# vvvvvw/Sentinel

Hardware: AMD Instinct MI355X
Metric: decided entries/sec (whole node) at 1M resources; % of HBM roofline (higher is better)
Workload: dtype int64/f64

## Files before the change

### sentinel_amd/csrc/chain.h

```cpp
#pragma once
#include <hip/hip_runtime.h>
#include <stdint.h>

#include "../../include/sentinel_gpu.h"
#include "dev_types.h"

namespace sg {

__device__ __forceinline__ int64_t j_d2l(double d) {
    if (d != d) return 0;
    if (d >= 9223372036854775807.0) return INT64_MAX;
    if (d <= -9223372036854775808.0) return INT64_MIN;
    return (int64_t)d;
}
__device__ __forceinline__ int32_t j_d2i(double d) {
    if (d != d) return 0;
    if (d >= 2147483647.0) return INT32_MAX;
    if (d <= -2147483648.0) return INT32_MIN;
    return (int32_t)d;
}
__device__ __forceinline__ int32_t j_iadd(int32_t a, int32_t b) { return (int32_t)((uint32_t)a + (uint32_t)b); }
__device__ __forceinline__ int64_t j_round(double a) {
    int64_t bits = __double_as_longlong(a);
    int64_t biased = (bits & 0x7ff0000000000000LL) >> 52;
// ... 307 lines not shown
__device__ __forceinline__ int64_t try_occupy_next(Node& N, const Ctx& C, int64_t now, int acquire, double threshold,
                                                   int32_t occupy_timeout) {
    const double max_count = threshold * 1000 / 1000;
    const int64_t cur_borrow = bor_waiting(N.bor, now);
    if ((double)cur_borrow >= max_count) return occupy_timeout;
    const int64_t wlen = 500;
    int64_t earliest = now - now % wlen + wlen - 1000;
    int64_t idx = 0;
    sec_current(N, now, C.max_rt);
    int64_t cur_pass = SEC_SUM(N, now, pass);
    while (earliest < now) {
        const int64_t wait = idx * wlen + wlen - now % wlen;
        if (wait >= occupy_timeout) break;
        const int64_t wp = sec_window_pass(N, earliest);
        if ((double)(cur_pass + cur_borrow + acquire - wp) <= max_count) return wait;
        earliest += wlen;
        cur_pass -= wp;
        ++idx;
    }
    return occupy_timeout;
}
__device__ __forceinline__ int default_can_pass_prio(Node& N, const Ctx& C, const DRule& r, int64_t t, int acquire,
                                                     int32_t occupy_timeout, int64_t& wait) {
    int32_t cur;
    if (r.grade == SG_FLOW_GRADE_THREAD) cur = N.thread;
    else { sec_current(N, t, C.max_rt); cur = j_d2i((double)SEC_SUM(N, t, pass)); }
    if (!((double)j_iadd(cur, acquire) > r.count)) return 1;
    if (r.grade != SG_FLOW_GRADE_QPS || !N.bor) return 0;
    const int64_t w = try_occupy_next(N, C, t, acquire, r.count, occupy_timeout);
    if (w >= occupy_timeout) return 0;
    const int bs = bor_current(N.bor, t + w);
    if (bs >= 0) N.bor[2 * bs + 1] += acquire;
    min_current(N, C.minb, t, C.max_rt, C.pflags);
    if (!(N.mst & MS_DETACHED)) {
        N.mb.occ += acquire;
        N.mb.pass += acquire;
        N.mst |= MS_DIRTY;
    }
    wait = w;
    return 2;
}

__device__ __forceinline__ void stat_entry(Node& N, const Ctx& C, int64_t t, int count, bool passed) {
    int sl = sec_current(N, t, C.max_rt);
    min_current(N, C.minb, t, C.max_rt, C.pflags);
    if (passed) {
        N.thread++;
        sec_add(N, sl, count, 0, 0, 0, 0, INT64_MAX);
        min_add(N, count, 0, 0, 0, 0, INT64_MAX);
    } else {
        sec_add(N, sl, 0, count, 0, 0, 0, INT64_MAX);
        min_add(N, 0, count, 0, 0, 0, INT64_MAX);
    }
}
__device__ __forceinline__ void stat_exit(Node& N, const Ctx& C, int64_t t, int count, int64_t rt) {
    int sl = sec_current(N, t, C.max_rt);
    sec_add(N, sl, 0, 0, count, rt, 0, rt);
    min_current(N, C.minb, t, C.max_rt, C.pflags);
    min_add(N, 0, 0, count, rt, 0, rt);
    N.thread--;
}
__device__ __forceinline__ void stat_trace(Node& N, const Ctx& C, int64_t t, int count) {
    if (count <= 0) return;
    int sl = sec_current(N, t, C.max_rt);
    sec_add(N, sl, 0, 0, 0, 0, count, INT64_MAX);
    min_current(N, C.minb, t, C.max_rt, C.pflags);
    if (!(N.mst & MS_DETACHED)) {
        min_add(N, 0, 0, 0, 0, count, INT64_MAX);
        if (N.exc_sum_sec == t - t % 1000) N.exc_sum += count;
    }
}

__device__ __forceinline__ void node_store(const Node& N, const DevState& S, uint32_t res, uint32_t pflags) {
    S.sec[(uint64_t)res * 2 + 0] = N.sb[0];
    S.sec[(uint64_t)res * 2 + 1] = N.sb[1];
    NodeInfo o = S.info[res];
    o.thread = N.thread;
    o.flags = N.flags;
    o.exc_sum_sec = (pflags & PF_EXC_COUNT) ? N.exc_sum_sec : -1;
    o.exc_sum = N.exc_sum;
    S.info[res] = o;
}

}
```

### sentinel_amd/csrc/decide.hip

```cpp
#include <hip/hip_runtime.h>
#include <stdlib.h>
#include <stdint.h>

#include "authority.h"
#include "chain.h"
#include "aux.h"
#include "pmap.h"

using namespace sg;

#define WAVE 64
#define MAXR 16
#define JMAX_FLOW 4
#define JMAX_DEG 4
#define JMAX_RL 2

__device__ __forceinline__ uint32_t lane_id() { return __lane_id(); }
__device__ __forceinline__ uint64_t lanemask_lt() {
    uint32_t l = lane_id();
    return l == 0 ? 0ull : (~0ull >> (64 - l));
}

#define J8_MAX (1u << 23)
#define SEG_ITEMS 16
// ... 1079 lines not shown
                if (r.kind == SG_EV_EXIT) {
                    const uint64_t ref = r.code == RC_NONE ? SG_REF_NONE
                                         : r.code == RC_BATCH ? S.gbase + (vals[r.x] & 0x7FFFFFFFu) : (aux & SG_REF_NONE);
                    lane_exit<NRMAX>(N, C, S, cfg, pg, res, t, r, x, ref, bflags, LP);
                } else {
                    stat_trace(N, C, t, r.cnt);
                }
            }
            LPROF(ktc)
        }
        if (r.kind == SG_EV_ENTRY) dec[sg.start + j] = d;
    }
    min_flush(N, C.minb);
    node_store(N, S, res, pg.pflags);
    if (L.mid != NO_ID) pm_store(S, L.mid, L.mp);
    if (L.tid != NO_ID) pm_store(S, L.tid, L.tm);
#pragma unroll
    for (int s = 0; s < NRMAX; ++s) if (s < nr) S.rstate[pg.rule_off + s] = rs[s];
#ifdef SG_KPROF
    if (kp) {
        S.dbg[32] += kta; S.dbg[33] += ktb; S.dbg[34] += ktc; S.dbg[35] += sg.len; S.dbg[36] += 1;
    }
#endif
#undef LPROF
}
template <int NRMAX>
__global__ __launch_bounds__(256) void k_lane(const SEv* __restrict__ recs, const sg_event* __restrict__ ev,
                                              const uint32_t* __restrict__ vals, const Seg* __restrict__ segs,
                                              const uint32_t* __restrict__ order, uint32_t m, DevState S, DevCfg cfg,
                                              int64_t t0, uint32_t* __restrict__ dec, uint32_t* __restrict__ bflags) {
    const uint32_t i = blockIdx.x * blockDim.x + threadIdx.x;
    if (i >= m) return;
    lane_seg<NRMAX>(recs, ev, vals, segs[order[i]], S, cfg, t0, dec, bflags, i);
}

struct MinDelta {
    int32_t p, b, s, rt, e, minrt;
};
struct LiteMin {
    int64_t T;
    MinDelta pd;
    int64_t H;
};
__device__ __forceinline__ void md_zero(MinDelta& d) { d.p = d.b = d.s = d.rt = d.e = 0; d.minrt = INT32_MAX; }
__device__ __forceinline__ bool md_full(const MinDelta& d) { return (uint32_t)(d.p | d.b | d.s | d.rt | d.e) >= 0x40000000u; }
__device__ __forceinline__ Bkt md_apply(Bkt b, int64_t T, const MinDelta& d, int32_t max_rt) {
    if (b.ws > T) return b;
    if (b.ws < T) bkt_reset(b, T, max_rt);
    b.pass += d.p; b.block += d.b; b.succ += d.s; b.rt += d.rt; b.exc += d.e;
    if ((int64_t)d.minrt < b.minrt) b.minrt = d.minrt;
    return b;
}
__device__ __forceinline__ void lm_put(LiteMin& L, Bkt* minb, int32_t max_rt, bool check, uint32_t* bflags) {
    if (L.T < 0) return;
    Bkt* p = minb + (L.T / 1000) % 60;
    if (L.T > L.H) {
        if (check && p->ws >= L.T) atomicOr(bflags, BF_LITE_STALE);
        Bkt b;
        bkt_reset(b, L.T, max_rt);
        b.pass = L.pd.p; b.block = L.pd.b; b.succ = L.pd.s; b.rt = L.pd.rt; b.exc = L.pd.e;
        if ((int64_t)L.pd.minrt < b.minrt) b.minrt = L.pd.minrt;
        *p = b;
        L.H = L.T;
    } else {
        *p = md_apply(*p, L.T, L.pd, max_rt);
    }
}
__device__ __forceinline__ void lm_roll(LiteMin& L, Node& N, Bkt* minb, int64_t T, int32_t max_rt, uint32_t pflags,
                                        bool check, uint32_t* bflags) {
    lm_put(L, minb, max_rt, check, bflags);
    L.T = T;
    md_zero(L.pd);
    if ((pflags & PF_EXC_COUNT) && N.exc_sum_sec < T) exc_advance(N, minb, T);
}
template <uint32_t CH>
__device__ __forceinline__ void lite_flush(uint32_t* __restrict__ dec, uint32_t base, uint32_t n, const uint32_t (&w)[CH],
                                           uint32_t& mask) {
#pragma unroll
    for (uint32_t m = 0; m < CH; ++m)
        if ((mask >> m) & 1u) dec[base + m - (CH - n)] = w[m];
    mask = 0;
}

#ifndef LITE_PL_WAVES
#define LITE_PL_WAVES 1
#endif
template <bool PL>
__global__ __launch_bounds__(256) __attribute__((amdgpu_waves_per_eu(PL ? LITE_PL_WAVES : 2))) void k_lite(const SEv* __restrict__ recs, const sg_event* __restrict__ ev,
                                              const uint32_t* __restrict__ vals, const Seg* __restrict__ segs,
                                              const uint32_t* __restrict__ order, uint32_t m, DevState S, DevCfg cfg,
                                              int64_t t0, uint32_t* __restrict__ dec, uint32_t* __restrict__ bflags) {
    const uint32_t i = blockIdx.x * blockDim.x + threadIdx.x;
    if (i >= m) return;
    const Seg sg = segs[order[i]];
    const uint32_t res = sg.res;
    const Prog pg = S.prog[res];
    Node N;
    node_load(N, S, res);
#ifndef LITE_CH
#define LITE_CH 4
#endif
    constexpr uint32_t CH = LITE_CH;
    const uint4* r4 = reinterpret_cast<const uint4*>(recs + sg.start);
    const uint32_t qmax = sg.len ? sg.len - 1 : 0;
    uint4 cur[CH], nxt[CH];
#pragma unroll
    for (uint32_t k = 0; k < CH; ++k) cur[k] = r4[k < qmax ? k : qmax];
    if (((pg.xf & XF_PLITE) != 0) != PL) return;
    const int nf = pg.n_flow, nd = pg.n_degrade;
    const DRule* rules = S.rules + pg.rule_off + (PL ? 1 : 0);
    __shared__ DRule spr[PL ? 256 : 1];
    __shared__ PMap smp[PL ? 256 : 1], stm[PL ? 256 : 1];
    DRule& pr = spr[PL ? threadIdx.x : 0];
    PmLaneRef PLM{NO_ID, NO_ID, smp[PL ? threadIdx.x : 0], stm[PL ? threadIdx.x : 0]};
    if (PL) {
        pr = S.rules[pg.rule_off];
        PLM.mid = pr.pmap;
        PLM.mp = S.pmap[pr.pmap];
        PLM.tid = tmap_of(S, pg.tm_base, 0);
        if (PLM.tid != NO_ID) PLM.tm = S.pmap[PLM.tid];
    }
    double fcnt[2] = {0.0, 0.0};
    bool fthr[2] = {false, false};
    uint32_t fslot[2] = {0, 0};
    DegParam dr[2];
    uint32_t dslot[2] = {0, 0};
    RState ds[2];
    if (nf + nd) {
        const int last = nf + nd - 1;
#pragma unroll
        for (int k = 0; k < 2; ++k) {
            const int fi = k < last ? k : last, di = nf + k < last ? nf + k : last;
            fcnt[k] = rules[fi].count;
            fthr[k] = rules[fi].grade == SG_FLOW_GRADE_THREAD;
            fslot[k] = rules[fi].slot;
            dr[k] = deg_param(rules[di]);
            dslot[k] = rules[di].slot;
            ds[k] = S.rstate[pg.rule_off + (PL ? 1 : 0) + di];
        }
    }
#ifdef SG_KPROF
    const bool kp = S.dbg && i == 0;
    unsigned long long kt0 = kp ? __builtin_amdgcn_s_memtime() : 0, kta = 0, ktb = 0, ktc = 0, ktd = 0, ktf = 0, ktg = 0, kth = 0;
#define LPROF(acc)                                                \
    if (kp) {                                                     \
        unsigned long long _n = __builtin_amdgcn_s_memtime();     \
        acc += _n - kt0;                                          \
        kt0 = _n;                                                 \
    }
#else
#define LPROF(acc)
#endif
    const Ctx C{S.minb + (uint64_t)res * 60, cfg.max_rt, pg.pflags};
    LiteMin L;
    L.T = -1;
    md_zero(L.pd);
    {
        const int64_t sw = N.sb[0].ws > N.sb[1].ws ? N.sb[0].ws : N.sb[1].ws;
        const int64_t sh = sw < 0 ? -1 : sw - sw % 1000;
        L.H = sh > cfg.snap_hi ? sh : cfg.snap_hi;
    }
    const bool lchk = (cfg.dbg_flags & LITE_CHECK) != 0;
    const bool has_chain = (N.flags & NI_CHAIN) != 0;
    const bool chain = has_chain && cfg.switch_on;
    if (sg.len && (t0 + recs[sg.start].dt) < (N.sb[0].ws > N.sb[1].ws ? N.sb[0].ws : N.sb[1].ws))
        atomicOr(bflags, BF_BACKWARD);
    uint64_t pm0 = 0, pm1 = 0, pm2 = 0, pm3 = 0;
#ifndef LITE_HOLD
#define LITE_HOLD 1
#endif
    uint32_t dw[CH], dmask = 0;
#pragma unroll
    for (uint32_t k = 0; k < CH; ++k) dw[k] = 0;
    LPROF(kta)
    for (uint32_t j0 = 0; j0 < sg.len; j0 += CH) {
    if (j0) lite_flush<CH>(dec, sg.start + j0 - CH, CH, dw, dmask);
#pragma unroll
    for (uint32_t k = 0; k < CH; ++k) nxt[k] = r4[j0 + CH + k < qmax ? j0 + CH + k : qmax];
#pragma unroll 1
    for (uint32_t k = 0; k < CH; ++k) {
        const uint4 rw = cur[0];
#pragma unroll
        for (uint32_t m = 0; m + 1 < CH; ++m) cur[m] = cur[m + 1];
        const uint32_t j = j0 + k;
        if (j >= sg.len) break;
        const int32_t rdt = (int32_t)rw.x;
        const uint32_t rx = rw.y;
        const int cntv = (int)(rw.z & 0xFFFFu);
        const int32_t rtv = (int32_t)(rw.z >> 16);
        const uint32_t kind = rw.w & 0xFFu, code = (rw.w >> 16) & 0xFFu;
        const int64_t t = t0 + rdt;
        const int64_t T = t - t % 1000;
        uint32_t d = mk_dec(ST_NOT_ENTRY, 0, 0);
        if (kind == SG_EV_ENTRY) {
            if (!chain) d = mk_dec(ST_NO_CHECK, 0, 0);
            else {
                if (T != L.T || md_full(L.pd)) lm_roll(L, N, C.minb, T, C.max_rt, C.pflags, lchk, bflags);
                uint32_t status = ST_PASS, slot = 0;
                uint64_t key = NO_KEY;
                if (PL) {
                    N.flags |= NI_PM | ni_tm(0);
                    if ((rw.w >> 8) & SG_F_HAS_ARG)
                        key = S.key_ring[(S.gbase + (vals[sg.start + j] & 0x7FFFFFFFu)) & cfg.ring_mask];
                    if (key != NO_KEY && !param_default_lane(S, pr, PLM.mp, cntv, key, t, bflags)) {
                        status = ST_BLOCK_PARAM;
                        slot = pr.slot;
                    }
                }
#pragma unroll
                for (int k = 0; k < 2; ++k) {
                    if (k < nf && status == ST_PASS) {
                        int32_t cur;
                        if (fthr[k]) cur = N.thread;
                        else { sec_current(N, t, C.max_rt); cur = j_d2i((double)SEC_SUM(N, t, pass)); }
                        if ((double)j_iadd(cur, cntv) > fcnt[k]) { status = ST_BLOCK_FLOW; slot = fslot[k]; }
                    }
                }
                LPROF(ktf)
                const int64_t exc_total = N.exc_sum;
#pragma unroll
                for (int k = 0; k < 2; ++k) {
                    if (k < nd && status == ST_PASS && !degrade_pass(N, C, dr[k], ds[k], t, &exc_total)) {
                        status = ST_BLOCK_DEGRADE;
                        slot = dslot[k];
                    }
                }
                LPROF(ktg)
                const bool passed = status == ST_PASS;
                const int sl = sec_current(N, t, C.max_rt);
                if (passed) {
                    N.thread++;
                    sec_add(N, sl, cntv, 0, 0, 0, 0, INT64_MAX);
                    L.pd.p += cntv;
                } else {
                    sec_add(N, sl, 0, cntv, 0, 0, 0, INT64_MAX);
                    L.pd.b += cntv;
                }
                LPROF(kth)
                if (PL && passed && key != NO_KEY && PLM.tid != NO_ID) thread_add_lane(S, PLM.tm, key, 1, bflags);
                d = passed ? mk_dec(ST_PASS, 0, 0) : mk_dec(status, slot, 0);
                if (passed && j < 256) {
                    const uint64_t b = 1ull << (j & 63);
                    if (j < 64) pm0 |= b; else if (j < 128) pm1 |= b; else if (j < 192) pm2 |= b; else pm3 |= b;
                }
            }
            LPROF(ktb)
        } else {
            bool eff;
            if (code == RC_NONE) eff = kind == SG_EV_EXIT ? chain : has_chain;
            else if (code == RC_PASSED) eff = true;
            else if (code == RC_NOT) eff = false;
            else {
                const uint32_t rel = rx - sg.start;
                if (rel >= j) { atomicOr(bflags, BF_BAD_REF); eff = false; }
                else if (rel < 256) {
                    const uint64_t w = rel < 64 ? pm0 : rel < 128 ? pm1 : rel < 192 ? pm2 : pm3;
                    eff = ((w >> (rel & 63)) & 1) != 0;
                } else {
                    if (rel >= j0) lite_flush<CH>(dec, sg.start + j0, k, dw, dmask);
                    eff = st_passed(dec[rx] & 0xFF);
                }
            }
            if (eff && kind == SG_EV_EXIT) {
                if (T != L.T || md_full(L.pd)) lm_roll(L, N, C.minb, T, C.max_rt, C.pflags, lchk, bflags);
                const int sl = sec_current(N, t, C.max_rt);
                sec_add(N, sl, 0, 0, cntv, rtv, 0, rtv);
                L.pd.s += cntv;
                L.pd.rt += rtv;
                if (rtv < L.pd.minrt) L.pd.minrt = rtv;
                N.thread--;
                const uint32_t rfl = (rw.w >> 8) & 0xFFu;
                if (PL && (rfl & SG_F_EXIT_ARGS) && (N.flags & NI_PM) && (N.flags & ni_tm(0)) && PLM.tid != NO_ID) {
                    uint64_t ref = SG_REF_NONE;
                    if (rfl & RF_OWN_ARGS) ref = S.gbase + (vals[sg.start + j] & 0x7FFFFFFFu);
                    else if (code == RC_BATCH) ref = S.gbase + (vals[rx] & 0x7FFFFFFFu);
                    else if (code == RC_PASSED) ref = ev[vals[sg.start + j] & 0x7FFFFFFFu].aux & SG_REF_NONE;
                    if (ref != SG_REF_NONE) {
                        const uint64_t key = S.key_ring[ref & cfg.ring_mask];
                        if (key != NO_KEY) thread_add_lane(S, PLM.tm, key, -1, bflags);
                    }
                }
            } else if (eff && cntv > 0) {
                if (T != L.T || md_full(L.pd)) lm_roll(L, N, C.minb, T, C.max_rt, C.pflags, lchk, bflags);
                const int sl = sec_current(N, t, C.max_rt);
                sec_add(N, sl, 0, 0, 0, 0, cntv, INT64_MAX);
                L.pd.e += cntv;
                if (N.exc_sum_sec == T) N.exc_sum += cntv;
            }
            LPROF(ktc)
        }
#if LITE_HOLD
#pragma unroll
        for (uint32_t m = 0; m + 1 < CH; ++m) dw[m] = dw[m + 1];
        dw[CH - 1] = d;
        dmask = (dmask >> 1) | (kind == SG_EV_ENTRY ? 1u << (CH - 1) : 0u);
#else
        if (kind == SG_EV_ENTRY) dec[sg.start + j] = d;
#endif
    }
#pragma unroll
    for (uint32_t k = 0; k < CH; ++k) cur[k] = nxt[k];
    }
    if (sg.len) {
        const uint32_t jl = (sg.len - 1) / CH * CH;
        lite_flush<CH>(dec, sg.start + jl, sg.len - jl, dw, dmask);
    }
    lm_put(L, C.minb, C.max_rt, lchk, bflags);
    node_store(N, S, res, pg.pflags);
#pragma unroll
    for (int k = 0; k < 2; ++k)
        if (k < nd) S.rstate[pg.rule_off + (PL ? 1 : 0) + nf + k] = ds[k];
    if (PL) {
        pm_store(S, PLM.mid, PLM.mp);
        if (PLM.tid != NO_ID) pm_store(S, PLM.tid, PLM.tm);
    }
    LPROF(ktd)
#ifdef SG_KPROF
    if (kp) {
        S.dbg[32] += kta; S.dbg[33] += ktb; S.dbg[34] += ktc; S.dbg[35] += sg.len; S.dbg[36] += 1; S.dbg[37] += ktd; S.dbg[38] += ktf; S.dbg[39] += ktg; S.dbg[51] += kth;
    }
#endif
#undef LPROF
}

#define DPP_STEP(v, ident, ctrl, rmask, OP) \
    v = OP((uint32_t)__builtin_amdgcn_update_dpp((int)(ident), (int)(v), ctrl, rmask, 0xf, false), v)
#define WAVE_SCAN(v, ident, OP)              \
    do {                                      \
        DPP_STEP(v, ident, 0x111, 0xf, OP);   \
        DPP_STEP(v, ident, 0x112, 0xf, OP);   \
        DPP_STEP(v, ident, 0x114, 0xf, OP);   \
        DPP_STEP(v, ident, 0x118, 0xf, OP);   \
        DPP_STEP(v, ident, 0x142, 0xa, OP);   \
        DPP_STEP(v, ident, 0x143, 0xc, OP);   \
    } while (0)
__device__ __forceinline__ uint32_t op_add(uint32_t a, uint32_t b) { return a + b; }
__device__ __forceinline__ uint32_t op_min(uint32_t a, uint32_t b) { return a < b ? a : b; }
__device__ __forceinline__ uint32_t op_max(uint32_t a, uint32_t b) { return a > b ? a : b; }
__device__ __forceinline__ void wave_total64(uint32_t v, uint64_t* dst) {
    uint32_t lo = v & 0xFFFFu, hi = v >> 16;
    WAVE_SCAN(lo, 0u, op_add);
    WAVE_SCAN(hi, 0u, op_add);
    if (lane_id() == 63) *dst = (uint64_t)lo + ((uint64_t)hi << 16);
}
__device__ __forceinline__ uint32_t op_seg(uint32_t a, uint32_t b) {
    return (b & 0x80000000u) ? b : ((a & 0x80000000u) | ((a + b) & 0x7fffffffu));
}
__device__ __forceinline__ uint32_t shr1(uint32_t incl, uint32_t ident) {
    uint32_t v = (uint32_t)__shfl_up((int)incl, 1, 64);
    return lane_id() == 0 ? ident : v;
}
__device__ __forceinline__ int64_t wscan_i64_add(int64_t x) {
    const uint32_t l = lane_id();
#pragma unroll
    for (int o = 1; o < 64; o <<= 1) {
        int64_t y = __shfl_up(x, o, 64);
        if (l >= (uint32_t)o) x += y;
    }
    return x;
}
__device__ __forceinline__ int64_t wscan_i64_max(int64_t x) {
    const uint32_t l = lane_id();
#pragma unroll
    for (int o = 1; o < 64; o <<= 1) {
        int64_t y = __shfl_up(x, o, 64);
        if (l >= (uint32_t)o) x = x > y ? x : y;
    }
    return x;
}
#define NEG_INF64 ((int64_t)0x8000000000000000LL)

#define NO_LANE 0xFFFFFFFFu

#define ROW_SCAN(v, ident, OP, NWV)                                    \
    do {                                                               \
        if ((NWV) > 1) DPP_STEP(v, ident, 0x111, 0xf, OP);              \
        if ((NWV) > 2) DPP_STEP(v, ident, 0x112, 0xf, OP);              \
        if ((NWV) > 4) DPP_STEP(v, ident, 0x114, 0xf, OP);              \
        if ((NWV) > 8) DPP_STEP(v, ident, 0x118, 0xf, OP);              \
    } while (0)
template <int NW>
__device__ __forceinline__ uint32_t blk_min(const uint32_t* a) {
    static_assert(NW <= 16, "one DPP row");
    uint32_t v = lane_id() < (uint32_t)NW ? a[lane_id()] : NO_LANE;
    ROW_SCAN(v, NO_LANE, op_min, NW);
    return (uint32_t)__builtin_amdgcn_readlane((int)v, NW - 1);
}
template <int NW>
__device__ __forceinline__ uint32_t blk_sum_before(const uint32_t* a, uint32_t stride, uint32_t wv, uint32_t* tot) {
    static_assert(NW <= 16, "one DPP row");
    uint32_t v = lane_id() < (uint32_t)NW ? a[lane_id() * stride] : 0u;
    ROW_SCAN(v, 0u, op_add, NW);
    *tot = (uint32_t)__builtin_amdgcn_readlane((int)v, NW - 1);
    return wv == 0 ? 0u : (uint32_t)__builtin_amdgcn_readlane((int)v, (int)wv - 1);
// ... 2293 lines not shown
```

### sentinel_amd/csrc/dev_types.h

```cpp
#pragma once
#include <hip/hip_runtime.h>
#include <stdint.h>

#include "../../include/sentinel_gpu.h"

namespace sg {

struct AuthDesc;

struct Bkt {
    int64_t ws;
    int64_t pass;
    int64_t block;
    int64_t exc;
    int64_t succ;
    int64_t rt;
    int64_t occ;
    int64_t minrt;
};
static_assert(sizeof(Bkt) == 64, "Bkt must be 64 B");

#define NO_KEY 0xFFFFFFFFFFFFFFFFull

enum : uint32_t {
    NI_CHAIN = 1u,
    NI_REJECTED = 2u,
    NI_PM = 4u,
    NI_TOUCHED = 32u,
    NI_TM_SHIFT = 6u
};
__host__ __device__ inline uint32_t ni_tm(uint32_t idx) { return 1u << (NI_TM_SHIFT + idx); }

enum : uint8_t {
    PM_PRIO = 1,
    PM_LANE = 2,
    PM_AUX = 4,
    PM_ARGL = 8,
    PM_XARGS = 16
};
#define TAG_ORIGIN_BITS 20u
__host__ __device__ inline uint32_t tag_origin(uint32_t tag) { return tag & ((1u << TAG_ORIGIN_BITS) - 1); }
__host__ __device__ inline uint32_t tag_ctx(uint32_t tag) { return tag >> TAG_ORIGIN_BITS; }
#define RF_OWN_ARGS 0x80u
#define RF_PBLK 0x40u

struct NodeInfo {
    int32_t thread;
    uint32_t flags;
    int64_t exc_sum_sec;
    int64_t exc_sum;
    int64_t last_fetch;
};
static_assert(sizeof(NodeInfo) == 32, "NodeInfo must be 32 B");

enum : uint8_t {
    PF_EXC_COUNT = 1,
    PF_WARM = 2,
    PF_PQ = 4,
    PF_SERIAL = 8,
    PF_RL = 16,
    PF_RT = 32,
    PF_FROZEN = 64,
    PF_J16 = 128
};

struct Prog {
    uint32_t rule_off;
    uint8_t n_param, n_flow, n_degrade, pflags;
    uint32_t tm_base;
    uint16_t multi;
    uint16_t xf;
};
enum : uint16_t {
    XF_PTHREAD = 1,
    XF_MIX = 2,
    XF_PLITE = 4,
    XF_PVPQ = 8,
    XF_HEADT = 16,
    XF_HEADR = 32
};
enum : uint32_t {
    PX_MULTI = 1,
    PX_ORIGIN = 2,
    PX_CHAIN = 4
};
static_assert(sizeof(Prog) == 16, "Prog must be 16 B");

enum : uint8_t { RK_PARAM = 0, RK_FLOW = 1, RK_DEGRADE = 2 };

enum : uint32_t { LA_DEFAULT = 0, LA_ORIGIN = 1, LA_OTHER = 2 };
#define NO_ID 0xFFFFFFFFu
struct DRule {
    uint8_t kind;
    uint8_t grade;
    uint8_t behavior;
    uint8_t slot;
    int32_t max_queue;
    double count;
    double slope;
    int32_t warning_token;
    int32_t max_token;
    int32_t count_div_cold;
    int32_t time_window;
    int32_t burst;
    int32_t token_count;
    int64_t duration_sec;
    int64_t token_count_l;
    uint32_t hot_off, hot_n;
    uint32_t pmap;
    uint32_t ref;
    int32_t param_idx;
    uint32_t la_kind;
    uint32_t la_origin;
    uint32_t strategy;
    uint32_t chain_ctx;
    uint32_t pad[3];
};
#define NO_REF 0xFFFFFFFFu
#define PB_INIT_ONLY 0xFF
static_assert(sizeof(DRule) == 112, "DRule must be 112 B");

struct DHot {
    uint64_t key;
    int32_t count;
    int32_t pad;
};

struct RState {
    int64_t a;
    int64_t b;
    int64_t c;
    int64_t d;
};

#define PM_BKT 8
#define PK_EMPTY 0xFFFFFFFFFFFFFFFFull
struct PBucket {
    uint64_t key[PM_BKT];
    int64_t stamp[PM_BKT];
};
static_assert(sizeof(PBucket) == 128, "PBucket must be one 128-byte line");
struct PData {
    int64_t v0;
    int32_t v1;
    uint32_t pad;
};
static_assert(sizeof(PData) == 16, "PData must be 16 B");
#define PM_MIN_NB 2u
enum { PC_NEXT = 0, PC_FLOOR = 1, PC_RESCUES = 2, PC_RESCUE = 3, PC_WORDS = 4 };
__host__ __device__ inline uint32_t map_buckets(uint32_t cap) { return (2u * cap + PM_BKT - 1) / PM_BKT > 2u ? (2u * cap + PM_BKT - 1) / PM_BKT : 2u; }
struct PMap {
    uint64_t base;
    uint64_t bm;
    int64_t clock;
    int64_t thr;
    uint32_t nb;
    uint32_t cap;
    uint32_t live;
    uint32_t rb_log2;
    uint32_t pad[4];
};
static_assert(sizeof(PMap) == 64, "PMap must be 64 B");
#define PM_BASE_CAP 4000u
#define PM_TOTAL_CAP 200000u
#define PQ_MAX_CAP 8176u

enum : uint8_t { ST_PASS = 0, ST_PASS_WAIT = 1, ST_BLOCK_FLOW = 2, ST_BLOCK_DEGRADE = 3, ST_BLOCK_PARAM = 4,
                 ST_NO_CHECK = 5, ST_BLOCK_UPSTREAM = 6, ST_BLOCK_AUTHORITY = 7, ST_NOT_ENTRY = 0xFF };

// ... 86 lines not shown
    int64_t occ_pass, occ_req;
};
struct CSlot {
    int64_t key;
    uint32_t idx, pad;
};
#define CP_MAXN 16
struct PFlow {
    int64_t flow_id;
    double count;
    int32_t thr_type;
    int32_t n, interval;
    int32_t connected;
    uint32_t hoff, nhot;
    int64_t fws[CP_MAXN];
};
struct PHot {
    uint64_t key;
    int32_t count, pad;
};
#define PV_EMPTY 0xFFFFFFFFu
struct PVal {
    uint64_t key;
    uint32_t flow, pad;
    int64_t ws[CP_MAXN];
    int64_t cnt[CP_MAXN];
};
#define NS_BUCKETS 10
#define NS_WLEN 100
#define NS_INTERVAL 1000
struct NsLimiter {
    int64_t ws[NS_BUCKETS];
    int64_t cnt[NS_BUCKETS];
};

struct Link {
    uint64_t exit_l;
    uint64_t trace_l;
};
struct Span {
    uint32_t s, e, res;
    int32_t pint;
};
#define SPAN_CHUNK 8192u
#define BST_STATIC 0x80000000u
#define BST_CNT 0x7FFFFFFFu

struct AuxNode {
    unsigned long long key;
    int32_t thread;
    uint32_t flags;
    int64_t mws[2];
    int64_t mpass[2];
    int64_t pad0[2];
    Bkt sec[2];
    int64_t borrow[4];
    int64_t pad1[4];
};
static_assert(sizeof(AuxNode) == 256, "AuxNode size");
#define AUXF_BORROW 1u
#define AUX_EMPTY 0xFFFFFFFFFFFFFFFFull
enum : uint32_t { AUX_ORIGIN = 0, AUX_CONTEXT = 1 };
struct AuxAcc {
    uint32_t key;
    int32_t thread;
    int64_t W[2];
    uint64_t s[2][4];
    uint32_t minrt[2];
    int64_t MW[2];
    uint64_t mpass[2];
};
static_assert(sizeof(AuxAcc) == 128, "AuxAcc size");
#define AUX_PIECE 4096u

struct DevState {
    Bkt* sec;
    int64_t* borrow;
    const uint32_t* prio;
    uint64_t* key_ring;
    uint64_t gbase;
    Bkt* minb;
    NodeInfo* info;
    const Prog* prog;
    const DRule* rules;
    RState* rstate;
    const DHot* hot;
    PMap* pmap;
    PBucket* pbkt;
    PData* pdat;
    uint64_t* pbm;
    uint32_t* ppre;
    const uint32_t* tmid;
    uint8_t* ring;
    unsigned long long* dbg;
    uint32_t* sink;
    const Link* link;
    const uint32_t* bst;
    uint32_t* pend;
    Span* spans;
    uint32_t* nspan;
    uint32_t span_cap;
    uint32_t epoch;
    uint32_t skip_ok;
    uint32_t skip_min;
    const sg_event_ext* ext;
    const sg_arg* args;
    AuxNode* aux_tab;
    uint32_t* aux_count;
    uint32_t aux_cap;
    uint32_t max_ctx;
    uint64_t aux_mask;
    const AuthDesc* auth;
    const uint32_t* auth_ids;
};

enum : uint32_t { BF_PRIORITIZED = 1,
                  BF_PQ_INVARIANT = 2,
                  BF_PTAB_FULL = 4,
                  BF_BAD_RES = 8, BF_BAD_REF = 16,
                  BF_BACKWARD = 32, BF_TSPAN = 64,
                  BF_BAD_ARGS = 512,
                  BF_AUX_FULL = 1024,
                  BF_POOL_FULL = 2048,
                  BF_MULTI_LINK = 128,
                  BF_ZERO_CNT = 256,
                  BF_TINY_FALLBACK = 4096,
                  BF_TINY_REJECTED = 8192,
                  BF_LITE_STALE = 16384 };

struct SEv {
    int32_t dt;
    uint32_t x;
    uint16_t cnt;
    uint16_t rt;
    uint8_t kind;
    uint8_t flags;
    uint8_t code;
    uint8_t pad;
};
static_assert(sizeof(SEv) == 16, "SEv must be 16 B");
enum : uint8_t {
    RC_NONE = 0,
    RC_BATCH = 1,
    RC_PASSED = 2,
    RC_NOT = 3,
    RC_PREV = 4
};

enum : uint32_t {
    BIN_J16 = 0,
    BIN_J4 = 1,
    BIN_J1 = 2,
    BIN_PQ16 = 3,
    BIN_PQ4 = 4,
    BIN_J8 = 5,
    BIN_LANE = 6,
    LANE_BINS = 19,
    BIN_LANE16 = BIN_LANE + LANE_BINS,
    BIN_LITE = BIN_LANE16 + LANE_BINS,
    N_BINS = BIN_LITE + LANE_BINS
};

}
```

### sentinel_amd/csrc/engine.cpp

```cpp
#include <hip/hip_runtime.h>

#include <algorithm>
#include <array>
#include <chrono>
#include <cmath>
#include <cstdint>
#include <cstdio>
#include <cstdlib>
#include <cstring>
#include <deque>
#include <functional>
#include <map>
#include <set>
#include <string>
#include <unordered_map>
#include <vector>

#include "../../include/sentinel_gpu.h"
#include "authority.h"
#include "dev_types.h"
#include "pkeys.h"
#include "pmap.h"

namespace sg {
hipError_t launch_rs_first(const sg_event* ev, uint64_t n, uint32_t max_res, uint64_t gbase, const uint8_t* ring,
                           uint64_t ring_mask, int32_t max_rt, SEv* rec_o, uint32_t* keys, uint32_t* vals,
                           uint32_t* ghist, uint32_t nblocks, uint32_t* bflags, int64_t* t0_out, uint32_t* prio,
                           uint64_t* key_ring, const uint32_t* comp, const sg_event_ext* ext, const sg_arg* args,
                           uint64_t n_args, uint32_t max_ctx, const AuthDesc* auth, const uint32_t* auth_ids,
                           hipStream_t st);
hipError_t launch_radix_hist(const uint32_t* keys, uint64_t n, int shift, uint32_t* ghist, uint32_t nblocks,
                             hipStream_t st);
hipError_t launch_radix_hist_n(const uint32_t* keys, uint64_t n, const uint32_t* ndev, int shift, uint32_t* ghist,
                               uint32_t nblocks, hipStream_t st);
hipError_t launch_radix_scatter_n(const uint32_t* kin, const uint32_t* vin, uint64_t n, const uint32_t* ndev, int shift,
                                  const uint32_t* goff, uint32_t nblocks, uint32_t* kout, uint32_t* vout, hipStream_t st);
hipError_t launch_radix_scatter_x(const uint32_t* kin, const uint32_t* vin, uint64_t n, const uint32_t* ndev,
                                  const uint32_t* tcnt, const uint32_t* dbase, int shift, const uint32_t* goff,
                                  uint32_t nblocks, uint32_t* kout, uint32_t* vout, uint32_t* pos_of, hipStream_t st);
hipError_t launch_grp_first(const sg_event* ev, uint64_t n, uint32_t max_res, uint64_t gbase, uint64_t ring_mask,
                            uint32_t* bflags, int64_t* t0_out, uint32_t* prio, uint64_t* key_ring, const uint32_t* comp,
                            const sg_event_ext* ext, const sg_arg* args, uint64_t n_args, uint32_t max_ctx,
                            const AuthDesc* auth, const uint32_t* auth_ids,
                            const uint16_t* hot_tab, uint32_t nhot, uint32_t nblocks, uint32_t* words,
                            uint32_t* hot_hist, uint32_t* ckeys, uint32_t* cvals, uint32_t* ccnt, uint32_t* chist,
                            hipStream_t st);
hipError_t launch_hot_scan(uint32_t* C, uint32_t nblocks, uint32_t nhot, uint32_t* part, uint32_t* hb, uint32_t* total,
                           hipStream_t st);
hipError_t launch_hot_bmax(const sg_event* ev, uint32_t nblocks, const uint32_t* P, uint32_t nhot, const uint32_t* hb,
                           uint32_t* edges, uint32_t* bmax, hipStream_t st);
hipError_t launch_grp_records(const sg_event* ev, uint64_t n, uint64_t gbase, uint64_t ring_mask, int32_t max_rt,
                              const uint32_t* words, const uint32_t* P, uint32_t nhot, uint32_t nblocks,
                              const uint32_t* hb, SEv* recs, uint32_t* svals, uint32_t* prev,
                              uint32_t* nprev, uint32_t* bst, uint32_t* bflags, const sg_event_ext* ext,
                              const sg_arg* args, uint32_t max_ctx, Link* link, uint32_t epoch,
                              const uint32_t* need_hot, const uint32_t* need_blk, hipStream_t st);
hipError_t launch_hot_segs(const uint32_t* hb, uint32_t nhot, const uint32_t* hot_list, Seg* segs, uint32_t* out,
                           hipStream_t st);
hipError_t launch_hot_build(const Seg* segs, const uint32_t* mp, uint32_t mb, uint32_t min_len, uint32_t max_res, uint16_t* hot_tab,
                            uint32_t* hot_list, uint32_t nhot_old, uint32_t* hot_n, hipStream_t st);
hipError_t launch_cold_n(uint64_t n, const uint32_t* hot_total, uint32_t* out, hipStream_t st);
hipError_t launch_cold_small(const uint32_t* kin, const uint32_t* vin, const uint32_t* cnt, const uint32_t* dbase,
                             uint32_t* kout, uint32_t* vout, uint32_t* words, hipStream_t st);
uint32_t hot_max();
hipError_t launch_grp_clear(uint32_t* bsmall, uint32_t nsmall, uint32_t* bst, uint32_t nbst, uint32_t* need,
                            uint32_t nneed, hipStream_t st);
hipError_t launch_seg_cold(const uint32_t* keys, uint64_t n, const uint32_t* lo, const uint32_t* sbase, uint32_t* flag,
                           uint32_t* pos, Seg* segs, hipStream_t st,
                           hipError_t (*scan)(const uint32_t*, uint32_t*, uint64_t, uint32_t*, uint32_t*, hipStream_t),
                           uint32_t* part, uint32_t* ccount, uint32_t* nseg);
hipError_t launch_block_sums(const SEv* recs, uint64_t n, uint32_t* bst, Link* link, uint32_t epoch, uint32_t* bflags,
                             const uint32_t* skeys, const uint32_t* lo, const uint32_t* need_blk, hipStream_t st);
hipError_t launch_radix_scatter(const uint32_t* kin, const uint32_t* vin, uint64_t n, int shift, const uint32_t* goff,
                                uint32_t nblocks, uint32_t* kout, uint32_t* vout, uint32_t* pos_of, hipStream_t st);
uint32_t radix_tile();
hipError_t launch_scan(const uint32_t*, uint32_t*, uint64_t, uint32_t*, uint32_t*, hipStream_t);
hipError_t launch_snapshot(Bkt*, NodeInfo*, uint32_t, int64_t, int32_t, uint32_t*, uint32_t*, uint32_t*, uint32_t*,
                           sg_metric_node*, uint64_t, hipStream_t);
hipError_t launch_init_state(Bkt* sec, Bkt* minb, NodeInfo* info, int64_t* borrow, uint32_t nres, hipStream_t st);
hipError_t launch_set_flags(NodeInfo* info, const uint64_t* upd, uint32_t n, hipStream_t st);
hipError_t launch_region_copy(const uint64_t* src, uint64_t* dst, const uint64_t* tri, uint32_t n, hipStream_t st);
hipError_t launch_seg(const uint32_t* keys, uint64_t n, uint32_t* flag, uint32_t* pos, Seg* segs, hipStream_t st,
                      hipError_t (*scan)(const uint32_t*, uint32_t*, uint64_t, uint32_t*, uint32_t*, hipStream_t),
                      uint32_t* part, uint32_t* nseg);
hipError_t launch_seg_bin(Seg* segs, const uint32_t* mp, uint32_t mb, uint64_t n, const Prog* prog, const uint32_t* prio,
                          uint32_t lane_max, uint32_t j1_max, uint32_t j4_max, uint32_t force_lane, uint32_t* blkcnt,
                          uint32_t pq_ok, uint32_t pq_wide, uint32_t* aux, uint32_t* ashort, uint64_t* along,
                          uint64_t* amulti, uint32_t* mixc, uint32_t* mix, uint32_t mix_cap, uint32_t* mixlen,
                          uint32_t mix_wide, uint32_t head_min, const uint16_t* hot_tab, uint32_t nhot,
                          const uint32_t* nhotseg, uint32_t* need_hot, uint32_t* need_blk, const uint32_t* bmax,
                          uint32_t skip_min, uint32_t* nmark, hipStream_t st);
hipError_t launch_aux(const SEv* recs, const Seg* segs, const uint32_t* aux, const uint32_t* ashort,
                      const uint64_t* along, uint64_t* apiece, const uint64_t* amulti, const DevState& S, const DevCfg& cfg,
                      int64_t t0, const uint32_t* dec, AuxAcc* pool, uint32_t pool_cap, uint32_t* pool_n, uint64_t* meta,
                      uint32_t* bflags, hipStream_t st);
hipError_t launch_aux_cold(const SEv* recs, const Seg* segs, const uint32_t* aux, const uint32_t* ashort, const DevState& S,
                           const DevCfg& cfg, int64_t t0, const uint32_t* dec, uint32_t* bflags, hipStream_t st);
hipError_t launch_pq(int wide, const SEv* recs, const sg_event* ev, const uint32_t* vals, const Seg* segs,
                     const uint32_t* order, uint32_t m, const DevState& S, const DevCfg& cfg, int64_t t0, uint32_t* dec,
                     uint32_t* bflags, hipStream_t st);
hipError_t launch_pm_grow(const Seg* segs, const uint32_t* mp, uint32_t mb, const DevState& S, unsigned long long* pool_next,
                          uint64_t pool_nb, uint32_t* bflags, uint4* mv, uint32_t* nmv, uint32_t mcap, uint32_t epoch,
                          uint32_t nm, PBucket* b2, PData* d2, uint32_t* sz, uint32_t* off, uint32_t* part,
                          hipError_t (*scan)(const uint32_t*, uint32_t*, uint64_t, uint32_t*, uint32_t*, hipStream_t),
                          hipStream_t st);
hipError_t launch_pm_compact(PMap* pm, uint32_t n, const PBucket* ob, const PData* od, PBucket* nbk, PData* nd,
                             uint32_t* sz, uint32_t* off, uint32_t* part, unsigned long long* pool_next,
                             hipError_t (*scan)(const uint32_t*, uint32_t*, uint64_t, uint32_t*, uint32_t*, hipStream_t),
                             hipStream_t st);
hipError_t launch_pm_grow_ids(const uint32_t* ids, uint32_t n, const DevState& S, unsigned long long* pool_next,
                              uint64_t pool_nb, uint32_t* bflags, hipStream_t st);
hipError_t launch_pv_a(SEv* recs, const uint32_t* vals, Seg* segs, const uint32_t* list, uint32_t m,
                       const DevState& S, const DevCfg& cfg, uint32_t* dec, PvSeg* pv, PvBuf B, uint32_t cap,
                       uint32_t* tot, uint32_t* hist, uint32_t* part, hipStream_t st,
                       hipError_t (*radix_hist)(const uint32_t*, uint64_t, const uint32_t*, int, uint32_t*, uint32_t, hipStream_t),
                       hipError_t (*radix_scatter)(const uint32_t*, const uint32_t*, uint64_t, const uint32_t*, int,
                                                   const uint32_t*, uint32_t, uint32_t*, uint32_t*, hipStream_t),
                       hipError_t (*scan)(const uint32_t*, uint32_t*, uint64_t, uint32_t*, uint32_t*, hipStream_t),
                       uint32_t tile, uint32_t* rest, uint32_t grant_all);
hipError_t launch_pv_b(SEv* recs, Seg* segs, const uint32_t* list, uint32_t m, const DevState& S, int64_t t0,
                       uint32_t* dec, uint32_t* bflags, PvSeg* pv, PvBuf B, uint32_t cap, uint32_t* tot, uint32_t* part,
                       uint32_t jumps, hipStream_t st,
                       hipError_t (*scan)(const uint32_t*, uint32_t*, uint64_t, uint32_t*, uint32_t*, hipStream_t),
                       uint32_t* rest);
hipError_t launch_pvt(SEv* recs, const sg_event* ev, const uint32_t* vals, Seg* segs, const uint32_t* list, uint32_t m,
                      const DevState& S, const DevCfg& cfg, uint32_t* dec, uint32_t* bflags, PvSeg* pv, PvBuf B,
                      uint32_t cap, uint32_t* tot, uint32_t* hist, uint32_t* part, hipStream_t st,
                      hipError_t (*radix_hist)(const uint32_t*, uint64_t, const uint32_t*, int, uint32_t*, uint32_t, hipStream_t),
                      hipError_t (*radix_scatter)(const uint32_t*, const uint32_t*, uint64_t, const uint32_t*, int,
                                                      const uint32_t*, uint32_t, uint32_t*, uint32_t*, hipStream_t),
                      hipError_t (*scan)(const uint32_t*, uint32_t*, uint64_t, uint32_t*, uint32_t*, hipStream_t),
                      uint32_t tile, uint32_t* rest);
hipError_t launch_pq_mix(int post, SEv* recs, const sg_event* ev, const uint32_t* vals, const Seg* segs,
// ... 287 lines not shown
    h = h31(h, s.burst_count);
    h = h31(h, long_hash(s.duration_in_sec));
    int32_t lh = 1;
    for (auto& q : p.items) {
        int32_t e = q.has_obj ? j_string_hash(q.obj.c_str()) : 0;
        e = h31(e, q.has_count ? q.count : 0);
        e = h31(e, q.has_ct ? j_string_hash(q.ct.c_str()) : 0);
        lh = h31(lh, e);
    }
    h = h31(h, lh);
    h = h31(h, s.cluster_mode ? 1 : 0);
    int32_t ch = 0;
    if (s.cluster_mode || s.cluster_flow_id)
        ch = cluster_hash(s.cluster_flow_id, s.cluster_threshold_type, s.cluster_fallback_to_local, 0,
                          s.cluster_sample_count, s.cluster_window_interval_ms, false);
    p.hash = h31(h, ch);
    char buf[512];
    std::snprintf(buf, sizeof(buf), "%d|%016llx|%d|%d|%d|%lld|%d|%d:%d|", s.grade, (unsigned long long)dbl_bits(s.count),
                  s.control_behavior, s.max_queueing_time_ms, s.burst_count, (long long)s.duration_in_sec,
                  s.cluster_mode ? 1 : 0, s.has_param_idx, s.has_param_idx ? s.param_idx : 0);
    std::string k = std::string(buf) + p.res + "\x01" + p.la + "\x01";
    for (auto& q : p.items) {
        std::snprintf(buf, sizeof(buf), "[%d%d%d:%d]", q.has_obj, q.has_ct, q.has_count, q.has_count ? q.count : 0);
        k += buf + q.obj + "\x02" + q.ct + "\x03";
    }
    if (s.cluster_mode || s.cluster_flow_id) {
        std::snprintf(buf, sizeof(buf), "C%lld|%d|%d|%d|%d", (long long)s.cluster_flow_id, s.cluster_threshold_type,
                      s.cluster_fallback_to_local ? 1 : 0, s.cluster_sample_count, s.cluster_window_interval_ms);
        k += buf;
    }
    p.eqkey = k;
    return p;
}

template <class T> void dfree(T*& p) {
    if (p) (void)hipFree(p);
    p = nullptr;
}

}

#define TMAP_KEY (1ull << 63)
struct sg_engine {
    sg_config cfg;
    int device = 0;
    hipStream_t stream = nullptr;
    double last_ms[4] = {0, 0, 0, 0};

    std::unordered_map<std::string, uint32_t> ids;
    std::vector<std::string> names;
    uint32_t n_chains = 0;

    bool flow_loaded = false, deg_loaded = false, par_loaded = false;
    std::vector<std::string> last_flow, last_deg, last_par;
    std::vector<FlowR> flows;
    std::vector<DegR> degs;
    std::vector<ParamR> params;
    std::vector<std::vector<int>> res_flow, res_deg, res_par;
    std::map<std::string, uint32_t> psid_of;
    uint32_t next_psid = 1;
    std::map<uint32_t, uint32_t> rmap_cap;
    std::set<uint64_t> tmaps;
    std::vector<uint64_t> pmap_key;
    std::unordered_map<uint32_t, uint32_t> pmap_index;
    std::vector<uint32_t> tm_base;
    uint64_t n_pslot = 0;
    uint64_t pool_nb = 0;
    unsigned long long* d_pool_next = nullptr;
    uint4* d_pmoves = nullptr;
    PBucket* d_pbkt2 = nullptr;
    PData* d_pdat2 = nullptr;
    uint32_t* d_pcwork = nullptr;
    uint64_t pmoves_cap = 0;
    unsigned long long* h_pool_next = nullptr;
    uint64_t n_compact = 0;
    uint64_t pool2_nb = 0;
    uint32_t n_dev_rules = 0;

    Bkt* d_sec = nullptr;
    Bkt* d_minb = nullptr;
    int64_t snap_hi = -1;
    NodeInfo* d_info = nullptr;
    Prog* d_prog = nullptr;
    DRule* d_rules = nullptr;
    RState* d_rstate = nullptr;
    DHot* d_hot = nullptr;
    PMap* d_pmap = nullptr;
    PBucket* d_pbkt = nullptr;
    PData* d_pdat = nullptr;
    uint64_t* d_pbm = nullptr;
    uint32_t* d_ppre = nullptr;
    uint32_t* d_tmid = nullptr;
    uint8_t* d_ring = nullptr;
    uint32_t rules_cap = 0, hot_cap = 0;

    struct BatchSlot {
        sg_event* d_ev = nullptr;
        uint32_t* d_out = nullptr;
        uint32_t *d_k0 = nullptr, *d_v0 = nullptr, *d_k1 = nullptr, *d_v1 = nullptr;
        uint32_t *d_hist = nullptr, *d_part = nullptr, *d_flag = nullptr, *d_pos = nullptr, *d_order = nullptr;
        uint32_t *d_posof = nullptr, *d_dec = nullptr, *d_blkcnt = nullptr, *d_prev = nullptr;
        SEv *d_recs = nullptr, *d_rec_o = nullptr;
        uint32_t* d_ccnt = nullptr;
        bool radix = false;
        uint32_t nhot = 0;
        uint32_t hot_marked = 0;
        Seg* d_segs = nullptr;
        uint64_t* d_cand = nullptr;
        uint32_t* d_bsmall = nullptr;
        sg_event_ext* d_ext = nullptr;
        sg_arg* d_args = nullptr;
        uint64_t ext_cap = 0, args_cap = 0;
        uint32_t* d_ashort = nullptr;
        uint64_t *d_apiece = nullptr, *d_amulti = nullptr, *d_along = nullptr;
        uint64_t aux_cap_n = 0;
        uint32_t* d_mix = nullptr;
        uint64_t mix_cap = 0;
        Link* d_link = nullptr;
        uint32_t *d_bst = nullptr, *d_pend = nullptr;
        Span* d_spans = nullptr;
        hipEvent_t* ev = nullptr;
        hipEvent_t last_post = nullptr;
        uint32_t* h_head = nullptr;
        struct Grouped {
            uint64_t n = 0, n_args = 0, gbase = 0, ring_mask = 0;
            const sg_event* dev_ev = nullptr;
            const sg_event_ext* dev_ext = nullptr;
            const sg_arg* dev_args = nullptr;
            uint32_t *out = nullptr, *dev_out = nullptr, *vin = nullptr;
            uint32_t epoch = 0, skip_min = 0, lane_max = 0, mb = 0;
            bool ext = false, host_out = false, force_lane = false;
            int set = 0;
        } g;
    } slot[2];
    int cur = 0;
    int last = -1;
    int grouped = -1;
    int held_rc = 0;
    std::string held_msg;
    bool handoff_late = true;
    static constexpr int N_SETS = 4;
    hipEvent_t evset[N_SETS][5] = {};
    uint32_t* h_mirror = nullptr;
    uint64_t seq = 0;
    struct InFlight { int set; uint32_t hot_marked; };
    std::deque<InFlight> inflight;
    hipStream_t gstream = nullptr;
    std::vector<std::array<double, 4>> tlog;
    std::vector<std::array<double, 2>> glog;
    std::string fatal;
    uint32_t* d_prio = nullptr;
    uint16_t* d_hot_tab = nullptr;
    uint32_t* d_hot_list = nullptr;
    uint32_t nhot = 0;
    uint32_t* d_hot_part = nullptr;
    uint32_t* d_hot_hb = nullptr;
    uint32_t* d_need = nullptr;
    uint64_t need_words = 0;
    uint32_t* d_edges = nullptr;
    uint32_t hot_marked_last = 0;
    bool radix_group = false;
    uint64_t radix_below = 1u << 18;
    uint32_t tok_light = 8192;
    uint32_t tok_wide = 1024;
    bool tiny_on = true;
    AuxNode* d_auxtab = nullptr;
    uint32_t* d_auxcnt = nullptr;
    uint64_t aux_mask = 0;
    AuxAcc* d_auxpool = nullptr;
    uint64_t* d_auxmeta = nullptr;
    uint32_t auxpool_cap = 0;
    uint64_t auxmeta_cap = 0;
    std::unordered_map<std::string, uint32_t> origin_ids, context_ids;
    std::unordered_map<std::string, int> rule_names;
    AuthTable auth;
    AuthDesc* d_auth = nullptr;
    uint32_t* d_auth_ids = nullptr;
    size_t auth_ids_cap = 0;
    bool auth_on = false, auth_loaded = false;
    std::vector<std::string> last_auth;
    uint32_t* d_comp = nullptr;
    uint32_t* d_prev = nullptr;
    uint32_t* d_bsmall = nullptr;
    Link* d_link = nullptr;
    uint32_t *d_bst = nullptr, *d_pend = nullptr;
    Span* d_spans = nullptr;
    uint32_t span_cap = 0;
    uint32_t epoch = 0;
    uint64_t spans_total = 0;
    uint64_t cap_n = 0;
    sg_event* d_ev = nullptr;
    uint32_t* d_out = nullptr;
    uint32_t *d_k0 = nullptr, *d_v0 = nullptr, *d_k1 = nullptr, *d_v1 = nullptr;
    uint32_t *d_hist = nullptr, *d_part = nullptr, *d_flag = nullptr, *d_pos = nullptr, *d_order = nullptr;
    uint32_t *d_posof = nullptr, *d_dec = nullptr, *d_blkcnt = nullptr;
    SEv *d_recs = nullptr, *d_rec_o = nullptr;
    Seg* d_segs = nullptr;
    uint32_t* d_small = nullptr;
    uint32_t* d_sink = nullptr;
    int64_t* d_borrow = nullptr;
    uint64_t* d_keyring = nullptr;
    uint64_t* d_cand = nullptr;
    uint32_t dbg_flags = 0;
    int prof_bin = 0;
    unsigned long long* d_dbg = nullptr;
    uint64_t cap_hist = 0;
    uint64_t gbase = 0;
    hipStream_t bin_stream[2] = {nullptr, nullptr};
    hipEvent_t fork = nullptr, join[2] = {nullptr, nullptr};
    hipEvent_t fork0 = nullptr;
    hipEvent_t grown = nullptr;
    bool pipeline = true;
    int j1_stream = -1;
    uint32_t lane_max = 256, j1_max = 4096, j4_max = 65536;
    uint32_t head_min = 0;
    bool bins_pinned = false;
    uint32_t skip_min = 32768;
    bool pq_on = true;
    uint32_t pq_wide = 8192;
    bool mix_on = true;
    bool mix_pq = false;
    bool pv_pq = true;
    bool has_mix = false;
    bool has_head = false;
    bool pv_on = true;
    PvBuf pvb{};
    PvBuf pvbt{};
    bool has_multi = false;
    uint64_t pv_cap = 0;
    PvSeg* d_pvseg = nullptr;
    PvSeg* d_pvtseg = nullptr;
    uint32_t* d_pvrest = nullptr;
    bool pvt_on = false;
    uint64_t pvseg_cap = 0;
    uint64_t pvch_cap = 0;
    uint32_t *d_pvtot = nullptr, *d_pvhist = nullptr, *d_pvpart = nullptr, *d_pvthist = nullptr, *d_pvtpart = nullptr;
    uint32_t pv_last_m = 0;
    bool skip_pinned = false;
    std::vector<CFlow> cflows;
    std::unordered_map<int64_t, uint32_t> cmap;
    CFlow* d_cflow = nullptr;
    CBkt* d_cbkt = nullptr;
// ... 23 lines not shown
    uint32_t pftab_mask = 0;
    PVal* d_pvtab = nullptr;
    uint32_t pv_mask = 0;
    sg_param_token_req* d_preq = nullptr;
    uint64_t* d_pvals = nullptr;
    uint64_t pcap = 0, pvcap = 0;
    pk::Dict<pk::StdHash> pkeys;
    std::vector<uint64_t> par_pins;
    uint64_t* d_ks_key = nullptr;
    uint32_t *d_ks_idx = nullptr, *d_ks_marks = nullptr;
    uint64_t ks_cap = 0;
    hipEvent_t ks_ev[4] = {nullptr, nullptr, nullptr, nullptr};
    uint64_t ks_sweeps = 0, ks_last[4] = {0, 0, 0, 0};
    double ks_scan_ms[3] = {0, 0, 0};
    uint64_t pbm_words = 0;
    uint32_t *d_snap_cnt = nullptr, *d_snap_off = nullptr;
    sg_metric_node* d_snap_out = nullptr;
    uint64_t snap_cap = 0;
};

static int handoff(sg_engine* e);

namespace {

constexpr uint64_t SHARD_BATCH = 3ull << 21;

static void activate(sg_engine* e, int k) {
    auto& B = e->slot[k];
    e->d_ev = B.d_ev; e->d_out = B.d_out;
    e->d_k0 = B.d_k0; e->d_v0 = B.d_v0; e->d_k1 = B.d_k1; e->d_v1 = B.d_v1;
    e->d_hist = B.d_hist; e->d_part = B.d_part; e->d_flag = B.d_flag; e->d_pos = B.d_pos; e->d_order = B.d_order;
    e->d_posof = B.d_posof; e->d_dec = B.d_dec; e->d_blkcnt = B.d_blkcnt; e->d_prev = B.d_prev;
    e->d_recs = B.d_recs; e->d_rec_o = B.d_rec_o; e->d_segs = B.d_segs; e->d_cand = B.d_cand;
    e->d_bsmall = B.d_bsmall;
    e->d_link = B.d_link; e->d_bst = B.d_bst; e->d_pend = B.d_pend; e->d_spans = B.d_spans;
}
static void free_slot(sg_engine::BatchSlot& B) {
    dfree(B.d_ev); dfree(B.d_out); dfree(B.d_k0); dfree(B.d_v0); dfree(B.d_k1); dfree(B.d_v1);
    dfree(B.d_hist); dfree(B.d_part); dfree(B.d_flag); dfree(B.d_pos); dfree(B.d_order); dfree(B.d_segs);
    dfree(B.d_cand); dfree(B.d_posof); dfree(B.d_dec); dfree(B.d_recs); dfree(B.d_rec_o); dfree(B.d_blkcnt);
    dfree(B.d_prev); dfree(B.d_bsmall); dfree(B.d_ccnt);
    B.d_ccnt = nullptr;
    dfree(B.d_link); dfree(B.d_bst); dfree(B.d_pend); dfree(B.d_spans); dfree(B.d_ext); dfree(B.d_args);
    dfree(B.d_ashort); dfree(B.d_apiece); dfree(B.d_amulti); dfree(B.d_along); dfree(B.d_mix);
    B.d_mix = nullptr;
    B.ext_cap = B.args_cap = B.aux_cap_n = B.mix_cap = 0;
    B.d_link = nullptr; B.d_bst = B.d_pend = nullptr; B.d_spans = nullptr;
    B.d_ev = nullptr; B.d_out = nullptr; B.d_k0 = B.d_v0 = B.d_k1 = B.d_v1 = nullptr;
    B.d_hist = B.d_part = B.d_flag = B.d_pos = B.d_order = nullptr;
    B.d_posof = B.d_dec = B.d_blkcnt = B.d_prev = B.d_bsmall = nullptr;
    B.d_recs = B.d_rec_o = nullptr; B.d_segs = nullptr; B.d_cand = nullptr;
}
int ensure_batch(sg_engine* e, uint64_t n) {
    if (n <= e->cap_n) return SG_OK;
    uint64_t c = std::max<uint64_t>(n, 1u << 20);
    HIPCHK(hipStreamSynchronize(e->stream));
    uint64_t nblocks = (c + radix_tile() - 1) / radix_tile();
    e->cap_hist = nblocks * 256;
    for (auto& B : e->slot) {
        free_slot(B);
        HIPCHK(hipMalloc(&B.d_ev, c * sizeof(sg_event)));
        HIPCHK(hipMalloc(&B.d_out, c * 4));
        HIPCHK(hipMalloc(&B.d_k0, c * 4));
        HIPCHK(hipMalloc(&B.d_v0, c * 4));
        HIPCHK(hipMalloc(&B.d_k1, c * 4));
        HIPCHK(hipMalloc(&B.d_v1, c * 4));
        HIPCHK(hipMalloc(&B.d_hist, e->cap_hist * 4));
        HIPCHK(hipMalloc(&B.d_part, (e->cap_hist / 4096 + c / 4096 + 64) * 4));
        HIPCHK(hipMalloc(&B.d_flag, c * 4));
        HIPCHK(hipMalloc(&B.d_pos, c * 4));
        HIPCHK(hipMalloc(&B.d_order, c * 4));
        HIPCHK(hipMalloc(&B.d_segs, c * sizeof(Seg)));
        HIPCHK(hipMalloc(&B.d_cand, c * 8));
        HIPCHK(hipMalloc(&B.d_posof, c * 4));
        HIPCHK(hipMalloc(&B.d_dec, c * 4));
        HIPCHK(hipMalloc(&B.d_recs, c * sizeof(SEv)));
        const uint64_t co = (e->radix_group || c >= (1ull << 30)) ? c : std::min<uint64_t>(c, e->radix_below);
        if (co) HIPCHK(hipMalloc(&B.d_rec_o, co * sizeof(SEv)));
        HIPCHK(hipMalloc(&B.d_ccnt, 3 * (nblocks + 64) * 4));
    }
    dfree(e->d_hot_part);
    dfree(e->d_hot_hb);
    dfree(e->d_need);
    dfree(e->d_edges);
    e->need_words = hot_max() + c / 32768 + 2 + hot_max();
    HIPCHK(hipMalloc(&e->d_need, e->need_words * 4));
    HIPCHK(hipMalloc(&e->d_edges, (nblocks + 2) * 4));
    HIPCHK(hipMalloc(&e->d_hot_part, (nblocks / 16 + 2) * hot_max() * 4));
    HIPCHK(hipMalloc(&e->d_hot_hb, 2 * hot_max() * 4));
    for (auto& B : e->slot) {
        HIPCHK(hipMalloc(&B.d_blkcnt, ((c + 255) / 256 + 1) * N_BINS * 4));
        HIPCHK(hipMalloc(&B.d_prev, c * 4));
        HIPCHK(hipMalloc(&B.d_bsmall, 256 * 4));
        HIPCHK(hipMemset(B.d_bsmall, 0, 256 * 4));
        HIPCHK(hipMalloc(&B.d_link, c * sizeof(Link)));
        HIPCHK(hipMemset(B.d_link, 0, c * sizeof(Link)));
        HIPCHK(hipMalloc(&B.d_bst, ((c + 1023) / 1024 + 1) * 4));
        HIPCHK(hipMalloc(&B.d_pend, c * 4));
        HIPCHK(hipMalloc(&B.d_spans, (c / SPAN_CHUNK + 65536) * sizeof(Span)));
    }
    e->span_cap = (uint32_t)(c / SPAN_CHUNK + 65536);
    e->cap_n = c;
    activate(e, e->cur);
    return SG_OK;
}

constexpr uint32_t HEAD_WORDS = 77;
constexpr uint32_t MIRROR_WORDS = 121;

static int collect(sg_engine* e) {
    if (e->inflight.empty()) return SG_OK;
    const sg_engine::InFlight f = e->inflight.front();
    e->inflight.pop_front();
    hipEvent_t* ev = e->evset[f.set];
    HIPCHK(hipEventSynchronize(ev[4]));
    float g = 0, d = 0, p = 0;
    (void)hipEventElapsedTime(&g, ev[0], ev[1]);
    (void)hipEventElapsedTime(&d, ev[2], ev[3]);
    (void)hipEventElapsedTime(&p, ev[3], ev[4]);
    (void)hipGetLastError();
    e->last_ms[0] = g; e->last_ms[1] = d; e->last_ms[2] = p; e->last_ms[3] = (double)g + d + p;
    e->tlog.push_back({(double)g, (double)d, (double)p, (double)g + d + p});
    if (e->tlog.size() > 4096) e->tlog.erase(e->tlog.begin(), e->tlog.begin() + 2048);
    float ga = 0, gb = 0;
    const uint64_t collected = e->seq - e->inflight.size() - 1;
    if (collected > 0) {
        hipEvent_t* pv = e->evset[(f.set + sg_engine::N_SETS - 1) % sg_engine::N_SETS];
        if (hipEventElapsedTime(&ga, pv[1], ev[0]) != hipSuccess) ga = NAN;
        if (hipEventElapsedTime(&gb, pv[4], ev[2]) != hipSuccess) gb = NAN;
        (void)hipGetLastError();
    }
    e->glog.push_back({(double)ga, (double)gb});
    if (e->glog.size() > 4096) e->glog.erase(e->glog.begin(), e->glog.begin() + 2048);
    const uint32_t* mir = e->h_mirror + (size_t)f.set * MIRROR_WORDS;
    const uint32_t bflags = mir[0];
    e->spans_total += mir[120];
    e->hot_marked_last = f.hot_marked;
    if (bflags & BF_BAD_REF)
        return fail(SG_EINVAL, "an EXIT/TRACE references an event that is not an earlier ENTRY of the same resource");
    if (bflags & BF_BACKWARD)
        return fail(SG_EINVAL, "event timestamps must be non-decreasing across batches (SURVEY Q3)");
    if (bflags & BF_AUX_FULL) return fail(SG_ECAPACITY, "origin/context node pool full (raise aux_node_capacity)");
    if (bflags & BF_LITE_STALE)
        return fail(SG_ESTATE, "internal error (SG_LITE_CHECK): k_lite stored a minute bucket without a load that was not stale");
    if (bflags & BF_PQ_INVARIANT)
        e->fatal = "internal error: a k_pq tile's presorted key subset did not match its accesses";
    else if (bflags & BF_POOL_FULL)
        e->fatal = "the hot-parameter map pool is used up (raise param_table_log2)";
    else if (bflags & BF_PTAB_FULL)
        e->fatal = "a hot-parameter map table could not place a key (its map holds a ghost entry)";
    if (bflags & (BF_PQ_INVARIANT | BF_PTAB_FULL | BF_POOL_FULL)) return fail(SG_ECAPACITY, e->fatal + " -- engine unusable");
    return SG_OK;
}
static inline const AuthDesc* dev_auth(const sg_engine* e) { return e->auth_on ? e->d_auth : nullptr; }
static inline const uint32_t* dev_auth_ids(const sg_engine* e) { return e->auth_on ? e->d_auth_ids : nullptr; }

static int drain(sg_engine* e) {
    int rc = e->held_rc;
    std::string msg = e->held_msg;
    e->held_rc = 0;
    auto note = [&](int r) {
        if (r && !rc) { rc = r; msg = g_err; }
    };
    note(handoff(e));
    while (!e->inflight.empty()) note(collect(e));
    HIPCHK(hipStreamSynchronize(e->stream));
    return rc ? fail(rc, msg) : SG_OK;
}
static void drain_hold(sg_engine* e) {
    const int rc = drain(e);
    if (rc) { e->held_rc = rc; e->held_msg = g_err; }
}


static uint32_t rule_map_cap(int64_t duration_sec) {
    const int64_t c = (int64_t)PM_BASE_CAP * std::max<int64_t>(duration_sec, 1);
    return (uint32_t)std::min<int64_t>(c, PM_TOTAL_CAP);
}

int upload_rules(sg_engine* e, bool reset_flow_state, bool reset_deg_state, bool reset_par_state) {
    uint32_t R = e->cfg.max_resources;
    std::vector<Prog> prog(R);
    std::vector<DRule> rules;
    std::vector<RState> rst;
    std::vector<DHot> hot;
    std::vector<RState> old_rst;
    std::vector<Prog> old_prog;
    if ((!reset_flow_state || !reset_deg_state || !reset_par_state) && e->n_dev_rules) {
        old_rst.resize(e->n_dev_rules);
        old_prog.resize(R);
        HIPCHK(hipMemcpy(old_rst.data(), e->d_rstate, e->n_dev_rules * sizeof(RState), hipMemcpyDeviceToHost));
        HIPCHK(hipMemcpy(old_prog.data(), e->d_prog, R * sizeof(Prog), hipMemcpyDeviceToHost));
    }
    size_t nres = e->names.size();
    bool any_mix = false, any_head = false;
    std::vector<std::pair<uint32_t, uint32_t>> relate;
    for (size_t r = 0; r < nres && r < R; ++r) {
        Prog p;
        std::memset(&p, 0, sizeof(p));
        p.rule_off = (uint32_t)rules.size();
        p.tm_base = r < e->tm_base.size() ? e->tm_base[r] : NO_ID;
        const auto& pl = r < e->res_par.size() ? e->res_par[r] : std::vector<int>();
        for (size_t i = 0; i < pl.size(); ++i) {
            const ParamR& q = e->params[pl[i]];
            DRule d;
            std::memset(&d, 0, sizeof(d));
            d.kind = RK_PARAM;
            d.grade = (uint8_t)q.r.grade;
            d.behavior = (uint8_t)q.r.control_behavior;
            if (q.r.cluster_mode && q.r.grade == SG_FLOW_GRADE_QPS && !q.r.cluster_fallback_to_local) {
                d.behavior = PB_INIT_ONLY;
                if (q.r.param_idx >= 0 && p.n_param && rules.back().behavior == PB_INIT_ONLY &&
                    rules.back().param_idx >= 0) {
                    if (q.r.param_idx < SG_MAX_ARGS) rules.back().burst |= (int32_t)(1u << q.r.param_idx);
                    continue;
                }
            }
            d.slot = (uint8_t)i;
            d.max_queue = q.r.max_queueing_time_ms;
            d.count = q.r.count;
            d.burst = q.r.burst_count;
            if (d.behavior == PB_INIT_ONLY && q.r.param_idx >= 0)
                d.burst = q.r.param_idx < SG_MAX_ARGS ? (int32_t)(1u << q.r.param_idx) : 0;
            double c = q.r.count;
            d.token_count = (c != c) ? 0 : c >= 2147483647.0 ? INT32_MAX : (int32_t)c;
            d.token_count_l = (c != c) ? 0 : c >= 9.2e18 ? INT64_MAX : (int64_t)c;
            d.duration_sec = q.r.duration_in_sec;
            d.hot_off = (uint32_t)hot.size();
            d.hot_n = (uint32_t)q.hot.size();
            for (auto& h : q.hot) hot.push_back(DHot{h.first, h.second, 0});
            d.pmap = e->pmap_index.at(e->psid_of.at(q.res + std::string("\0", 1) + q.eqkey));
            d.param_idx = q.r.param_idx;
            d.ref = NO_REF;
            rules.push_back(d);
            rst.push_back(RState{0, 0, 0, 0});
            p.n_param++;
        }
        const auto& fl = r < e->res_flow.size() ? e->res_flow[r] : std::vector<int>();
        std::vector<uint32_t> skipped_origins;
        for (size_t i = 0; i < fl.size(); ++i) {
            const FlowR& f = e->flows[fl[i]];
            if (!(f.r.cluster_mode && !f.r.cluster_fallback_to_local) || f.la == "default" || f.la == "other") continue;
            auto oi = e->origin_ids.find(f.la);
            if (oi != e->origin_ids.end()) skipped_origins.push_back(oi->second);
        }
        for (size_t i = 0; i < fl.size(); ++i) {
            const FlowR& f = e->flows[fl[i]];
            if (f.r.cluster_mode && !f.r.cluster_fallback_to_local) continue;
            DRule d;
            std::memset(&d, 0, sizeof(d));
            d.kind = RK_FLOW;
            d.grade = (uint8_t)f.r.grade;
            d.behavior = (uint8_t)(f.r.grade == SG_FLOW_GRADE_QPS ? f.r.control_behavior : SG_CONTROL_BEHAVIOR_DEFAULT);
            if (d.behavior > 3) d.behavior = SG_CONTROL_BEHAVIOR_DEFAULT;
            d.slot = (uint8_t)i;
            d.max_queue = f.r.max_queueing_time_ms;
            d.count = f.r.count;
            d.ref = NO_REF;
            d.la_kind = f.la == "default" ? LA_DEFAULT : f.la == "other" ? LA_OTHER : LA_ORIGIN;
            auto oi = e->origin_ids.find(f.la);
// ... 131 lines not shown
            if (!reset_flow_state && op.n_flow == p.n_flow)
                for (int i = 0; i < p.n_flow; ++i) rst[p.rule_off + p.n_param + i] = old_rst[op.rule_off + op.n_param + i];
            if (!reset_deg_state && op.n_degrade == p.n_degrade)
                for (int i = 0; i < p.n_degrade; ++i)
                    rst[p.rule_off + p.n_param + p.n_flow + i] = old_rst[op.rule_off + op.n_param + op.n_flow + i];
        }
        prog[r] = p;
    }
    std::vector<uint32_t> comp;
    bool any_multi = false;
    if (!relate.empty()) {
        comp.resize(R);
        for (uint32_t x = 0; x < R; ++x) comp[x] = x;
        std::function<uint32_t(uint32_t)> find = [&](uint32_t x) { return comp[x] == x ? x : comp[x] = find(comp[x]); };
        for (auto& pr : relate) {
            uint32_t a = find(pr.first), b = find(pr.second);
            if (a != b) comp[std::max(a, b)] = std::min(a, b);
        }
        for (uint32_t x = 0; x < R; ++x) comp[x] = find(x);
        std::vector<uint32_t> members;
        for (uint32_t x = 0; x < R; ++x)
            if (comp[x] != x) { members.push_back(x); members.push_back(comp[x]); }
        std::sort(members.begin(), members.end());
        members.erase(std::unique(members.begin(), members.end()), members.end());
        for (uint32_t x : members) {
            if (comp[x] == x) { prog[x].multi |= PX_MULTI; prog[x].pflags |= PF_SERIAL; }
        }
        any_multi = !members.empty();
        std::vector<NodeInfo> ni(members.size());
        for (size_t k = 0; k < members.size(); ++k)
            HIPCHK(hipMemcpy(&ni[k], e->d_info + members[k], sizeof(NodeInfo), hipMemcpyDeviceToHost));
        for (size_t k = 0; k < members.size(); ++k) {
            if (ni[k].flags & NI_CHAIN) ni[k].flags |= NI_TOUCHED;
            HIPCHK(hipMemcpy(e->d_info + members[k], &ni[k], sizeof(NodeInfo), hipMemcpyHostToDevice));
        }
        if (e->d_pmap) {
            const std::set<uint32_t> ms(members.begin(), members.end());
            std::vector<uint32_t> ids;
            for (uint32_t i = 0; i < (uint32_t)e->pmap_key.size(); ++i)
                if ((e->pmap_key[i] & TMAP_KEY) && ms.count((uint32_t)(e->pmap_key[i] >> 8))) ids.push_back(i);
            for (const auto& kv : e->psid_of) {
                auto it = e->ids.find(kv.first.substr(0, kv.first.find('\0')));
                auto pi = e->pmap_index.find(kv.second);
                if (it != e->ids.end() && ms.count(it->second) && pi != e->pmap_index.end()) ids.push_back(pi->second);
            }
            if (!ids.empty()) {
                uint32_t* d_ids = nullptr;
                HIPCHK(hipMalloc(&d_ids, ids.size() * 4));
                HIPCHK(hipMemcpy(d_ids, ids.data(), ids.size() * 4, hipMemcpyHostToDevice));
                DevState Sg{};
                std::memset(&Sg, 0, sizeof(Sg));
                Sg.pmap = e->d_pmap; Sg.pbkt = e->d_pbkt; Sg.pdat = e->d_pdat; Sg.pbm = e->d_pbm;
                HIPCHK(hipMemset(e->d_small, 0, 4));
                HIPCHK(launch_pm_grow_ids(d_ids, (uint32_t)ids.size(), Sg, e->d_pool_next, e->pool_nb, e->d_small, e->stream));
                uint32_t fl = 0;
                HIPCHK(hipMemcpyAsync(&fl, e->d_small, 4, hipMemcpyDeviceToHost, e->stream));
                HIPCHK(hipStreamSynchronize(e->stream));
                (void)hipFree(d_ids);
                if (fl & (BF_POOL_FULL | BF_PTAB_FULL))
                    return fail(SG_ECAPACITY, "hot-parameter map pool too small for the maps of STRATEGY_RELATE members "
                                              "(raise param_table_log2)");
            }
        }
    }
    if (rules.size() > e->cfg.max_rules) return fail(SG_ECAPACITY, "compiled rule table exceeds max_rules");
    if (rules.size() > e->rules_cap) {
        dfree(e->d_rules); dfree(e->d_rstate);
        e->rules_cap = (uint32_t)std::max<size_t>(rules.size(), 1024);
        HIPCHK(hipMalloc(&e->d_rules, e->rules_cap * sizeof(DRule)));
        HIPCHK(hipMalloc(&e->d_rstate, e->rules_cap * sizeof(RState)));
    }
    if (hot.size() > e->hot_cap) {
        dfree(e->d_hot);
        e->hot_cap = (uint32_t)std::max<size_t>(hot.size(), 1024);
        HIPCHK(hipMalloc(&e->d_hot, e->hot_cap * sizeof(DHot)));
    }
    HIPCHK(hipDeviceSynchronize());
    if (!rules.empty()) {
        HIPCHK(hipMemcpy(e->d_rules, rules.data(), rules.size() * sizeof(DRule), hipMemcpyHostToDevice));
        HIPCHK(hipMemcpy(e->d_rstate, rst.data(), rst.size() * sizeof(RState), hipMemcpyHostToDevice));
    }
    if (!hot.empty()) HIPCHK(hipMemcpy(e->d_hot, hot.data(), hot.size() * sizeof(DHot), hipMemcpyHostToDevice));
    HIPCHK(hipMemcpy(e->d_prog, prog.data(), R * sizeof(Prog), hipMemcpyHostToDevice));
    e->n_dev_rules = (uint32_t)rules.size();
    e->has_mix = any_mix;
    e->has_head = any_head;
    e->has_multi = any_multi;
    if (comp.empty()) {
        dfree(e->d_comp);
        e->d_comp = nullptr;
    } else {
        if (!e->d_comp) HIPCHK(hipMalloc(&e->d_comp, (uint64_t)R * 4));
        HIPCHK(hipMemcpy(e->d_comp, comp.data(), (uint64_t)R * 4, hipMemcpyHostToDevice));
    }
    return SG_OK;
}

uint32_t intern(sg_engine* e, const std::string& name) {
    auto it = e->ids.find(name);
    if (it != e->ids.end()) return it->second;
    uint32_t id = (uint32_t)e->names.size();
    e->ids.emplace(name, id);
    e->names.push_back(name);
    return id;
}

template <class V> void resize_lists(sg_engine* e, V& v) {
    if (v.size() < e->names.size()) v.resize(e->names.size());
}

}

extern "C" {

const char* sg_last_error(void) { return g_err.c_str(); }

void sg_config_default(sg_config* c) {
    std::memset(c, 0, sizeof(*c));
    c->sample_count = 2;
    c->interval_ms = 1000;
    c->statistic_max_rt = 4900;
    c->cold_factor = 3;
    c->occupy_timeout_ms = 500;
    c->max_slot_chain_size = 6000;
    c->switch_on = 1;
    c->device = 0;
    c->max_resources = 1u << 20;
    c->max_rules = 1u << 21;
    c->param_table_log2 = 28;
    c->status_ring_log2 = 28;
    c->max_batch_events = 1u << 25;
    c->cluster_sample_count = 10;
    c->cluster_interval_ms = 1000;
    c->cluster_exceed_count = 1.0;
    c->cluster_max_occupy_ratio = 1.0;
    c->cluster_max_allowed_qps = 30000;
    c->aux_node_capacity = 65536;
}

int sg_engine_create(const sg_config* cfg_in, sg_engine** out) {
    if (!out) return fail(SG_EINVAL, "out is null");
    sg_config cfg;
    if (cfg_in) cfg = *cfg_in;
    else sg_config_default(&cfg);
    if (cfg.sample_count != 2 || cfg.interval_ms != 1000)
        return fail(SG_ENOTSUP, "the device path implements SAMPLE_COUNT=2, INTERVAL=1000 (the reference defaults)");
    if (cfg.cold_factor <= 1) return fail(SG_EINVAL, "cold factor must be > 1");
    if (cfg.max_resources == 0 || cfg.param_table_log2 < 4 || cfg.param_table_log2 > 34 || cfg.status_ring_log2 < 10 ||
        cfg.status_ring_log2 > 36)
        return fail(SG_EINVAL, "bad capacity in sg_config");
    int ndev = 0;
    if (hipGetDeviceCount(&ndev) != hipSuccess || ndev == 0) return fail(SG_EDEVICE, "no HIP device visible");
    if (cfg.device < 0 || cfg.device >= ndev) return fail(SG_EDEVICE, "device ordinal out of range");
    hipDeviceProp_t prop;
    if (hipGetDeviceProperties(&prop, cfg.device) != hipSuccess) return fail(SG_EDEVICE, "hipGetDeviceProperties failed");
    if (std::strncmp(prop.gcnArchName, "gfx950", 6) != 0)
        return fail(SG_EDEVICE, std::string("this build targets gfx950, found ") + prop.gcnArchName);
    sg_engine* e = new sg_engine();
    e->cfg = cfg;
    e->device = cfg.device;
    auto bad = [&](int rc) { sg_engine_destroy(e); return rc; };
    if (hipSetDevice(e->device) != hipSuccess) return bad(fail(SG_EDEVICE, "hipSetDevice failed"));
    int prio_lo = 0, prio_hi = 0;
    const char* sp = std::getenv("SG_STREAM_PRIO");
    if (!(sp && sp[0] == '0')) (void)hipDeviceGetStreamPriorityRange(&prio_lo, &prio_hi);
    if (!(sp && sp[0] == '1')) std::swap(prio_lo, prio_hi);
    if (hipStreamCreateWithPriority(&e->stream, hipStreamNonBlocking, prio_hi) != hipSuccess) return bad(fail(SG_EDEVICE, "stream"));
    if (hipStreamCreateWithPriority(&e->gstream, hipStreamNonBlocking, prio_lo) != hipSuccess) {
        return bad(fail(SG_EDEVICE, "stream"));
    }
    for (auto& s : e->evset)
        for (auto& v : s) if (hipEventCreate(&v) != hipSuccess) return bad(fail(SG_EDEVICE, "event"));
    for (auto& B : e->slot) {
        if (hipHostMalloc(&B.h_head, HEAD_WORDS * 4) != hipSuccess) return bad(fail(SG_ENOMEM, "pinned batch head"));
        B.ev = e->evset[0];
    }
    if (hipHostMalloc(&e->h_mirror, sg_engine::N_SETS * MIRROR_WORDS * 4) != hipSuccess)
        return bad(fail(SG_ENOMEM, "pinned batch flags"));
    std::memset(e->h_mirror, 0, sg_engine::N_SETS * MIRROR_WORDS * 4);
    uint64_t R = cfg.max_resources;
    if (hipMalloc(&e->d_sec, R * 2 * sizeof(Bkt)) != hipSuccess || hipMalloc(&e->d_minb, R * 60 * sizeof(Bkt)) != hipSuccess ||
        hipMalloc(&e->d_info, R * sizeof(NodeInfo)) != hipSuccess || hipMalloc(&e->d_prog, R * sizeof(Prog)) != hipSuccess ||
        hipMalloc(&e->d_ring, 1ull << cfg.status_ring_log2) != hipSuccess || hipMalloc(&e->d_small, 256 * 4) != hipSuccess ||
        hipMalloc(&e->d_sink, 1024 * 4) != hipSuccess || hipMalloc(&e->d_borrow, R * 4 * sizeof(int64_t)) != hipSuccess ||
        hipMalloc(&e->d_prio, R * 4) != hipSuccess || hipMalloc(&e->d_hot_tab, R * 2) != hipSuccess ||
        hipMalloc(&e->d_hot_list, hot_max() * 4) != hipSuccess)
        return bad(fail(SG_ENOMEM, "device allocation of the engine state failed"));
    {
        const uint64_t cap = std::max<uint32_t>(cfg.aux_node_capacity, 16u);
        uint64_t slots = 32;
        while (2 * slots < 3 * cap) slots <<= 1;
        e->aux_mask = slots - 1;
        e->cfg.aux_node_capacity = (uint32_t)cap;
        if (hipMalloc(&e->d_auxtab, slots * sizeof(AuxNode)) != hipSuccess || hipMalloc(&e->d_auxcnt, 4) != hipSuccess ||
            hipMemsetAsync(e->d_auxtab, 0xFF, slots * sizeof(AuxNode), e->stream) != hipSuccess ||
            hipMemsetAsync(e->d_auxcnt, 0, 4, e->stream) != hipSuccess)
            return bad(fail(SG_ENOMEM, "device allocation of the origin/context node table failed"));
    }
    if (hipMemsetAsync(e->d_prog, 0, R * sizeof(Prog), e->stream) != hipSuccess ||
        hipMemsetAsync(e->d_ring, 0xFF, 1ull << cfg.status_ring_log2, e->stream) != hipSuccess ||
        hipMemsetAsync(e->d_prio, 0, R * 4, e->stream) != hipSuccess ||
        hipMemsetAsync(e->d_hot_tab, 0xFF, R * 2, e->stream) != hipSuccess ||
        launch_init_state(e->d_sec, e->d_minb, e->d_info, e->d_borrow, (uint32_t)R, e->stream) != hipSuccess ||
        hipStreamSynchronize(e->stream) != hipSuccess)
        return bad(fail(SG_EDEVICE, "device initialisation failed"));
    for (auto& s : e->bin_stream)
        if (hipStreamCreateWithPriority(&s, hipStreamNonBlocking, prio_hi) != hipSuccess) return bad(fail(SG_EDEVICE, "stream"));
    if (hipEventCreateWithFlags(&e->fork, hipEventDisableTiming) != hipSuccess ||
        hipEventCreateWithFlags(&e->fork0, hipEventDisableTiming) != hipSuccess ||
        hipEventCreateWithFlags(&e->grown, hipEventDisableTiming) != hipSuccess)
        return bad(fail(SG_EDEVICE, "event"));
    for (auto& v : e->join)
        if (hipEventCreateWithFlags(&v, hipEventDisableTiming) != hipSuccess) return bad(fail(SG_EDEVICE, "event"));
    if (const char* d = std::getenv("SG_DEBUG")) {
        if (d[0] == '1' && hipMalloc(&e->d_dbg, 64 * 8) == hipSuccess) (void)hipMemset(e->d_dbg, 0, 64 * 8);
    }
    if (const char* f = std::getenv("SG_DEBUG_FLAGS")) e->dbg_flags = (uint32_t)std::strtoul(f, nullptr, 0);
    e->radix_group = (e->dbg_flags & 8192) != 0;
    if (const char* f = std::getenv("SG_PROF_BIN")) e->prof_bin = std::atoi(f);
    if (const char* v = std::getenv("SG_LANE_MAX")) { e->lane_max = (uint32_t)std::strtoul(v, nullptr, 0); e->bins_pinned = true; }
    if (const char* v = std::getenv("SG_J1_MAX")) { e->j1_max = (uint32_t)std::strtoul(v, nullptr, 0); e->bins_pinned = true; }
    if (const char* v = std::getenv("SG_HEAD_MIN")) e->head_min = (uint32_t)std::strtoul(v, nullptr, 0);
    if (const char* v = std::getenv("SG_J4_MAX")) { e->j4_max = (uint32_t)std::strtoul(v, nullptr, 0); e->bins_pinned = true; }
    if (const char* v = std::getenv("SG_PIPELINE")) e->pipeline = v[0] == '1';
    if (const char* v = std::getenv("SG_HANDOFF")) e->handoff_late = v[0] != '0';
    if (const char* v = std::getenv("SG_TINY")) e->tiny_on = v[0] != '0';
    if (const char* v = std::getenv("SG_LITE_CHECK")) { if (v[0] == '1') e->dbg_flags |= LITE_CHECK; }
    if (const char* v = std::getenv("SG_RADIX_BELOW")) e->radix_below = std::strtoull(v, nullptr, 0);
    if (const char* v = std::getenv("SG_TOK_WIDE")) e->tok_wide = std::atoi(v) == 512 ? 512u : 1024u;
    if (const char* v = std::getenv("SG_TOK_LIGHT")) e->tok_light = (uint32_t)std::strtoul(v, nullptr, 0);
    if (const char* v = std::getenv("SG_TOK_NS")) e->tok_ns = v[0] == '1';
    e->ns_names.push_back("default");
    e->ns_of["default"] = 0;
    e->ns_limit.push_back((double)cfg.cluster_max_allowed_qps);
    e->ns_conn.push_back(0);
    if (const char* v = std::getenv("SG_J1_STREAM")) e->j1_stream = std::atoi(v);
    if (const char* v = std::getenv("SG_PQ")) e->pq_on = v[0] != '0';
    if (const char* v = std::getenv("SG_MIX")) e->mix_on = v[0] != '0';
    if (const char* v = std::getenv("SG_MIX_PQ")) e->mix_pq = v[0] != '0';
    if (const char* v = std::getenv("SG_PV_PQ")) e->pv_pq = v[0] != '0';
    if (const char* v = std::getenv("SG_PV")) e->pv_on = v[0] != '0';
    e->pvt_on = e->pv_on;
    if (const char* v = std::getenv("SG_PVT")) e->pvt_on = v[0] != '0';
    if (const char* v = std::getenv("SG_PQ_WIDE")) e->pq_wide = (uint32_t)std::strtoul(v, nullptr, 0);
    if (const char* v = std::getenv("SG_SKIP_MIN")) {
        e->skip_min = std::max<uint32_t>(1u, (uint32_t)std::strtoul(v, nullptr, 0));
        e->skip_pinned = true;
    }
    *out = e;
    return SG_OK;
}

extern "C" int sgx_timing_log(sg_engine* e, double* out, int cap) {
    if (!e || !out) return 0;
    drain_hold(e);
    int k = 0;
    for (; k < cap && k < (int)e->tlog.size(); ++k)
        for (int j = 0; j < 4; ++j) out[4 * k + j] = e->tlog[k][j];
    e->tlog.clear();
    return k;
}
extern "C" int sgx_gap_log(sg_engine* e, double* out, int cap) {
    if (!e || !out) return 0;
    drain_hold(e);
    int k = 0;
    for (; k < cap && k < (int)e->glog.size(); ++k)
        for (int j = 0; j < 2; ++j) out[2 * k + j] = e->glog[k][j];
    e->glog.clear();
    return k;
}
extern "C" unsigned long long sgx_spans_total(sg_engine* e) {
    if (!e) return 0;
    drain_hold(e);
    return e->spans_total;
}
extern "C" unsigned int sgx_hot_marked(sg_engine* e) {
    if (!e) return 0;
    drain_hold(e);
    return e->hot_marked_last;
}
extern "C" int sgx_debug_reset(sg_engine* e) {
    if (!e || !e->d_dbg) return 0;
    drain_hold(e);
    unsigned long long z[64] = {0};
    z[20] = ~0ull;
    return hipMemcpy(e->d_dbg, z, sizeof(z), hipMemcpyHostToDevice) == hipSuccess ? 1 : 0;
}
extern "C" int sgx_debug_counters(sg_engine* e, unsigned long long* out, int cap) {
    if (!e || !e->d_dbg || !out) return 0;
    int k = cap < 64 ? cap : 64;
    if (hipDeviceSynchronize() != hipSuccess) return 0;
    if (hipMemcpy(out, e->d_dbg, (size_t)k * 8, hipMemcpyDeviceToHost) != hipSuccess) return 0;
    return k;
}

extern "C" int sgx_read_aux_node(sg_engine* e, uint32_t res, uint32_t kind, uint32_t id, long long* out) {
    if (!e || !out || drain(e) != SG_OK) return -1;
    const unsigned long long key = ((unsigned long long)res << 32) | ((unsigned long long)kind << 31) | (id & 0x7FFFFFFFu);
    uint64_t h = mix64(key) & e->aux_mask;
    for (uint64_t probe = 0; probe <= e->aux_mask; ++probe) {
        AuxNode a;
        if (hipMemcpy(&a, e->d_auxtab + h, sizeof(a), hipMemcpyDeviceToHost) != hipSuccess) return -1;
        if (a.key == AUX_EMPTY) return 0;
        if (a.key == key) {
            for (int p = 0; p < 2; ++p) {
                const Bkt& b = a.sec[p];
                const int64_t v[8] = {b.ws, b.pass, b.block, b.exc, b.succ, b.rt, b.occ, b.minrt};
                for (int k = 0; k < 8; ++k) out[8 * p + k] = v[k];
            }
            out[16] = a.thread;
            out[17] = a.mws[0]; out[18] = a.mpass[0]; out[19] = a.mws[1]; out[20] = a.mpass[1];
            return 1;
        }
        h = (h + 1) & e->aux_mask;
    }
    return 0;
}
extern "C" int sgx_pv_last(sg_engine* e, unsigned long long* out) {
    if (!e || !out || drain(e) != SG_OK) return -1;
    out[0] = out[1] = out[2] = out[3] = out[4] = out[5] = out[6] = 0;
    if (!e->d_pvseg || !e->d_pvtot || !e->pv_last_m) return 0;
    std::vector<PvSeg> v(e->pv_last_m);
    uint32_t tot[8] = {0, 0, 0, 0, 0, 0, 0, 0};
    if (hipMemcpy(v.data(), e->d_pvseg, v.size() * sizeof(PvSeg), hipMemcpyDeviceToHost) != hipSuccess) return -1;
    if (hipMemcpy(tot, e->d_pvtot, 32, hipMemcpyDeviceToHost) != hipSuccess) return -1;
    for (const auto& s : v) out[0] += s.ok ? 1 : 0;
    out[1] = tot[0];
    out[2] = tot[2];
    out[6] = tot[3];
    if (e->pvt_on && e->d_pvtseg) {
        if (hipMemcpy(v.data(), e->d_pvtseg, v.size() * sizeof(PvSeg), hipMemcpyDeviceToHost) != hipSuccess) return -1;
        for (const auto& s : v) out[3] += s.ok ? 1 : 0;
        out[4] = tot[4];
        out[5] = tot[7];
    }
    if (!e->pv_on) out[0] = out[1] = out[2] = out[6] = 0;
    return 0;
}
extern "C" int sgx_param_pool(sg_engine* e, unsigned long long* out) {
    if (!e || !out || drain(e) != SG_OK) return -1;
    unsigned long long ctl[PC_WORDS] = {0, 0, 0, 0};
    if (e->d_pool_next && hipMemcpy(ctl, e->d_pool_next, sizeof(ctl), hipMemcpyDeviceToHost) != hipSuccess) return -1;
    out[0] = e->pool_nb; out[1] = ctl[PC_NEXT]; out[2] = ctl[PC_FLOOR]; out[3] = e->n_compact; out[4] = ctl[PC_RESCUES];
    return 0;
}

static int compact_pmaps(sg_engine* e);
extern "C" int sgx_param_compact(sg_engine* e) {
    if (!e || drain(e) != SG_OK) return -1;
    if (!e->pool_nb) return 0;
    if (compact_pmaps(e) != SG_OK) return -1;
    ++e->n_compact;
    return 0;
}

static void free_pv(sg_engine* e);

int sg_engine_destroy(sg_engine* e) {
    if (!e) return SG_OK;
    (void)hipSetDevice(e->device);
    e->grouped = -1;
    if (e->stream) (void)hipStreamSynchronize(e->stream);
    if (e->gstream) (void)hipStreamSynchronize(e->gstream);
    dfree(e->d_sec); dfree(e->d_minb); dfree(e->d_info); dfree(e->d_prog); dfree(e->d_rules); dfree(e->d_rstate);
    dfree(e->d_hot); dfree(e->d_pmap); dfree(e->d_pbkt); dfree(e->d_pdat); dfree(e->d_pbm); dfree(e->d_ppre); dfree(e->d_tmid); dfree(e->d_ring); dfree(e->d_small); dfree(e->d_sink);
    dfree(e->d_pool_next); dfree(e->d_pmoves); dfree(e->d_pbkt2); dfree(e->d_pdat2); dfree(e->d_pcwork);
    if (e->h_pool_next) (void)hipHostFree(e->h_pool_next);
    free_pv(e);
    dfree(e->d_pvseg); dfree(e->d_pvtseg); dfree(e->d_pvtot); dfree(e->d_pvrest);
    if (e->gstream) (void)hipStreamSynchronize(e->gstream);
    for (auto& B : e->slot) free_slot(B);
    dfree(e->d_auth); dfree(e->d_auth_ids);
    dfree(e->d_prio); dfree(e->d_hot_tab); dfree(e->d_hot_list); dfree(e->d_hot_part); dfree(e->d_hot_hb); dfree(e->d_need); dfree(e->d_edges); dfree(e->d_comp); dfree(e->d_auxtab); dfree(e->d_auxpool); dfree(e->d_auxcnt); dfree(e->d_auxmeta);
    dfree(e->d_pflow); dfree(e->d_phot); dfree(e->d_pftab); dfree(e->d_pvtab); dfree(e->d_preq); dfree(e->d_pvals);
    dfree(e->d_cflow); dfree(e->d_cbkt); dfree(e->d_ctab); dfree(e->d_nslim); dfree(e->d_nslimit); dfree(e->d_nsb); dfree(e->d_borrow); dfree(e->d_keyring);
    dfree(e->d_treq); dfree(e->d_tres); dfree(e->d_tfidx); dfree(e->d_tbounds);
    dfree(e->d_snap_cnt); dfree(e->d_snap_off); dfree(e->d_snap_out); dfree(e->d_dbg);
    dfree(e->d_ks_key); dfree(e->d_ks_idx); dfree(e->d_ks_marks);
    for (auto& v : e->ks_ev) if (v) (void)hipEventDestroy(v);
    for (auto& s : e->evset)
        for (auto& v : s) if (v) (void)hipEventDestroy(v);
    for (auto& B : e->slot) if (B.h_head) (void)hipHostFree(B.h_head);
    if (e->h_mirror) (void)hipHostFree(e->h_mirror);
    if (e->gstream) (void)hipStreamDestroy(e->gstream);
    for (auto& v : e->join) if (v) (void)hipEventDestroy(v);
    if (e->fork) (void)hipEventDestroy(e->fork);
    if (e->fork0) (void)hipEventDestroy(e->fork0);
    if (e->grown) (void)hipEventDestroy(e->grown);
    for (auto& s : e->bin_stream) if (s) (void)hipStreamDestroy(s);
    if (e->stream) (void)hipStreamDestroy(e->stream);
    delete e;
    return SG_OK;
}

int sg_register_resources(sg_engine* e, const char* const* names, uint32_t n, uint32_t* out_ids) {
    if (!e || (n && !names)) return fail(SG_EINVAL, "null argument");
    if (int rc = drain(e)) return rc;
    for (uint32_t i = 0; i < n; ++i) {
        if (!names[i]) return fail(SG_EINVAL, "null resource name");
        auto it = e->ids.find(names[i]);
        uint32_t id;
        if (it != e->ids.end()) id = it->second;
        else {
            if (e->names.size() >= e->cfg.max_resources) return fail(SG_ECAPACITY, "max_resources reached");
            id = intern(e, names[i]);
        }
        if (out_ids) out_ids[i] = id;
    }
    return SG_OK;
}

int sg_resource_id(sg_engine* e, const char* name, uint32_t* out_id) {
    if (!e || !name || !out_id) return fail(SG_EINVAL, "null argument");
    auto it = e->ids.find(name);
    if (it == e->ids.end()) return fail(SG_ENOTFOUND, std::string("unknown resource ") + name);
    *out_id = it->second;
    return SG_OK;
}

int sg_param_key(sg_engine* e, const char* value, const char* class_type, uint64_t* out_key) {
    (void)e;
    if (!out_key) return fail(SG_EINVAL, "null out_key");
    *out_key = param_key(value, class_type);
    return SG_OK;
}

static int register_rule_resource(sg_engine* e, const char* name, uint32_t* id) {
    auto it = e->ids.find(name);
    if (it != e->ids.end()) { *id = it->second; return SG_OK; }
    if (e->names.size() >= e->cfg.max_resources) return fail(SG_ECAPACITY, "max_resources reached");
    *id = intern(e, name);
    return SG_OK;
}

int sg_param_intern(sg_engine* e, const char* value, const char* class_type, uint64_t* out_key) {
    if (!e || !out_key) return fail(SG_EINVAL, "null argument");
    *out_key = e->pkeys.intern(value, class_type);
    return SG_OK;
}

int sg_param_intern_batch(sg_engine* e, const char* const* values, const char* const* class_types, uint32_t n,
                          uint64_t* out_keys) {
    if (!e || (n && (!values || !out_keys))) return fail(SG_EINVAL, "null argument");
    for (uint32_t i = 0; i < n; ++i) out_keys[i] = e->pkeys.intern(values[i], class_types ? class_types[i] : nullptr);
    return SG_OK;
}

int sg_param_keys_sweep(sg_engine* e) {
    if (!e) return fail(SG_EINVAL, "null engine");
    HIPCHK(hipSetDevice(e->device));
    if (int rc = drain(e)) return rc;
    const auto t_start = std::chrono::steady_clock::now();
    std::vector<uint64_t> cand;
    const uint64_t E = e->pkeys.sweep_begin(cand);
    const uint64_t nc = cand.size();
    std::vector<uint32_t> held((nc + 31) / 32, 0u);
// ... 856 lines not shown
        }
        HIPCHK(hipMemcpyAsync(B.d_args, args, n_args * sizeof(sg_arg), hipMemcpyHostToDevice, gs));
        dev_args = B.d_args;
    }
    const uint64_t ring_mask = (1ull << e->cfg.status_ring_log2) - 1;
    if (!e->pipeline && e->last >= 0 && e->slot[e->last].last_post)
        HIPCHK(hipStreamWaitEvent(gs, e->slot[e->last].last_post, 0));
    HIPCHK(hipEventRecord(B.ev[0], gs));
    uint32_t R = e->cfg.max_resources;
    int bits = 1;
    while (bits < 32 && (1ull << bits) < R) ++bits;
    const int db = 8;
    int passes = (bits + db - 1) / db;
    uint32_t nblocks = (uint32_t)((n + radix_tile() - 1) / radix_tile());
    int64_t* d_t0 = reinterpret_cast<int64_t*>(e->d_bsmall + 4);
    uint32_t *kin = e->d_k1, *vin = e->d_v1, *kout = e->d_k0, *vout = e->d_v0;
    if (++e->epoch == 0) e->epoch = 1;
    B.radix = e->radix_group || n >= (1ull << 30) || n < e->radix_below;
    HIPCHK(launch_grp_clear(e->d_bsmall, 256, e->d_bst, B.radix ? 0u : (uint32_t)((n + 1023) / 1024), e->d_need,
                            B.radix ? 0u : (uint32_t)e->need_words, gs));
    const bool force_lane = !e->cfg.switch_on || (e->dbg_flags & 2);
    const uint32_t mb = (uint32_t)std::min<uint64_t>(n, R);
    const uint32_t nblk = (mb + 255) / 256;
    uint32_t lane_max = e->lane_max, j1_max = e->j1_max, j4_max = e->j4_max;
    if (!e->bins_pinned && n < SHARD_BATCH) {
        lane_max = std::min<uint32_t>(lane_max, 128);
        j1_max = std::min<uint32_t>(j1_max, 1024);
        j4_max = std::min<uint32_t>(j4_max, 4096);
    }
    j1_max = std::min<uint32_t>(j1_max, 64u * 65000u);
    j4_max = std::min<uint32_t>(j4_max, 256u * 65000u);
    const uint32_t skip_min = (!e->skip_pinned && n < SHARD_BATCH) ? std::min<uint32_t>(e->skip_min, 8192) : e->skip_min;
    auto bins = [&](uint32_t* need_hot, uint32_t* need_blk, const uint32_t* bmax) -> int {
        if (ext) {
            if (int arc = ensure_aux(e, B, n)) return arc;
        }
        if (e->has_mix) {
            if (int mrc = ensure_mix(B, mb)) return mrc;
        }
        HIPCHK(launch_seg_bin(e->d_segs, e->d_bsmall + 1, mb, n, e->d_prog, e->d_prio, lane_max, j1_max, j4_max,
                              force_lane ? 1 : 0, e->d_blkcnt, e->pq_on ? 1u : 0u, e->pq_wide, ext ? e->d_bsmall + 130 : nullptr,
                              B.d_ashort, B.d_along, B.d_amulti, e->d_bsmall + 6, e->has_mix ? B.d_mix : nullptr,
                              (uint32_t)B.mix_cap, e->d_bsmall + 72, (e->pv_on || e->pvt_on) ? 0u : e->pq_wide,
                              (e->dbg_flags & HEAD_OFF) ? 0u : e->head_min, e->d_hot_tab, e->nhot, e->d_bsmall + 80, need_hot,
                              need_blk, bmax, skip_min, e->d_bsmall + 73, gs));
        HIPCHK(launch_scan(e->d_blkcnt, e->d_blkcnt, (uint64_t)nblk * N_BINS, e->d_part, nullptr, gs));
        HIPCHK(launch_seg_order(e->d_segs, e->d_bsmall + 1, mb, e->d_blkcnt, e->d_order, e->d_bsmall + 8, gs));
        return SG_OK;
    };
    auto decide_prev = [&]() -> int {
        if (*prev < 0) return SG_OK;
        const int pk = *prev;
        *prev = -1;
        const int drc = decide_stage(e, pk);
        activate(e, k);
        return drc;
    };
    if (B.radix) {
        HIPCHK(launch_rs_first(dev_ev, n, R, e->gbase, e->d_ring, ring_mask, e->cfg.statistic_max_rt, e->d_rec_o,
                               e->d_k1, e->d_v1, e->d_hist, nblocks, e->d_bsmall + 0, d_t0, e->d_prio, e->d_keyring,
                               e->d_comp, dev_ext, dev_args, n_args, SG_MAX_CONTEXTS, dev_auth(e), dev_auth_ids(e), gs));
        if (int drc = decide_prev()) return drc;
        for (int p = 0; p < passes; ++p) {
            if (p > 0) HIPCHK(launch_radix_hist(kin, n, p * db, e->d_hist, nblocks, gs));
            HIPCHK(launch_scan(e->d_hist, e->d_hist, (uint64_t)nblocks << db, e->d_part, nullptr, gs));
            HIPCHK(launch_radix_scatter(kin, vin, n, p * db, e->d_hist, nblocks, kout, vout,
                                        p == passes - 1 ? e->d_posof : nullptr, gs));
            std::swap(kin, kout);
            std::swap(vin, vout);
        }
        HIPCHK(launch_seg(kin, n, e->d_flag, e->d_pos, e->d_segs, gs, launch_scan, e->d_part, e->d_bsmall + 1));
        HIPCHK(launch_gather(e->d_rec_o, vin, kin, n, e->d_posof, e->d_recs, e->d_prev, e->d_bsmall + 3, e->d_link,
                             e->d_bst, e->epoch, e->d_bsmall + 0, gs));
        if (int brc = bins(nullptr, nullptr, nullptr)) return brc;
    } else {
        const uint32_t nhot = e->nhot;
        B.nhot = nhot;
        uint32_t* words = e->d_flag;
        uint32_t* hot_off = e->d_pos;
        uint32_t* ccnt = B.d_ccnt;
        HIPCHK(launch_grp_first(dev_ev, n, R, e->gbase, ring_mask, e->d_bsmall + 0, d_t0, e->d_prio, e->d_keyring,
                                e->d_comp, dev_ext, dev_args, n_args, SG_MAX_CONTEXTS, dev_auth(e), dev_auth_ids(e),
                                e->d_hot_tab, nhot, nblocks,
                                words, hot_off, e->d_k1, e->d_v1, ccnt, e->d_hist, gs));
        if (int drc = decide_prev()) return drc;
        HIPCHK(launch_hot_scan(hot_off, nblocks, nhot, e->d_hot_part, e->d_hot_hb, e->d_bsmall + 77, gs));
        HIPCHK(launch_cold_n(n, e->d_bsmall + 77, e->d_bsmall + 78, gs));
        if (nblocks == 1) {
            HIPCHK(launch_cold_small(kin, vin, ccnt, e->d_bsmall + 77, kout, vout, words, gs));
            std::swap(kin, kout);
            std::swap(vin, vout);
        }
        for (int p = 0; p < passes && nblocks > 1; ++p) {
            if (p > 0) HIPCHK(launch_radix_hist_n(kin, n, e->d_bsmall + 78, p * db, e->d_hist, nblocks, gs));
            HIPCHK(launch_scan(e->d_hist, e->d_hist, (uint64_t)nblocks << db, e->d_part, nullptr, gs));
            const bool last = p == passes - 1;
            HIPCHK(launch_radix_scatter_x(kin, vin, n, p ? e->d_bsmall + 78 : nullptr, p ? nullptr : ccnt,
                                          last ? e->d_bsmall + 77 : nullptr, p * db, e->d_hist, nblocks, kout, vout,
                                          last ? words : nullptr, gs));
            std::swap(kin, kout);
            std::swap(vin, vout);
        }
        HIPCHK(launch_hot_segs(e->d_hot_hb, nhot, e->d_hot_list, e->d_segs, e->d_bsmall + 80, gs));
        const uint64_t sc = nblocks + 64;
        HIPCHK(launch_seg_cold(kin, n, e->d_bsmall + 77, e->d_bsmall + 80, ccnt + sc, ccnt + 2 * sc, e->d_segs, gs,
                               launch_scan, e->d_part, e->d_bsmall + 82, e->d_bsmall + 1));
        uint32_t *need_hot = nullptr, *need_blk = nullptr, *bmax = nullptr;
        if (!(e->dbg_flags & TABLES_ALL)) {
            need_hot = e->d_need;
            need_blk = e->d_need + hot_max();
            bmax = e->d_need + e->need_words - hot_max();
            HIPCHK(launch_hot_bmax(dev_ev, nblocks, hot_off, nhot, e->d_hot_hb, e->d_edges, bmax, gs));
        }
        if (int brc = bins(need_hot, need_blk, bmax)) return brc;
        HIPCHK(launch_grp_records(dev_ev, n, e->gbase, ring_mask, e->cfg.statistic_max_rt, words, hot_off, nhot, nblocks,
                                  e->d_hot_hb, e->d_recs, vin, e->d_prev, e->d_bsmall + 3, e->d_bst,
                                  e->d_bsmall + 0, dev_ext, dev_args, SG_MAX_CONTEXTS, e->d_link, e->epoch, need_hot,
                                  need_blk, gs));
        HIPCHK(launch_block_sums(e->d_recs, n, e->d_bst, e->d_link, e->epoch, e->d_bsmall + 0, kin, e->d_bsmall + 77,
                                 need_blk, gs));
    }
    const uint32_t hot_min = (uint32_t)std::max<uint64_t>(64, n / 8192);
    if (!B.radix)
        HIPCHK(launch_hot_build(e->d_segs, e->d_bsmall + 1, mb, hot_min, R, e->d_hot_tab, e->d_hot_list, e->nhot,
                                e->d_bsmall + 76, gs));
    static_assert(8 + N_BINS + 1 <= 72 && HEAD_WORDS == 77, "head layout");
    HIPCHK(hipMemcpyAsync(B.h_head, e->d_bsmall, HEAD_WORDS * 4, hipMemcpyDeviceToHost, gs));
    HIPCHK(hipEventRecord(B.ev[1], gs));
    auto& G = B.g;
    G.n = n; G.n_args = n_args; G.gbase = e->gbase; G.ring_mask = ring_mask;
    G.dev_ev = dev_ev; G.dev_ext = dev_ext; G.dev_args = dev_args;
    G.out = out; G.dev_out = dev_out; G.vin = vin;
    G.epoch = e->epoch; G.skip_min = skip_min; G.lane_max = lane_max; G.mb = mb;
    G.ext = ext != nullptr; G.host_out = host_out; G.force_lane = force_lane;
    G.set = (int)(e->seq % sg_engine::N_SETS);
    e->grouped = k;
    return SG_OK;
}

static int accept_grouped(sg_engine* e, bool drop = false) {
    const int k = e->grouped;
    auto& B = e->slot[k];
    e->grouped = -1;
    HIPCHK(hipEventSynchronize(B.ev[1]));
    const uint32_t* head = B.h_head;
    if (!B.radix) e->nhot = std::min<uint32_t>(head[76], hot_max());
    if (drop) return SG_OK;
    B.hot_marked = head[73];
    const uint32_t bflags = head[0];
    if (bflags & BF_BAD_RES) return fail(SG_EINVAL, "event res_id >= max_resources");
    if (bflags & BF_BAD_REF)
        return fail(SG_EINVAL, "an EXIT/TRACE references an event that is not an earlier ENTRY of the same resource");
    if (bflags & BF_TSPAN) return fail(SG_EINVAL, "a batch must span less than 2^31 ms");
    if (bflags & BF_BACKWARD) return fail(SG_EINVAL, "event timestamps must be non-decreasing (SURVEY Q3)");
    if (bflags & BF_BAD_ARGS)
        return fail(SG_EINVAL, "an sg_event_ext names args outside the table (or more than SG_MAX_ARGS, or a bad kind)");
    if (e->has_mix && head[7] && (e->pv_on || e->pvt_on) && head[72]) {
        if (int prc = ensure_pv(e, head[72], head[7])) return prc;
    }
    e->inflight.push_back({B.g.set, B.hot_marked});
    ++e->seq;
    e->last = k;
    e->cur = k ^ 1;
    e->gbase += B.g.n;
    return SG_OK;
}

static int handoff(sg_engine* e) {
    if (e->grouped < 0) return SG_OK;
    const int k = e->grouped;
    if (int rc = accept_grouped(e)) return rc;
    return decide_stage(e, k);
}

static int decide_enqueue(sg_engine* e, int k);

static int decide_stage(sg_engine* e, int k) {
    const int rc = decide_enqueue(e, k);
    if (rc) {
        const std::string why = g_err;
        if (!e->inflight.empty()) e->inflight.pop_back();
        if (e->fatal.empty()) e->fatal = "the decide stage of an accepted batch could not be enqueued (" + why + ")";
        return fail(rc, why);
    }
    return rc;
}

static int decide_enqueue(sg_engine* e, int k) {
    activate(e, k);
    auto& B = e->slot[k];
    const auto& G = B.g;
    hipStream_t st = e->stream;
    const uint64_t n = G.n, n_args = G.n_args, ring_mask = G.ring_mask;
    const sg_event* dev_ev = G.dev_ev;
    const sg_event_ext* dev_ext = G.dev_ext;
    const sg_arg* dev_args = G.dev_args;
    uint32_t *out = G.out, *dev_out = G.dev_out, *vin = G.vin;
    const uint32_t skip_min = G.skip_min, lane_max = G.lane_max, mb = G.mb;
    const bool ext = G.ext, host_out = G.host_out, force_lane = G.force_lane;
    (void)n_args;
    const uint32_t* head = B.h_head;
    const uint32_t m = head[1];
    const uint32_t nprev = head[3];
    int64_t t0 = 0;
    std::memcpy(&t0, head + 4, 8);
    const uint32_t bflags = head[0];
    const uint32_t* off = head + 8;
    uint32_t bin_n[N_BINS];
    for (int b = 0; b < N_BINS; ++b) bin_n[b] = off[b + 1] - off[b];
    DevCfg dc;
    std::memset(&dc, 0, sizeof(dc));
    dc.max_rt = e->cfg.statistic_max_rt;
    dc.occupy_timeout = e->cfg.occupy_timeout_ms;
    dc.max_chain = e->cfg.max_slot_chain_size;
    dc.switch_on = e->cfg.switch_on;
    dc.ring_mask = ring_mask;
    dc.snap_hi = e->snap_hi;
    dc.dbg_flags = e->dbg_flags;
    dc.heads = e->has_head ? 1u : 0u;
    DevState S{};
    std::memset(&S, 0, sizeof(S));
    S.sec = e->d_sec;
    S.minb = e->d_minb;
    S.info = e->d_info;
    S.prog = e->d_prog;
    S.rules = e->d_rules;
    S.rstate = e->d_rstate;
    S.hot = e->d_hot;
    S.pmap = e->d_pmap;
    S.pbkt = e->d_pbkt;
    S.pdat = e->d_pdat;
    S.pbm = e->d_pbm;
    S.ppre = e->d_ppre;
    S.tmid = e->d_tmid;
    S.ring = e->d_ring;
    S.sink = e->d_sink;
    S.borrow = e->d_borrow;
    S.prio = e->d_prio;
    S.key_ring = e->d_keyring;
    S.gbase = G.gbase;
    S.link = e->d_link;
    S.bst = e->d_bst;
    S.pend = e->d_pend;
    S.spans = e->d_spans;
    S.nspan = e->d_bsmall + 120;
    S.span_cap = e->span_cap;
    S.epoch = G.epoch;
    S.skip_ok = !(bflags & (BF_MULTI_LINK | BF_ZERO_CNT)) && !(e->dbg_flags & 4) ? 1u : 0u;
    S.skip_min = skip_min;
    S.ext = dev_ext;
    S.args = dev_args;
    S.aux_tab = e->d_auxtab;
    S.aux_count = e->d_auxcnt;
    S.aux_cap = e->cfg.aux_node_capacity;
    S.aux_mask = e->aux_mask;
    S.max_ctx = SG_MAX_CONTEXTS;
    S.auth = dev_auth(e);
    S.auth_ids = dev_auth_ids(e);
    HIPCHK(hipStreamWaitEvent(st, B.ev[1], 0));
    const uint32_t n_mix = e->has_mix ? head[6] : 0u, n_mixw = e->has_mix ? head[7] : 0u;
    const bool serial_bins = (e->dbg_flags & 8) != 0;
    const bool pre_split = (n_mix || n_mixw) && !serial_bins;
    hipStream_t ps = pre_split ? e->bin_stream[1] : st;
    const uint32_t grant_all = (e->cfg.switch_on && e->cfg.max_slot_chain_size <= 0) ? 1u : 0u;
    if (n_mixw && (e->pv_on || e->pvt_on) && head[72]) {
        if (int prc = ensure_pv(e, head[72], n_mixw)) return prc;
        e->pv_last_m = n_mixw;
    }
    const bool pv_ran = n_mixw && e->pv_on && head[72];
    const bool pv_early = pv_ran && pre_split && grant_all && !e->has_multi;
    if (pv_early) {
        HIPCHK(hipStreamWaitEvent(ps, B.ev[1], 0));
        HIPCHK(launch_pv_a(e->d_recs, vin, e->d_segs, B.d_mix + B.mix_cap, n_mixw, S, dc, e->d_dec, e->d_pvseg, e->pvb,
                           head[72], e->d_pvtot, e->d_pvhist, e->d_pvpart, ps, launch_radix_hist_n,
                           launch_radix_scatter_n, launch_scan, radix_tile(), e->d_pvrest, grant_all));
    }
    HIPCHK(launch_resolve(e->d_prev, nprev, e->d_ring, e->d_recs, vin, dev_ext, st));
    if (e->cfg.switch_on && (e->cfg.max_slot_chain_size <= 0 || e->n_chains < (uint32_t)e->cfg.max_slot_chain_size)) {
        const bool grant_all = e->cfg.max_slot_chain_size <= 0;
        HIPCHK(launch_chain(e->d_recs, vin, e->d_segs, m, e->d_info, grant_all ? 1 : 0, e->d_bsmall + 2, e->d_cand,
                            dev_ev, e->d_prog, dev_ext, SG_MAX_CONTEXTS, st));
        if (!grant_all) {
            uint32_t ncand = 0;
            HIPCHK(hipMemcpyAsync(&ncand, e->d_bsmall + 2, 4, hipMemcpyDeviceToHost, st));
            HIPCHK(hipStreamSynchronize(st));
            if (ncand) {
                std::vector<uint64_t> cand(ncand);
                HIPCHK(hipMemcpy(cand.data(), e->d_cand, ncand * 8ull, hipMemcpyDeviceToHost));
                std::sort(cand.begin(), cand.end());
                std::vector<uint64_t> upd;
                std::unordered_map<uint32_t, int> seen;
                for (uint32_t i = 0; i < ncand; ++i) {
                    uint32_t res = (uint32_t)cand[i];
                    if (!seen.emplace(res, 1).second) continue;
                    bool grant = e->n_chains < (uint32_t)e->cfg.max_slot_chain_size;
                    if (grant) e->n_chains++;
                    upd.push_back(((uint64_t)(grant ? NI_CHAIN : NI_REJECTED) << 32) | res | (1ull << 63));
                }
                ncand = (uint32_t)upd.size();
                HIPCHK(hipMemcpyAsync(e->d_cand, upd.data(), ncand * 8ull, hipMemcpyHostToDevice, st));
                HIPCHK(launch_set_flags(e->d_info, e->d_cand, ncand, st));
                HIPCHK(hipStreamSynchronize(st));
            }
        }
    }
    if (pre_split) {
        HIPCHK(hipEventRecord(e->fork0, st));
        HIPCHK(hipStreamWaitEvent(ps, e->fork0, 0));
// ... 171 lines not shown
    if (!late || compact) {
        if (prev >= 0) {
            const int pk = prev;
            prev = -1;
            if ((rc = decide_stage(e, pk))) return rc;
        }
        while (e->inflight.size() > 1)
            if ((rc = collect(e))) return rc;
    }
    if (compact) {
        if (int drc = drain(e)) return drc;
        if (int crc = compact_pmaps(e)) return crc;
        ++e->n_compact;
    }
    const int k = e->cur;
    if ((rc = group_stage(e, k, ev, ext, n, args, n_args, out, &prev))) return give_up(rc);
    if (!late) return handoff(e);
    while (e->inflight.size() > 1)
        if ((rc = collect(e))) {
            (void)accept_grouped(e, true);
            return rc;
        }
    return SG_OK;
}

constexpr int TINY_FALLBACK = 1;
static int tiny_impl(sg_engine* e, const sg_event* ev, const sg_event_ext* ext, uint64_t n, const sg_arg* args,
                     uint64_t n_args, uint32_t* out) {
    if (!e || !ev || !out) return fail(SG_EINVAL, "null argument");
    if (n_args && !args) return fail(SG_EINVAL, "null args table");
    if (!e->fatal.empty()) return fail(SG_ESTATE, e->fatal + " -- engine unusable, recreate it");
    if (n > e->cfg.max_batch_events) return fail(SG_EINVAL, "batch larger than max_batch_events");
    HIPCHK(hipSetDevice(e->device));
    int rc = ensure_batch(e, n);
    if (rc) return rc;
    if ((rc = drain(e))) return rc;
    if ((rc = ensure_pool2(e))) return rc;
    const unsigned long long pfloor = e->h_pool_next ? e->h_pool_next[PC_FLOOR] : 0;
    if (e->pool_nb && e->h_pool_next[PC_NEXT] > pfloor + (e->pool_nb - pfloor) / 2) return TINY_FALLBACK;
    const int k = e->cur;
    activate(e, k);
    auto& B = e->slot[k];
    hipStream_t st = e->stream;
    const sg_event* dev_ev = ev;
    const bool host_out = !is_device_ptr(out);
    if (!is_device_ptr(ev)) {
        HIPCHK(hipMemcpyAsync(e->d_ev, ev, n * sizeof(sg_event), hipMemcpyHostToDevice, st));
        dev_ev = e->d_ev;
    }
    uint32_t* dev_out = host_out ? e->d_out : out;
    const sg_event_ext* dev_ext = ext;
    const sg_arg* dev_args = n_args ? args : nullptr;
    if (ext && !is_device_ptr(ext)) {
        if (n > B.ext_cap) {
            dfree(B.d_ext);
            B.ext_cap = std::max<uint64_t>(n, 1u << 16);
            HIPCHK(hipMalloc(&B.d_ext, B.ext_cap * sizeof(sg_event_ext)));
        }
        HIPCHK(hipMemcpyAsync(B.d_ext, ext, n * sizeof(sg_event_ext), hipMemcpyHostToDevice, st));
        dev_ext = B.d_ext;
    }
    if (n_args && !is_device_ptr(args)) {
        if (n_args > B.args_cap) {
            dfree(B.d_args);
            B.args_cap = std::max<uint64_t>(n_args, 1u << 16);
            HIPCHK(hipMalloc(&B.d_args, B.args_cap * sizeof(sg_arg)));
        }
        HIPCHK(hipMemcpyAsync(B.d_args, args, n_args * sizeof(sg_arg), hipMemcpyHostToDevice, st));
        dev_args = B.d_args;
    }
    if (++e->epoch == 0) e->epoch = 1;
    DevCfg dc;
    std::memset(&dc, 0, sizeof(dc));
    dc.max_rt = e->cfg.statistic_max_rt;
    dc.occupy_timeout = e->cfg.occupy_timeout_ms;
    dc.max_chain = e->cfg.max_slot_chain_size;
    dc.switch_on = e->cfg.switch_on;
    dc.ring_mask = (1ull << e->cfg.status_ring_log2) - 1;
    dc.snap_hi = e->snap_hi;
    dc.dbg_flags = e->dbg_flags;
    dc.heads = e->has_head ? 1u : 0u;
    DevState S{};
    std::memset(&S, 0, sizeof(S));
    S.sec = e->d_sec; S.minb = e->d_minb; S.info = e->d_info; S.prog = e->d_prog; S.rules = e->d_rules;
    S.rstate = e->d_rstate; S.hot = e->d_hot; S.pmap = e->d_pmap; S.pbkt = e->d_pbkt; S.pdat = e->d_pdat;
    S.pbm = e->d_pbm; S.ppre = e->d_ppre; S.tmid = e->d_tmid; S.ring = e->d_ring; S.sink = e->d_sink;
    S.borrow = e->d_borrow; S.prio = e->d_prio; S.key_ring = e->d_keyring; S.gbase = e->gbase; S.link = e->d_link;
    S.bst = e->d_bst; S.pend = e->d_pend; S.spans = e->d_spans; S.nspan = e->d_bsmall + 120; S.span_cap = e->span_cap;
    S.epoch = e->epoch; S.skip_ok = 0; S.skip_min = e->skip_min; S.ext = dev_ext; S.args = dev_args;
    S.aux_tab = e->d_auxtab; S.aux_count = e->d_auxcnt; S.aux_cap = e->cfg.aux_node_capacity; S.aux_mask = e->aux_mask;
    S.max_ctx = SG_MAX_CONTEXTS;
    S.auth = dev_auth(e);
    S.auth_ids = dev_auth_ids(e);
    const int cap = e->cfg.max_slot_chain_size;
    const uint32_t grants = cap <= 0 ? 1u : e->n_chains >= (uint32_t)cap ? 2u : 0u;
    HIPCHK(launch_tiny(dev_ev, (uint32_t)n, S, dc, e->cfg.max_resources, e->d_prio, e->d_comp, n_args, grants,
                       e->d_pool_next, e->pool_nb, e->epoch, e->d_recs, e->d_v0, e->d_dec, e->d_segs, e->d_bsmall,
                       dev_out, st));
    uint32_t bflags = 0;
    HIPCHK(hipMemcpyAsync(&bflags, e->d_bsmall, 4, hipMemcpyDeviceToHost, st));
    if (host_out) HIPCHK(hipMemcpyAsync(out, dev_out, n * 4, hipMemcpyDeviceToHost, st));
    if (e->pool_nb) HIPCHK(hipMemcpyAsync(e->h_pool_next, e->d_pool_next, PC_WORDS * 8, hipMemcpyDeviceToHost, st));
    HIPCHK(hipStreamSynchronize(st));
    if (bflags & BF_TINY_FALLBACK) return TINY_FALLBACK;
    if (bflags & BF_TINY_REJECTED) {
        if (bflags & BF_BAD_RES) return fail(SG_EINVAL, "event res_id >= max_resources");
        if (bflags & BF_BAD_REF)
            return fail(SG_EINVAL, "an EXIT/TRACE references an event that is not an earlier ENTRY of the same resource");
        if (bflags & BF_TSPAN) return fail(SG_EINVAL, "a batch must span less than 2^31 ms");
        if (bflags & BF_BACKWARD) return fail(SG_EINVAL, "event timestamps must be non-decreasing (SURVEY Q3)");
        return fail(SG_EINVAL, "an sg_event_ext names args outside the table (or more than SG_MAX_ARGS, or a bad kind)");
    }
    e->gbase += n;
    if (bflags & BF_BAD_REF)
        return fail(SG_EINVAL, "an EXIT/TRACE references an event that is not an earlier ENTRY of the same resource");
    if (bflags & BF_BACKWARD) return fail(SG_EINVAL, "event timestamps must be non-decreasing across batches (SURVEY Q3)");
    if (bflags & BF_AUX_FULL) return fail(SG_ECAPACITY, "origin/context node pool full (raise aux_node_capacity)");
    if (bflags & BF_PQ_INVARIANT)
        e->fatal = "internal error: a k_pq tile's presorted key subset did not match its accesses";
    else if (bflags & BF_POOL_FULL)
        e->fatal = "the hot-parameter map pool is used up (raise param_table_log2)";
    else if (bflags & BF_PTAB_FULL)
        e->fatal = "a hot-parameter map table could not place a key (its map holds a ghost entry)";
    if (bflags & (BF_PQ_INVARIANT | BF_PTAB_FULL | BF_POOL_FULL)) return fail(SG_ECAPACITY, e->fatal + " -- engine unusable");
    return SG_OK;
}

int sg_submit_async(sg_engine* e, const sg_event* ev, uint64_t n, uint32_t* out) {
    return submit_impl(e, ev, nullptr, n, nullptr, 0, out);
}

int sg_submit_ex_async(sg_engine* e, const sg_event* ev, const sg_event_ext* ext, uint64_t n, const sg_arg* args,
                       uint64_t n_args, uint32_t* out) {
    return submit_impl(e, ev, ext, n, args, n_args, out);
}

int sg_submit_ex(sg_engine* e, const sg_event* ev, const sg_event_ext* ext, uint64_t n, const sg_arg* args,
                 uint64_t n_args, uint32_t* out) {
    if (e && e->tiny_on && n && n <= tiny_max() && !e->radix_group) {
        const int trc = tiny_impl(e, ev, ext, n, args, n_args, out);
        if (trc != TINY_FALLBACK) return trc;
    }
    int rc = submit_impl(e, ev, ext, n, args, n_args, out);
    if (rc) {
        if (e) (void)drain(e);
        return rc;
    }
    return sg_sync(e);
}

int sg_intern_origin(sg_engine* e, const char* origin, uint32_t* out_id) {
    if (!e || !out_id) return fail(SG_EINVAL, "null argument");
    if (!origin || !*origin) { *out_id = 0; return SG_OK; }
    auto it = e->origin_ids.find(origin);
    if (it != e->origin_ids.end()) { *out_id = it->second; return SG_OK; }
    const uint32_t id = (uint32_t)e->origin_ids.size() + 1;
    if (id >= 0x7FFFFFFFu) return fail(SG_ECAPACITY, "too many origins");
    e->origin_ids.emplace(origin, id);
    *out_id = id;
    if (e->auth.by_name.count(origin)) {
        if (int rc = drain(e)) return rc;
        e->auth.on_intern(origin, id);
        if (int rc = upload_authority(e)) return rc;
    }
    if (e->rule_names.count(std::string("o\x01") + origin)) {
        if (int rc = drain(e)) return rc;
        return upload_rules(e, false, false, false);
// ... 476 lines not shown
```

### sentinel_amd/csrc/kernels.hip

```cpp
#include <hip/hip_runtime.h>
#include <stdint.h>
#include <stdlib.h>

#include "../../include/sentinel_gpu.h"
#include "authority.h"
#include "dev_types.h"

using namespace sg;

#define WAVE 64

#define RS_THREADS 256
#ifndef RS_ITEMS
#define RS_ITEMS 16
#endif
#define RS_TILE (RS_THREADS * RS_ITEMS)
#define RS_BINS 256

template <int DB>
__device__ __forceinline__ void hist_add(uint32_t* h, uint32_t d, bool valid) {
    uint64_t peers = __ballot(valid);
#pragma unroll
    for (int b = 0; b < DB; ++b) {
        const uint64_t bb = __ballot((d >> b) & 1);
// ... 62 lines not shown
                        for (uint32_t q = 0; q < a.len; ++q)
                            if (args[a.key + q].kind > SG_ARG_SCALAR) fl |= BF_BAD_ARGS;
                    }
                }
                const sg_arg a0 = args[x.arg_off];
                key0 = a0.kind == SG_ARG_SCALAR ? a0.key : NO_KEY;
                own_args = true;
            }
            if (x.context_id > max_ctx) mark |= PM_LANE;
            else if (x.origin_id != 0 || x.context_id != 0) {
                mark |= PM_AUX;
                if (x.origin_id >> TAG_ORIGIN_BITS) mark |= PM_LANE;
                else tag = x.origin_id | (x.context_id << TAG_ORIGIN_BITS);
            }
            if (auth && e.kind == SG_EV_ENTRY && x.origin_id != 0 && e.res_id < max_res &&
                auth_blocks(auth, auth_ids, e.res_id, x.origin_id))
                mark |= PM_LANE;
        }
        if (own_args) {
            r.flags = (uint8_t)((r.flags & ~SG_F_HAS_ARG) | (key0 != NO_KEY ? SG_F_HAS_ARG : 0));
            if (e.kind == SG_EV_EXIT) {
                r.flags |= RF_OWN_ARGS;
                if (e.flags & SG_F_EXIT_ARGS) mark |= PM_XARGS;
            }
        }
        r.x = tag;
        if (e.kind == SG_EV_ENTRY) {
            if (key_ring) key_ring[(gbase + i) & ring_mask] = key0;
            if (e.flags & SG_F_PRIORITIZED) mark |= PM_PRIO;
            if (e.flags & SG_F_BLOCKED_UPSTREAM) mark |= PM_LANE;
        } else {
            if (e.kind == SG_EV_EXIT) {
                const int64_t raw = (int64_t)(e.aux >> 48);
                r.rt = (uint16_t)(raw > max_rt ? max_rt : raw);
                if (own_args && key_ring) key_ring[(gbase + i) & ring_mask] = key0;
            }
            const uint64_t ref = e.aux & SG_REF_NONE;
            if (ref != SG_REF_NONE) {
                if (ref >= gbase) {
                    if (ref - gbase >= i) fl |= BF_BAD_REF;
                    else { r.code = RC_BATCH; r.x = (uint32_t)(ref - gbase); }
                } else {
                    r.code = RC_PREV;
                    r.x = (uint32_t)(ref & ring_mask);
                }
            }
        }
        if (mark && e.res_id < max_res && (prio[e.res_id] & mark) != mark) atomicOr(&prio[e.res_id], mark);
        rec_o[i] = r;
        const uint32_t key = (comp && e.res_id < max_res) ? comp[e.res_id] : e.res_id;
        keys[i] = key;
        vals[i] = (uint32_t)i | (e.kind == SG_EV_ENTRY ? 0x80000000u : 0u);
        hkey[it] = key;
    }
#pragma unroll
    for (int it = 0; it < RS_ITEMS; ++it) {
        const uint64_t i = base + (uint64_t)it * RS_THREADS + threadIdx.x;
        hist_add<DB>(h, hkey[it] & (NB - 1), i < n);
    }
    if (fl) atomicOr(bflags, fl);
    __syncthreads();
    for (int b = threadIdx.x; b < NB; b += RS_THREADS) ghist[(uint64_t)b * nblocks + blockIdx.x] = h[b];
}

#define HOT_MAX 1024u
#define HOT_NONE 0xFFFFu
#define W_HOT 0x80000000u
#define W_ENT 0x40000000u
#define W_POS 0x3FFFFFFFu

template <int DB>
__global__ __launch_bounds__(RS_THREADS) void k_grp_first(const sg_event* __restrict__ ev, uint64_t n, uint32_t max_res,
                                                       uint64_t gbase, uint64_t ring_mask, uint32_t* __restrict__ bflags,
                                                       int64_t* __restrict__ t0_out, uint32_t* __restrict__ prio,
                                                       uint64_t* __restrict__ key_ring, const uint32_t* __restrict__ comp,
                                                       const sg_event_ext* __restrict__ ext, const sg_arg* __restrict__ args,
                                                       uint64_t n_args, uint32_t max_ctx,
                                                       const AuthDesc* __restrict__ auth,
                                                       const uint32_t* __restrict__ auth_ids,
                                                       const uint16_t* __restrict__ hot_tab, uint32_t nhot,
                                                       uint32_t nblocks, uint32_t* __restrict__ words,
                                                       uint32_t* __restrict__ hot_hist, uint32_t* __restrict__ ckeys,
                                                       uint32_t* __restrict__ cvals, uint32_t* __restrict__ ccnt,
                                                       uint32_t* __restrict__ chist) {
    constexpr int NB = 1 << DB;
    __shared__ uint32_t wcnt[4][HOT_MAX];
    __shared__ uint32_t h[NB];
    __shared__ uint32_t cw[4];
    const int w = threadIdx.x >> 6, l = threadIdx.x & 63;
    for (int i = threadIdx.x; i < NB; i += RS_THREADS) h[i] = 0;
    for (uint32_t i = threadIdx.x; i < 4 * HOT_MAX; i += RS_THREADS) (&wcnt[0][0])[i] = 0;
    __syncthreads();
    const int64_t t0 = ev[0].ts;
    if (blockIdx.x == 0 && threadIdx.x == 0) *t0_out = t0;
    const uint64_t base = (uint64_t)blockIdx.x * RS_TILE;
    const uint64_t wbase = base + (uint64_t)w * (RS_TILE / 4);
    const uint64_t lt = (l == 0) ? 0ull : (~0ull >> (64 - l));
    uint32_t fl = 0;
    uint32_t kk[RS_ITEMS], rk[RS_ITEMS];
    uint32_t hotm = 0, entm = 0;
    uint32_t ccount = 0;
#pragma unroll
    for (int it = 0; it < RS_ITEMS; ++it) {
        const uint64_t i = wbase + (uint64_t)it * WAVE + l;
        const bool valid = i < n;
        uint32_t key = 0, hid = HOT_NONE;
        if (valid) {
            const sg_event e = ev[i];
            if (e.res_id >= max_res) fl |= BF_BAD_RES;
            const int64_t dt = e.ts - t0;
            if (dt < 0 || dt > 0x7FFFFFFFLL) fl |= (dt < 0 ? BF_BACKWARD : BF_TSPAN);
            if (i > 0 && ev[i - 1].ts > e.ts) fl |= BF_BACKWARD;
            uint32_t mark = 0;
            uint64_t key0 = (e.flags & SG_F_HAS_ARG) ? e.aux : NO_KEY;
            bool own_args = false;
            if (ext) {
                const sg_event_ext x = ext[i];
                if (x.n_args > SG_MAX_ARGS || (uint64_t)x.arg_off + x.n_args > n_args) fl |= BF_BAD_ARGS;
                else if (x.n_args) {
                    for (uint32_t k = 0; k < x.n_args; ++k) {
                        const sg_arg a = args[x.arg_off + k];
                        if (a.kind > SG_ARG_LIST || (a.kind == SG_ARG_LIST && (a.key > n_args || a.len > n_args - a.key)))
                            fl |= BF_BAD_ARGS;
                        else if (a.kind == SG_ARG_LIST) {
                            mark |= PM_ARGL;
                            for (uint32_t q = 0; q < a.len; ++q)
                                if (args[a.key + q].kind > SG_ARG_SCALAR) fl |= BF_BAD_ARGS;
                        }
                    }
                    const sg_arg a0 = args[x.arg_off];
                    key0 = a0.kind == SG_ARG_SCALAR ? a0.key : NO_KEY;
                    own_args = true;
                }
                if (x.context_id > max_ctx) mark |= PM_LANE;
                else if (x.origin_id != 0 || x.context_id != 0) {
                    mark |= PM_AUX;
                    if (x.origin_id >> TAG_ORIGIN_BITS) mark |= PM_LANE;
                }
                if (auth && e.kind == SG_EV_ENTRY && x.origin_id != 0 && e.res_id < max_res &&
                    auth_blocks(auth, auth_ids, e.res_id, x.origin_id))
                    mark |= PM_LANE;
            }
            if (own_args && e.kind == SG_EV_EXIT && (e.flags & SG_F_EXIT_ARGS)) mark |= PM_XARGS;
            if (e.kind == SG_EV_ENTRY) {
                if (key_ring) key_ring[(gbase + i) & ring_mask] = key0;
                if (e.flags & SG_F_PRIORITIZED) mark |= PM_PRIO;
                if (e.flags & SG_F_BLOCKED_UPSTREAM) mark |= PM_LANE;
            } else if (e.kind == SG_EV_EXIT && own_args && key_ring) {
                key_ring[(gbase + i) & ring_mask] = key0;
            }
            if (e.kind != SG_EV_ENTRY) {
                const uint64_t ref = e.aux & SG_REF_NONE;
                if (ref != SG_REF_NONE && ref >= gbase && ref - gbase >= i) fl |= BF_BAD_REF;
            }
            if (mark && e.res_id < max_res && (prio[e.res_id] & mark) != mark) atomicOr(&prio[e.res_id], mark);
            key = (comp && e.res_id < max_res) ? comp[e.res_id] : e.res_id;
            if (key < max_res) hid = hot_tab[key];
            if (e.kind == SG_EV_ENTRY) entm |= 1u << it;
        }
        kk[it] = key;
        const bool hot = valid && hid < nhot;
        uint64_t peers = __ballot(hot);
#pragma unroll
        for (int b = 0; b < 10; ++b) {
            const uint64_t bb = __ballot((hid >> b) & 1);
            peers &= ((hid >> b) & 1) ? bb : ~bb;
        }
        const uint32_t hrank = __popcll(peers & lt);
        uint32_t* myc = wcnt[w];
        const uint32_t old = hot ? myc[hid] : 0u;
        if (hot && hrank == 0) myc[hid] = old + (uint32_t)__popcll(peers);
        const uint64_t cb = __ballot(valid && !hot);
        if (hot) {
            hotm |= 1u << it;
            rk[it] = (hid << 16) | (old + hrank);
        } else {
            rk[it] = ccount + (uint32_t)__popcll(cb & lt);
        }
// ... 11 lines not shown
    }
    uint32_t coff = 0;
    for (int ww = 0; ww < w; ++ww) coff += cw[ww];
    if (threadIdx.x == 0) ccnt[blockIdx.x] = cw[0] + cw[1] + cw[2] + cw[3];
    for (int b = threadIdx.x; b < NB; b += RS_THREADS) chist[(uint64_t)b * nblocks + blockIdx.x] = h[b];
    __syncthreads();
#pragma unroll
    for (int it = 0; it < RS_ITEMS; ++it) {
        const uint64_t i = wbase + (uint64_t)it * WAVE + l;
        if (i >= n) continue;
        const uint32_t ent = ((entm >> it) & 1) ? W_ENT : 0u;
        if ((hotm >> it) & 1) {
            const uint32_t hid = rk[it] >> 16;
            words[i] = W_HOT | ent | (hid << 12) | (wcnt[w][hid] + (rk[it] & 0xFFFFu));
        } else {
            words[i] = ent;
            const uint64_t o = base + coff + rk[it];
            ckeys[o] = kk[it];
            cvals[o] = (uint32_t)i | (((entm >> it) & 1) ? 0x80000000u : 0u);
        }
    }
}

#define HS_TC 16u
__global__ __launch_bounds__(256) void k_hot_scan_a(const uint32_t* __restrict__ C, uint32_t nblocks, uint32_t nhot,
                                                    uint32_t* __restrict__ part) {
    const uint32_t c = blockIdx.x, t0 = c * HS_TC, t1 = min(nblocks, t0 + HS_TC);
    for (uint32_t h = threadIdx.x; h < nhot; h += 256) {
        uint32_t a = 0;
        for (uint32_t t = t0; t < t1; ++t) a += C[(uint64_t)t * nhot + h];
        part[(uint64_t)c * nhot + h] = a;
    }
}
__global__ __launch_bounds__(HOT_MAX) void k_hot_scan_b(uint32_t* __restrict__ part, uint32_t nch, uint32_t nhot,
                                                        uint32_t* __restrict__ hb, uint32_t* __restrict__ out) {
    __shared__ uint32_t ws[HOT_MAX / 64];
    const uint32_t h = threadIdx.x, l = h & 63, wv = h >> 6;
    uint32_t tot = 0;
    if (h < nhot) {
        constexpr uint32_t U = 16;
        uint32_t c = 0;
        for (; c + U <= nch; c += U) {
            uint32_t v[U];
#pragma unroll
            for (uint32_t k = 0; k < U; ++k) v[k] = part[(uint64_t)(c + k) * nhot + h];
#pragma unroll
            for (uint32_t k = 0; k < U; ++k) {
                part[(uint64_t)(c + k) * nhot + h] = tot;
                tot += v[k];
            }
        }
        for (; c < nch; ++c) {
            const uint32_t v = part[(uint64_t)c * nhot + h];
            part[(uint64_t)c * nhot + h] = tot;
            tot += v;
        }
    }
    uint32_t x = tot;
#pragma unroll
    for (int o = 1; o < 64; o <<= 1) {
        const uint32_t y = __shfl_up(x, o, 64);
        if ((int)l >= o) x += y;
    }
    if (l == 63) ws[wv] = x;
    __syncthreads();
    uint32_t pre = 0, all = 0;
    for (uint32_t k = 0; k < HOT_MAX / 64; ++k) { if (k < wv) pre += ws[k]; all += ws[k]; }
    if (h < nhot) { hb[h] = pre + x - tot; hb[HOT_MAX + h] = tot; }
    if (h == 0) *out = all;
}
__global__ __launch_bounds__(256) void k_hot_scan_c(uint32_t* __restrict__ C, uint32_t nblocks, uint32_t nhot,
                                                    const uint32_t* __restrict__ part, const uint32_t* __restrict__ hb) {
    const uint32_t c = blockIdx.x, t0 = c * HS_TC, t1 = min(nblocks, t0 + HS_TC);
    for (uint32_t h = threadIdx.x; h < nhot; h += 256) {
        uint32_t run = hb[h] + part[(uint64_t)c * nhot + h];
        for (uint32_t t = t0; t < t1; ++t) {
            const uint32_t v = C[(uint64_t)t * nhot + h];
            C[(uint64_t)t * nhot + h] = run;
            run += v;
        }
    }
}

#define BE_THREADS 1024
#define BE_ITEMS 8
__global__ __launch_bounds__(BE_THREADS) void k_bkt_edges(const sg_event* __restrict__ ev, uint32_t nblocks,
                                                          uint32_t* __restrict__ edges) {
    __shared__ uint32_t ws[BE_THREADS / 64];
    const uint32_t t = threadIdx.x, l = t & 63, wv = t >> 6;
    uint32_t run = 0;
    for (uint32_t c0 = 0; c0 < nblocks; c0 += BE_THREADS * BE_ITEMS) {
        const uint32_t t0 = c0 + t * BE_ITEMS;
        int64_t ts[BE_ITEMS + 1];
#pragma unroll
        for (int k = 0; k <= BE_ITEMS; ++k) {
            uint32_t tl = (t0 + k) ? t0 + k - 1 : 0u;
            if (tl >= nblocks) tl = nblocks - 1;
            ts[k] = ev[(uint64_t)tl * RS_TILE].ts;
        }
        uint32_t f = 0;
#pragma unroll
        for (int k = 0; k < BE_ITEMS; ++k)
            if (t0 + k < nblocks && (t0 + k == 0 || ts[k + 1] / 500 != ts[k] / 500)) f |= 1u << k;
        const uint32_t c = (uint32_t)__popc(f);
        uint32_t x = c;
#pragma unroll
        for (int o = 1; o < 64; o <<= 1) {
            const uint32_t y = __shfl_up(x, o, 64);
            if ((int)l >= o) x += y;
        }
        if (l == 63) ws[wv] = x;
        __syncthreads();
        uint32_t pre = 0, all = 0;
        for (uint32_t k = 0; k < BE_THREADS / 64; ++k) { if (k < wv) pre += ws[k]; all += ws[k]; }
        uint32_t o = 1 + run + pre + x - c;
#pragma unroll
        for (int k = 0; k < BE_ITEMS; ++k)
            if ((f >> k) & 1u) edges[o++] = t0 + k;
        run += all;
        __syncthreads();
    }
    if (t == 0) edges[0] = run;
}
#define BM_EDGES 32u
__global__ __launch_bounds__(256) void k_hot_bmax(const uint32_t* __restrict__ P, uint32_t nblocks, uint32_t nhot,
                                                  const uint32_t* __restrict__ hb, const uint32_t* __restrict__ edges,
                                                  uint32_t* __restrict__ bmax) {
    const uint32_t ne = edges[0], j0 = blockIdx.y * BM_EDGES, j1 = min(ne, j0 + BM_EDGES);
    const uint32_t h = blockIdx.x * 256 + threadIdx.x;
    if (j0 >= ne || h >= nhot) return;
    const uint32_t end = hb[h] + hb[HOT_MAX + h];
    uint32_t m = 0;
    for (uint32_t j = j0; j < j1; ++j) {
        const uint32_t a = edges[1 + j], b = j + 1 < ne ? edges[2 + j] : nblocks;
        const uint32_t lo = P[(uint64_t)(a ? a - 1 : 0u) * nhot + h];
        const uint32_t hi = b < nblocks ? P[(uint64_t)b * nhot + h] : end;
        m = max(m, hi - lo);
    }
    if (m) atomicMax(&bmax[h], m);
}

__device__ __forceinline__ uint32_t grp_pos(uint64_t j, uint32_t wd, const uint32_t* __restrict__ P, uint32_t nhot) {
    if (wd & W_HOT) return P[(j / RS_TILE) * nhot + ((wd >> 12) & (HOT_MAX - 1))] + (wd & 0xFFFu);
    return wd & W_POS;
}

#define GR_THREADS 256
#define GR_EVENTS (RS_TILE / 4)
#define GR_ITEMS (GR_EVENTS / GR_THREADS)
__global__ __launch_bounds__(GR_THREADS) void k_grp_records(const sg_event* __restrict__ ev, uint64_t n,
                                                            uint64_t gbase, uint64_t ring_mask, int32_t max_rt,
                                                            const uint32_t* __restrict__ words,
                                                            const uint32_t* __restrict__ P, uint32_t nhot,
                                                            uint32_t nblocks, const uint32_t* __restrict__ hb,
                                                            SEv* __restrict__ recs,
                                                            uint32_t* __restrict__ svals, uint32_t* __restrict__ prev,
                                                            uint32_t* __restrict__ nprev, uint32_t* __restrict__ bst,
                                                            uint32_t* __restrict__ bflags,
                                                            const sg_event_ext* __restrict__ ext,
                                                            const sg_arg* __restrict__ args, uint32_t max_ctx,
                                                            Link* __restrict__ link, uint32_t epoch,
                                                            const uint32_t* __restrict__ need_hot,
                                                            const uint32_t* __restrict__ need_blk) {
    __shared__ uint4 srec[GR_EVENTS];
    __shared__ uint32_t spos[GR_EVENTS], sval[GR_EVENTS];
    __shared__ uint32_t lo[HOT_MAX];
    __shared__ uint32_t r0[HOT_MAX];
    __shared__ uint32_t prow[HOT_MAX];
    __shared__ uint8_t hneed[HOT_MAX];
    __shared__ uint32_t ws[GR_THREADS / 64];
    __shared__ uint32_t nh_q;
    const uint32_t t = threadIdx.x, l = t & 63, wv = t >> 6;
    const uint32_t tile = blockIdx.x >> 2;
    const uint64_t base = (uint64_t)tile * RS_TILE + (uint64_t)(blockIdx.x & 3) * GR_EVENTS;
    sg_event e[GR_ITEMS];
    uint32_t wd[GR_ITEMS];
#pragma unroll
    for (int it = 0; it < GR_ITEMS; ++it) {
        const uint64_t i = base + (uint64_t)it * GR_THREADS + t;
        const uint64_t ic = i < n ? i : n - 1;
        e[it] = ev[ic];
        wd[it] = words[ic];
    }
#pragma unroll
    for (int it = 0; it < GR_ITEMS; ++it)
        if (base + (uint64_t)it * GR_THREADS + t >= n) { e[it].kind = 0xFF; wd[it] = 0; }
    for (uint32_t h = t; h < nhot; h += GR_THREADS) {
        lo[h] = 0;
        r0[h] = 0xFFFFFFFFu;
        prow[h] = P[(uint64_t)tile * nhot + h];
        hneed[h] = (!need_hot || need_hot[h]) ? 1 : 0;
    }
    __syncthreads();
#pragma unroll
    for (int it = 0; it < GR_ITEMS; ++it)
        if (wd[it] & W_HOT) {
            const uint32_t h = (wd[it] >> 12) & (HOT_MAX - 1);
            atomicAdd(&lo[h], 1u);
            atomicMin(&r0[h], wd[it] & 0xFFFu);
        }
    __syncthreads();
    {
        constexpr uint32_t PER = HOT_MAX / GR_THREADS;
        uint32_t c[PER], sum = 0;
#pragma unroll
        for (uint32_t k = 0; k < PER; ++k) {
            const uint32_t h = t * PER + k;
            c[k] = h < nhot ? lo[h] : 0u;
            sum += c[k];
        }
        uint32_t x = sum;
#pragma unroll
        for (int o = 1; o < 64; o <<= 1) {
            const uint32_t y = __shfl_up(x, o, 64);
            if ((int)l >= o) x += y;
        }
        if (l == 63) ws[wv] = x;
// ... 504 lines not shown
    info[r].last_fetch = nl;
}

__global__ void k_init_state(Bkt* __restrict__ sec, Bkt* __restrict__ minb, NodeInfo* __restrict__ info,
                             int64_t* __restrict__ borrow, uint32_t nres) {
    uint64_t i = (uint64_t)blockIdx.x * blockDim.x + threadIdx.x;
    Bkt z;
    z.ws = -1; z.pass = 0; z.block = 0; z.exc = 0; z.succ = 0; z.rt = 0; z.occ = 0; z.minrt = 0;
    if (i < (uint64_t)nres * 60) minb[i] = z;
    if (i < (uint64_t)nres * 2) {
        sec[i] = z;
        borrow[2 * i] = -1;
        borrow[2 * i + 1] = 0;
    }
    if (i < nres) {
        NodeInfo n;
        n.thread = 0; n.flags = 0; n.exc_sum_sec = -1; n.exc_sum = 0; n.last_fetch = -1;
        info[i] = n;
    }
}
__global__ void k_set_flags(NodeInfo* __restrict__ info, const uint64_t* __restrict__ upd, uint32_t n) {
    uint32_t i = blockIdx.x * blockDim.x + threadIdx.x;
    if (i >= n) return;
    uint64_t u = upd[i];
    uint32_t res = (uint32_t)u;
    uint32_t f = (uint32_t)((u >> 32) & 0x7FFFFFFFu);
    if (u >> 63) info[res].flags |= f;
    else info[res].flags &= ~f;
}
__global__ void k_region_copy(const uint64_t* __restrict__ src, uint64_t* __restrict__ dst, const uint64_t* __restrict__ tri) {
    const uint64_t s = tri[3 * blockIdx.x], d = tri[3 * blockIdx.x + 1], n = tri[3 * blockIdx.x + 2];
    for (uint64_t i = threadIdx.x; i < n; i += blockDim.x) dst[d + i] = src[s + i];
}

namespace sg {

hipError_t launch_rs_first(const sg_event* ev, uint64_t n, uint32_t max_res, uint64_t gbase, const uint8_t* ring,
                           uint64_t ring_mask, int32_t max_rt, SEv* rec_o, uint32_t* keys, uint32_t* vals,
                           uint32_t* ghist, uint32_t nblocks, uint32_t* bflags, int64_t* t0_out, uint32_t* prio,
                           uint64_t* key_ring, const uint32_t* comp, const sg_event_ext* ext, const sg_arg* args,
                           uint64_t n_args, uint32_t max_ctx, const AuthDesc* auth, const uint32_t* auth_ids,
                           hipStream_t st) {
    hipLaunchKernelGGL(k_rs_first<8>, dim3(nblocks), dim3(RS_THREADS), 0, st, ev, n, max_res, gbase, ring, ring_mask,
                       max_rt, rec_o, keys, vals, ghist, nblocks, bflags, t0_out, prio, key_ring, comp, ext, args,
                       n_args, max_ctx, auth, auth_ids);
    return hipGetLastError();
}
hipError_t launch_radix_hist(const uint32_t* keys, uint64_t n, int shift, uint32_t* ghist, uint32_t nblocks,
                             hipStream_t st) {
    hipLaunchKernelGGL(k_radix_hist<8>, dim3(nblocks), dim3(RS_THREADS), 0, st, keys, n, shift, ghist, nblocks,
                       (const uint32_t*)nullptr);
    return hipGetLastError();
}
hipError_t launch_radix_hist_n(const uint32_t* keys, uint64_t n, const uint32_t* ndev, int shift, uint32_t* ghist,
                               uint32_t nblocks, hipStream_t st) {
    hipLaunchKernelGGL(k_radix_hist<8>, dim3(nblocks), dim3(RS_THREADS), 0, st, keys, n, shift, ghist, nblocks, ndev);
    return hipGetLastError();
}
hipError_t launch_radix_scatter_n(const uint32_t* kin, const uint32_t* vin, uint64_t n, const uint32_t* ndev, int shift,
                                  const uint32_t* goff, uint32_t nblocks, uint32_t* kout, uint32_t* vout, hipStream_t st) {
    hipLaunchKernelGGL(k_radix_scatter<8>, dim3(nblocks), dim3(RS_THREADS), 0, st, kin, vin, n, shift, goff, nblocks,
                       kout, vout, (uint32_t*)nullptr, ndev, (const uint32_t*)nullptr, (const uint32_t*)nullptr, 0u);
    return hipGetLastError();
}
hipError_t launch_radix_scatter(const uint32_t* kin, const uint32_t* vin, uint64_t n, int shift, const uint32_t* goff,
                                uint32_t nblocks, uint32_t* kout, uint32_t* vout, uint32_t* pos_of, hipStream_t st) {
    hipLaunchKernelGGL(k_radix_scatter<8>, dim3(nblocks), dim3(RS_THREADS), 0, st, kin, vin, n, shift, goff, nblocks,
                       kout, vout, pos_of, (const uint32_t*)nullptr, (const uint32_t*)nullptr, (const uint32_t*)nullptr, 0u);
    return hipGetLastError();
}
hipError_t launch_radix_scatter_x(const uint32_t* kin, const uint32_t* vin, uint64_t n, const uint32_t* ndev,
                                  const uint32_t* tcnt, const uint32_t* dbase, int shift, const uint32_t* goff,
                                  uint32_t nblocks, uint32_t* kout, uint32_t* vout, uint32_t* pos_of, hipStream_t st) {
    hipLaunchKernelGGL(k_radix_scatter<8>, dim3(nblocks), dim3(RS_THREADS), 0, st, kin, vin, n, shift, goff, nblocks,
                       kout, vout, pos_of, ndev, tcnt, dbase, 1u);
    return hipGetLastError();
}
hipError_t launch_grp_first(const sg_event* ev, uint64_t n, uint32_t max_res, uint64_t gbase, uint64_t ring_mask,
                            uint32_t* bflags, int64_t* t0_out, uint32_t* prio, uint64_t* key_ring, const uint32_t* comp,
                            const sg_event_ext* ext, const sg_arg* args, uint64_t n_args, uint32_t max_ctx,
                            const AuthDesc* auth, const uint32_t* auth_ids,
                            const uint16_t* hot_tab, uint32_t nhot, uint32_t nblocks, uint32_t* words,
                            uint32_t* hot_hist, uint32_t* ckeys, uint32_t* cvals, uint32_t* ccnt, uint32_t* chist,
                            hipStream_t st) {
    hipLaunchKernelGGL(k_grp_first<8>, dim3(nblocks), dim3(RS_THREADS), 0, st, ev, n, max_res, gbase, ring_mask, bflags,
                       t0_out, prio, key_ring, comp, ext, args, n_args, max_ctx, auth, auth_ids, hot_tab, nhot, nblocks, words,
                       hot_hist, ckeys, cvals, ccnt, chist);
    return hipGetLastError();
}
hipError_t launch_hot_scan(uint32_t* C, uint32_t nblocks, uint32_t nhot, uint32_t* part, uint32_t* hb, uint32_t* total,
                           hipStream_t st) {
    if (!nhot) return hipMemsetAsync(total, 0, 4, st);
    const uint32_t nch = (nblocks + HS_TC - 1) / HS_TC;
    hipLaunchKernelGGL(k_hot_scan_a, dim3(nch), dim3(256), 0, st, C, nblocks, nhot, part);
    hipLaunchKernelGGL(k_hot_scan_b, dim3(1), dim3(HOT_MAX), 0, st, part, nch, nhot, hb, total);
    hipLaunchKernelGGL(k_hot_scan_c, dim3(nch), dim3(256), 0, st, C, nblocks, nhot, part, hb);
    return hipGetLastError();
}
hipError_t launch_hot_bmax(const sg_event* ev, uint32_t nblocks, const uint32_t* P, uint32_t nhot, const uint32_t* hb,
                           uint32_t* edges, uint32_t* bmax, hipStream_t st) {
    if (!nhot || !nblocks) return hipSuccess;
    hipLaunchKernelGGL(k_bkt_edges, dim3(1), dim3(BE_THREADS), 0, st, ev, nblocks, edges);
    hipLaunchKernelGGL(k_hot_bmax, dim3((nhot + 255) / 256, (nblocks + BM_EDGES - 1) / BM_EDGES), dim3(256), 0, st, P,
                       nblocks, nhot, hb, edges, bmax);
    return hipGetLastError();
}
hipError_t launch_grp_records(const sg_event* ev, uint64_t n, uint64_t gbase, uint64_t ring_mask, int32_t max_rt,
                              const uint32_t* words, const uint32_t* P, uint32_t nhot, uint32_t nblocks,
                              const uint32_t* hb, SEv* recs, uint32_t* svals, uint32_t* prev,
                              uint32_t* nprev, uint32_t* bst, uint32_t* bflags, const sg_event_ext* ext,
                              const sg_arg* args, uint32_t max_ctx, Link* link, uint32_t epoch,
                              const uint32_t* need_hot, const uint32_t* need_blk, hipStream_t st) {
    hipLaunchKernelGGL(k_grp_records, dim3(nblocks * 4), dim3(GR_THREADS), 0, st, ev, n, gbase, ring_mask, max_rt, words, P,
                       nhot, nblocks, hb, recs, svals, prev, nprev, bst, bflags, ext, args, max_ctx, link, epoch, need_hot,
                       need_blk);
    return hipGetLastError();
}
hipError_t launch_hot_segs(const uint32_t* hb, uint32_t nhot, const uint32_t* hot_list, Seg* segs, uint32_t* out,
                           hipStream_t st) {
    hipLaunchKernelGGL(k_hot_segs, dim3(1), dim3(HOT_MAX), 0, st, hb, nhot, hot_list, segs, out);
    return hipGetLastError();
}
hipError_t launch_hot_build(const Seg* segs, const uint32_t* mp, uint32_t mb, uint32_t min_len, uint32_t max_res, uint16_t* hot_tab,
                            uint32_t* hot_list, uint32_t nhot_old, uint32_t* hot_n, hipStream_t st) {
    if (nhot_old) hipLaunchKernelGGL(k_hot_clear, dim3((nhot_old + 255) / 256), dim3(256), 0, st, hot_tab, hot_list, nhot_old);
    if (mb) hipLaunchKernelGGL(k_hot_build, dim3((mb + 255) / 256), dim3(256), 0, st, segs, mp, min_len, max_res, hot_tab,
                               hot_list, hot_n);
    return hipGetLastError();
}
__global__ void k_cold_n(uint64_t n, const uint32_t* __restrict__ hot_total, uint32_t* __restrict__ out) {
    if (threadIdx.x == 0) *out = (uint32_t)(n - *hot_total);
}
hipError_t launch_cold_n(uint64_t n, const uint32_t* hot_total, uint32_t* out, hipStream_t st) {
    hipLaunchKernelGGL(k_cold_n, dim3(1), dim3(64), 0, st, n, hot_total, out);
    return hipGetLastError();
}
uint32_t hot_max() { return HOT_MAX; }

__global__ void k_grp_clear(uint32_t* __restrict__ bsmall, uint32_t nsmall, uint32_t* __restrict__ bst, uint32_t nbst,
                            uint32_t* __restrict__ need, uint32_t nneed) {
    const uint32_t i = blockIdx.x * blockDim.x + threadIdx.x;
    if (i < nsmall) bsmall[i] = 0;
    if (i < nbst) bst[i] = 0;
    if (i < nneed) need[i] = 0;
}
hipError_t launch_grp_clear(uint32_t* bsmall, uint32_t nsmall, uint32_t* bst, uint32_t nbst, uint32_t* need,
                            uint32_t nneed, hipStream_t st) {
    uint32_t m = nsmall > nbst ? nsmall : nbst;
    if (nneed > m) m = nneed;
    hipLaunchKernelGGL(k_grp_clear, dim3((m + 255) / 256), dim3(256), 0, st, bsmall, nsmall, bst, nbst, need, nneed);
    return hipGetLastError();
}

__global__ __launch_bounds__(1024) void k_cold_small(const uint32_t* __restrict__ kin, const uint32_t* __restrict__ vin,
                                                     const uint32_t* __restrict__ cnt_p, const uint32_t* __restrict__ dbase,
                                                     uint32_t* __restrict__ kout, uint32_t* __restrict__ vout,
                                                     uint32_t* __restrict__ words) {
    __shared__ unsigned long long s[RS_TILE];
    const uint32_t cnt = *cnt_p, ob = *dbase, t = threadIdx.x;
    uint32_t n2 = 1;
    while (n2 < cnt) n2 <<= 1;
    for (uint32_t i = t; i < n2; i += blockDim.x)
        s[i] = i < cnt ? (((unsigned long long)kin[i] << 32) | i) : ~0ull;
    __syncthreads();
    for (uint32_t k = 2; k <= n2; k <<= 1)
        for (uint32_t j = k >> 1; j > 0; j >>= 1) {
            for (uint32_t i = t; i < n2; i += blockDim.x) {
                const uint32_t l = i ^ j;
                if (l > i) {
                    const unsigned long long a = s[i], b = s[l];
                    if (((i & k) == 0) == (a > b)) { s[i] = b; s[l] = a; }
                }
            }
            __syncthreads();
        }
    for (uint32_t i = t; i < cnt; i += blockDim.x) {
        const uint32_t idx = (uint32_t)s[i], key = (uint32_t)(s[i] >> 32), v = vin[idx], dst = ob + i;
        kout[dst] = key;
        vout[dst] = v;
        words[v & 0x7FFFFFFFu] = dst | ((v >> 1) & W_ENT);
    }
}
hipError_t launch_cold_small(const uint32_t* kin, const uint32_t* vin, const uint32_t* cnt, const uint32_t* dbase,
                             uint32_t* kout, uint32_t* vout, uint32_t* words, hipStream_t st) {
    hipLaunchKernelGGL(k_cold_small, dim3(1), dim3(1024), 0, st, kin, vin, cnt, dbase, kout, vout, words);
    return hipGetLastError();
}
// ... 83 lines not shown
```

Before: 4.715 billion.

## Add per-resource lite descriptor, conditional state stores, and fuse bucket-edge pass

```diff
diff --git a/sentinel_amd/csrc/chain.h b/sentinel_amd/csrc/chain.h
--- a/sentinel_amd/csrc/chain.h
+++ b/sentinel_amd/csrc/chain.h
@@ -413,4 +413,31 @@
     S.info[res] = o;
 }
 
-}
+__device__ __forceinline__ void node_load_lite(Node& N, int64_t& last_fetch, const DevState& S, uint32_t res) {
+    N.sb[0] = S.sec[(uint64_t)res * 2 + 0];
+    N.sb[1] = S.sec[(uint64_t)res * 2 + 1];
+    const NodeInfo ni = S.info[res];
+    N.thread = ni.thread;
+    N.flags = ni.flags;
+    N.exc_sum_sec = ni.exc_sum_sec;
+    N.exc_sum = ni.exc_sum;
+    last_fetch = ni.last_fetch;
+    N.mslot = -1;
+    N.pfslot = -2;
+    N.mst = 0;
+    N.bor = nullptr;
+}
+__device__ __forceinline__ void node_store_lite(const Node& N, int64_t last_fetch, uint32_t sdirty, const DevState& S,
+                                                uint32_t res, uint32_t pflags) {
+    if (sdirty & 1u) S.sec[(uint64_t)res * 2 + 0] = N.sb[0];
+    if (sdirty & 2u) S.sec[(uint64_t)res * 2 + 1] = N.sb[1];
+    NodeInfo o;
+    o.thread = N.thread;
+    o.flags = N.flags;
+    o.exc_sum_sec = (pflags & PF_EXC_COUNT) ? N.exc_sum_sec : -1;
+    o.exc_sum = N.exc_sum;
+    o.last_fetch = last_fetch;
+    S.info[res] = o;
+}
+
+}
diff --git a/sentinel_amd/csrc/decide.hip b/sentinel_amd/csrc/decide.hip
--- a/sentinel_amd/csrc/decide.hip
+++ b/sentinel_amd/csrc/decide.hip
@@ -1185,6 +1185,29 @@
     mask = 0;
 }
 
+__device__ __forceinline__ bool lite_desc_matches(const LiteDesc& d, const DevState& S, uint32_t res, bool pl) {
+    const Prog pg = S.prog[res];
+    bool ok = !d.invalid && d.rule_off == pg.rule_off && d.n_flow == pg.n_flow && d.n_degrade == pg.n_degrade &&
+              d.pflags == pg.pflags && d.xf == pg.xf && d.tm_base == pg.tm_base && pg.n_param == (pl ? 1 : 0) && pg.n_flow <= 2 && pg.n_degrade <= 2;
+    if (!ok) return false;
+    const DRule* rules = S.rules + pg.rule_off + pg.n_param;
+#pragma unroll
+    for (int k = 0; k < 2; ++k) {
+        if (k >= pg.n_flow) break;
+        const DRule& r = rules[k];
+        ok = ok && __double_as_longlong(d.fcount[k]) == __double_as_longlong(r.count) && d.fslot[k] == r.slot &&
+             (((d.fthread >> k) & 1) != 0) == (r.grade == SG_FLOW_GRADE_THREAD);
+    }
+#pragma unroll
+    for (int k = 0; k < 2; ++k) {
+        if (k >= pg.n_degrade) break;
+        const DRule& r = rules[pg.n_flow + k];
+        ok = ok && __double_as_longlong(d.dcount[k]) == __double_as_longlong(r.count) && d.dwindow[k] == r.time_window &&
+             d.dgrade[k] == r.grade && d.dslot[k] == r.slot;
+    }
+    return ok;
+}
+
 #ifndef LITE_PL_WAVES
 #define LITE_PL_WAVES 1
 #endif
@@ -1197,9 +1220,17 @@
     if (i >= m) return;
     const Seg sg = segs[order[i]];
     const uint32_t res = sg.res;
-    const Prog pg = S.prog[res];
+    const LiteDesc pg = S.lite[res];
     Node N;
+#ifndef LITE_COND_STORE
+#define LITE_COND_STORE 1
+#endif
+#if LITE_COND_STORE
+    int64_t last_fetch;
+    node_load_lite(N, last_fetch, S, res);
+#else
     node_load(N, S, res);
+#endif
 #ifndef LITE_CH
 #define LITE_CH 4
 #endif
@@ -1210,8 +1241,12 @@
 #pragma unroll
     for (uint32_t k = 0; k < CH; ++k) cur[k] = r4[k < qmax ? k : qmax];
     if (((pg.xf & XF_PLITE) != 0) != PL) return;
+    if (pg.invalid) {
+        atomicOr(bflags, BF_LITE_DESC);
+        return;
+    }
     const int nf = pg.n_flow, nd = pg.n_degrade;
-    const DRule* rules = S.rules + pg.rule_off + (PL ? 1 : 0);
+    const uint32_t rs0 = pg.rule_off + (PL ? 1 : 0);
     __shared__ DRule spr[PL ? 256 : 1];
     __shared__ PMap smp[PL ? 256 : 1], stm[PL ? 256 : 1];
     DRule& pr = spr[PL ? threadIdx.x : 0];
@@ -1223,23 +1258,20 @@
         PLM.tid = tmap_of(S, pg.tm_base, 0);
         if (PLM.tid != NO_ID) PLM.tm = S.pmap[PLM.tid];
     }
-    double fcnt[2] = {0.0, 0.0};
-    bool fthr[2] = {false, false};
-    uint32_t fslot[2] = {0, 0};
-    DegParam dr[2];
-    uint32_t dslot[2] = {0, 0};
+    const double fcnt[2] = {pg.fcount[0], pg.fcount[1]};
+    const bool fthr[2] = {(pg.fthread & 1) != 0, (pg.fthread & 2) != 0};
+    const uint32_t fslot[2] = {pg.fslot[0], pg.fslot[1]};
+    const DegParam dr[2] = {DegParam{pg.dcount[0], pg.dwindow[0], pg.dgrade[0]},
+                            DegParam{pg.dcount[1], pg.dwindow[1], pg.dgrade[1]}};
+    const uint32_t dslot[2] = {pg.dslot[0], pg.dslot[1]};
     RState ds[2];
+    uint32_t rdirty = 0;
     if (nf + nd) {
         const int last = nf + nd - 1;
 #pragma unroll
         for (int k = 0; k < 2; ++k) {
-            const int fi = k < last ? k : last, di = nf + k < last ? nf + k : last;
-            fcnt[k] = rules[fi].count;
-            fthr[k] = rules[fi].grade == SG_FLOW_GRADE_THREAD;
-            fslot[k] = rules[fi].slot;
-            dr[k] = deg_param(rules[di]);
-            dslot[k] = rules[di].slot;
-            ds[k] = S.rstate[pg.rule_off + (PL ? 1 : 0) + di];
+            const int di = nf + k < last ? nf + k : last;
+            ds[k] = S.rstate[rs0 + di];
         }
     }
 #ifdef SG_KPROF
@@ -1264,6 +1296,8 @@
         L.H = sh > cfg.snap_hi ? sh : cfg.snap_hi;
     }
     const bool lchk = (cfg.dbg_flags & LITE_CHECK) != 0;
+    if (lchk && !lite_desc_matches(pg, S, res, PL)) atomicOr(bflags, BF_LITE_DESC);
+    uint32_t sdirty = 0;
     const bool has_chain = (N.flags & NI_CHAIN) != 0;
     const bool chain = has_chain && cfg.switch_on;
     if (sg.len && (t0 + recs[sg.start].dt) < (N.sb[0].ws > N.sb[1].ws ? N.sb[0].ws : N.sb[1].ws))
@@ -1323,14 +1357,19 @@
                 const int64_t exc_total = N.exc_sum;
 #pragma unroll
                 for (int k = 0; k < 2; ++k) {
-                    if (k < nd && status == ST_PASS && !degrade_pass(N, C, dr[k], ds[k], t, &exc_total)) {
-                        status = ST_BLOCK_DEGRADE;
-                        slot = dslot[k];
+                    if (k < nd && status == ST_PASS) {
+                        const RState o = ds[k];
+                        if (!degrade_pass(N, C, dr[k], ds[k], t, &exc_total)) {
+                            status = ST_BLOCK_DEGRADE;
+                            slot = dslot[k];
+                        }
+                        if ((o.a ^ ds[k].a) | (o.b ^ ds[k].b) | (o.c ^ ds[k].c)) rdirty |= 1u << k;
                     }
                 }
                 LPROF(ktg)
                 const bool passed = status == ST_PASS;
                 const int sl = sec_current(N, t, C.max_rt);
+                sdirty |= sl < 0 ? 0u : 1u << sl;
                 if (passed) {
                     N.thread++;
                     sec_add(N, sl, cntv, 0, 0, 0, 0, INT64_MAX);
@@ -1367,6 +1406,7 @@
             if (eff && kind == SG_EV_EXIT) {
                 if (T != L.T || md_full(L.pd)) lm_roll(L, N, C.minb, T, C.max_rt, C.pflags, lchk, bflags);
                 const int sl = sec_current(N, t, C.max_rt);
+                sdirty |= sl < 0 ? 0u : 1u << sl;
                 sec_add(N, sl, 0, 0, cntv, rtv, 0, rtv);
                 L.pd.s += cntv;
                 L.pd.rt += rtv;
@@ -1386,6 +1426,7 @@
             } else if (eff && cntv > 0) {
                 if (T != L.T || md_full(L.pd)) lm_roll(L, N, C.minb, T, C.max_rt, C.pflags, lchk, bflags);
                 const int sl = sec_current(N, t, C.max_rt);
+                sdirty |= sl < 0 ? 0u : 1u << sl;
                 sec_add(N, sl, 0, 0, 0, 0, cntv, INT64_MAX);
                 L.pd.e += cntv;
                 if (N.exc_sum_sec == T) N.exc_sum += cntv;
@@ -1409,10 +1450,15 @@
         lite_flush<CH>(dec, sg.start + jl, sg.len - jl, dw, dmask);
     }
     lm_put(L, C.minb, C.max_rt, lchk, bflags);
+#if LITE_COND_STORE
+    node_store_lite(N, last_fetch, sdirty, S, res, pg.pflags);
+#else
     node_store(N, S, res, pg.pflags);
+    rdirty = 3u;
+#endif
 #pragma unroll
     for (int k = 0; k < 2; ++k)
-        if (k < nd) S.rstate[pg.rule_off + (PL ? 1 : 0) + nf + k] = ds[k];
+        if (k < nd && ((rdirty >> k) & 1u)) S.rstate[rs0 + nf + k] = ds[k];
     if (PL) {
         pm_store(S, PLM.mid, PLM.mp);
         if (PLM.tid != NO_ID) pm_store(S, PLM.tid, PLM.tm);
diff --git a/sentinel_amd/csrc/dev_types.h b/sentinel_amd/csrc/dev_types.h
--- a/sentinel_amd/csrc/dev_types.h
+++ b/sentinel_amd/csrc/dev_types.h
@@ -85,6 +85,24 @@
     PX_CHAIN = 4
 };
 static_assert(sizeof(Prog) == 16, "Prog must be 16 B");
+
+struct alignas(64) LiteDesc {
+    uint32_t rule_off;
+    uint8_t n_flow, n_degrade, pflags;
+    uint8_t invalid;
+    uint16_t xf;
+    uint8_t fthread;
+    uint8_t pad0;
+    uint8_t fslot[2];
+    uint8_t dslot[2];
+    uint8_t dgrade[2];
+    uint8_t pad1[2];
+    int32_t dwindow[2];
+    uint32_t tm_base;
+    double fcount[2];
+    double dcount[2];
+};
+static_assert(sizeof(LiteDesc) == 64 && alignof(LiteDesc) == 64, "LiteDesc must be one 64-byte line");
 
 enum : uint8_t { RK_PARAM = 0, RK_FLOW = 1, RK_DEGRADE = 2 };
 
@@ -337,6 +355,7 @@
     Bkt* minb;
     NodeInfo* info;
     const Prog* prog;
+    const LiteDesc* lite;
     const DRule* rules;
     RState* rstate;
     const DHot* hot;
@@ -381,7 +400,8 @@
                   BF_ZERO_CNT = 256,
                   BF_TINY_FALLBACK = 4096,
                   BF_TINY_REJECTED = 8192,
-                  BF_LITE_STALE = 16384 };
+                  BF_LITE_STALE = 16384,
+                  BF_LITE_DESC = 32768 };
 
 struct SEv {
     int32_t dt;
diff --git a/sentinel_amd/csrc/engine.cpp b/sentinel_amd/csrc/engine.cpp
--- a/sentinel_amd/csrc/engine.cpp
+++ b/sentinel_amd/csrc/engine.cpp
@@ -44,11 +44,11 @@
                             const AuthDesc* auth, const uint32_t* auth_ids,
                             const uint16_t* hot_tab, uint32_t nhot, uint32_t nblocks, uint32_t* words,
                             uint32_t* hot_hist, uint32_t* ckeys, uint32_t* cvals, uint32_t* ccnt, uint32_t* chist,
-                            hipStream_t st);
+                            int64_t* tile_ts, hipStream_t st);
 hipError_t launch_hot_scan(uint32_t* C, uint32_t nblocks, uint32_t nhot, uint32_t* part, uint32_t* hb, uint32_t* total,
                            hipStream_t st);
-hipError_t launch_hot_bmax(const sg_event* ev, uint32_t nblocks, const uint32_t* P, uint32_t nhot, const uint32_t* hb,
-                           uint32_t* edges, uint32_t* bmax, hipStream_t st);
+hipError_t launch_hot_bmax(uint32_t nblocks, const uint32_t* P, uint32_t nhot, const uint32_t* hb,
+                           const int64_t* tile_ts, uint32_t* bmax, hipStream_t st);
 hipError_t launch_grp_records(const sg_event* ev, uint64_t n, uint64_t gbase, uint64_t ring_mask, int32_t max_rt,
                               const uint32_t* words, const uint32_t* P, uint32_t nhot, uint32_t nblocks,
                               const uint32_t* hb, SEv* recs, uint32_t* svals, uint32_t* prev,
@@ -502,6 +502,7 @@
     int64_t snap_hi = -1;
     NodeInfo* d_info = nullptr;
     Prog* d_prog = nullptr;
+    LiteDesc* d_lite = nullptr;
     DRule* d_rules = nullptr;
     RState* d_rstate = nullptr;
     DHot* d_hot = nullptr;
@@ -577,7 +578,7 @@
     uint32_t* d_hot_hb = nullptr;
     uint32_t* d_need = nullptr;
     uint64_t need_words = 0;
-    uint32_t* d_edges = nullptr;
+    int64_t* d_tile_ts = nullptr;
     uint32_t hot_marked_last = 0;
     bool radix_group = false;
     uint64_t radix_below = 1u << 18;
@@ -767,10 +768,10 @@
     dfree(e->d_hot_part);
     dfree(e->d_hot_hb);
     dfree(e->d_need);
-    dfree(e->d_edges);
+    dfree(e->d_tile_ts);
     e->need_words = hot_max() + c / 32768 + 2 + hot_max();
     HIPCHK(hipMalloc(&e->d_need, e->need_words * 4));
-    HIPCHK(hipMalloc(&e->d_edges, (nblocks + 2) * 4));
+    HIPCHK(hipMalloc(&e->d_tile_ts, (nblocks + 2) * 8));
     HIPCHK(hipMalloc(&e->d_hot_part, (nblocks / 16 + 2) * hot_max() * 4));
     HIPCHK(hipMalloc(&e->d_hot_hb, 2 * hot_max() * 4));
     for (auto& B : e->slot) {
@@ -828,6 +829,8 @@
     if (bflags & BF_AUX_FULL) return fail(SG_ECAPACITY, "origin/context node pool full (raise aux_node_capacity)");
     if (bflags & BF_LITE_STALE)
         return fail(SG_ESTATE, "internal error (SG_LITE_CHECK): k_lite stored a minute bucket without a load that was not stale");
+    if (bflags & BF_LITE_DESC)
+        return fail(SG_ESTATE, "internal error: a k_lite segment's descriptor is invalid or differs from its rule program");
     if (bflags & BF_PQ_INVARIANT)
         e->fatal = "internal error: a k_pq tile's presorted key subset did not match its accesses";
     else if (bflags & BF_POOL_FULL)
@@ -861,6 +864,34 @@
 static uint32_t rule_map_cap(int64_t duration_sec) {
     const int64_t c = (int64_t)PM_BASE_CAP * std::max<int64_t>(duration_sec, 1);
     return (uint32_t)std::min<int64_t>(c, PM_TOTAL_CAP);
+}
+
+static LiteDesc lite_desc(const Prog& p, const std::vector<DRule>& rules) {
+    LiteDesc d;
+    std::memset(&d, 0, sizeof(d));
+    const bool shape = (p.n_param == 0 || (p.xf & XF_PLITE)) && !p.multi && (p.pflags & PF_J16) &&
+                       !(p.pflags & (PF_WARM | PF_SERIAL));
+    if (!shape) { d.invalid = 1; return d; }
+    d.rule_off = p.rule_off;
+    d.n_flow = p.n_flow;
+    d.n_degrade = p.n_degrade;
+    d.pflags = p.pflags;
+    d.xf = p.xf;
+    d.tm_base = p.tm_base;
+    const DRule* r = rules.data() + p.rule_off + p.n_param;
+    for (int k = 0; k < p.n_flow; ++k) {
+        d.fcount[k] = r[k].count;
+        if (r[k].grade == SG_FLOW_GRADE_THREAD) d.fthread |= (uint8_t)(1u << k);
+        d.fslot[k] = r[k].slot;
+    }
+    for (int k = 0; k < p.n_degrade; ++k) {
+        const DRule& g = r[p.n_flow + k];
+        d.dcount[k] = g.count;
+        d.dwindow[k] = g.time_window;
+        d.dgrade[k] = g.grade;
+        d.dslot[k] = g.slot;
+    }
+    return d;
 }
 
 int upload_rules(sg_engine* e, bool reset_flow_state, bool reset_deg_state, bool reset_par_state) {
@@ -1158,6 +1189,15 @@
     }
     if (!hot.empty()) HIPCHK(hipMemcpy(e->d_hot, hot.data(), hot.size() * sizeof(DHot), hipMemcpyHostToDevice));
     HIPCHK(hipMemcpy(e->d_prog, prog.data(), R * sizeof(Prog), hipMemcpyHostToDevice));
+#ifdef SG_MUT_LITE_KEEP
+    static bool lite_once = false;
+    if (!lite_once && (lite_once = true))
+#endif
+    {
+        std::vector<LiteDesc> lite(R);
+        for (uint32_t r = 0; r < R; ++r) lite[r] = lite_desc(prog[r], rules);
+        HIPCHK(hipMemcpy(e->d_lite, lite.data(), R * sizeof(LiteDesc), hipMemcpyHostToDevice));
+    }
     e->n_dev_rules = (uint32_t)rules.size();
     e->has_mix = any_mix;
     e->has_head = any_head;
@@ -1257,6 +1297,7 @@
     uint64_t R = cfg.max_resources;
     if (hipMalloc(&e->d_sec, R * 2 * sizeof(Bkt)) != hipSuccess || hipMalloc(&e->d_minb, R * 60 * sizeof(Bkt)) != hipSuccess ||
         hipMalloc(&e->d_info, R * sizeof(NodeInfo)) != hipSuccess || hipMalloc(&e->d_prog, R * sizeof(Prog)) != hipSuccess ||
+        hipMalloc(&e->d_lite, R * sizeof(LiteDesc)) != hipSuccess ||
         hipMalloc(&e->d_ring, 1ull << cfg.status_ring_log2) != hipSuccess || hipMalloc(&e->d_small, 256 * 4) != hipSuccess ||
         hipMalloc(&e->d_sink, 1024 * 4) != hipSuccess || hipMalloc(&e->d_borrow, R * 4 * sizeof(int64_t)) != hipSuccess ||
         hipMalloc(&e->d_prio, R * 4) != hipSuccess || hipMalloc(&e->d_hot_tab, R * 2) != hipSuccess ||
@@ -1274,6 +1315,7 @@
             return bad(fail(SG_ENOMEM, "device allocation of the origin/context node table failed"));
     }
     if (hipMemsetAsync(e->d_prog, 0, R * sizeof(Prog), e->stream) != hipSuccess ||
+        hipMemsetAsync(e->d_lite, 0, R * sizeof(LiteDesc), e->stream) != hipSuccess ||
         hipMemsetAsync(e->d_ring, 0xFF, 1ull << cfg.status_ring_log2, e->stream) != hipSuccess ||
         hipMemsetAsync(e->d_prio, 0, R * 4, e->stream) != hipSuccess ||
         hipMemsetAsync(e->d_hot_tab, 0xFF, R * 2, e->stream) != hipSuccess ||
@@ -1438,7 +1480,7 @@
     e->grouped = -1;
     if (e->stream) (void)hipStreamSynchronize(e->stream);
     if (e->gstream) (void)hipStreamSynchronize(e->gstream);
-    dfree(e->d_sec); dfree(e->d_minb); dfree(e->d_info); dfree(e->d_prog); dfree(e->d_rules); dfree(e->d_rstate);
+    dfree(e->d_sec); dfree(e->d_minb); dfree(e->d_info); dfree(e->d_prog); dfree(e->d_lite); dfree(e->d_rules); dfree(e->d_rstate);
     dfree(e->d_hot); dfree(e->d_pmap); dfree(e->d_pbkt); dfree(e->d_pdat); dfree(e->d_pbm); dfree(e->d_ppre); dfree(e->d_tmid); dfree(e->d_ring); dfree(e->d_small); dfree(e->d_sink);
     dfree(e->d_pool_next); dfree(e->d_pmoves); dfree(e->d_pbkt2); dfree(e->d_pdat2); dfree(e->d_pcwork);
     if (e->h_pool_next) (void)hipHostFree(e->h_pool_next);
@@ -1447,7 +1489,7 @@
     if (e->gstream) (void)hipStreamSynchronize(e->gstream);
     for (auto& B : e->slot) free_slot(B);
     dfree(e->d_auth); dfree(e->d_auth_ids);
-    dfree(e->d_prio); dfree(e->d_hot_tab); dfree(e->d_hot_list); dfree(e->d_hot_part); dfree(e->d_hot_hb); dfree(e->d_need); dfree(e->d_edges); dfree(e->d_comp); dfree(e->d_auxtab); dfree(e->d_auxpool); dfree(e->d_auxcnt); dfree(e->d_auxmeta);
+    dfree(e->d_prio); dfree(e->d_hot_tab); dfree(e->d_hot_list); dfree(e->d_hot_part); dfree(e->d_hot_hb); dfree(e->d_need); dfree(e->d_tile_ts); dfree(e->d_comp); dfree(e->d_auxtab); dfree(e->d_auxpool); dfree(e->d_auxcnt); dfree(e->d_auxmeta);
     dfree(e->d_pflow); dfree(e->d_phot); dfree(e->d_pftab); dfree(e->d_pvtab); dfree(e->d_preq); dfree(e->d_pvals);
     dfree(e->d_cflow); dfree(e->d_cbkt); dfree(e->d_ctab); dfree(e->d_nslim); dfree(e->d_nslimit); dfree(e->d_nsb); dfree(e->d_borrow); dfree(e->d_keyring);
     dfree(e->d_treq); dfree(e->d_tres); dfree(e->d_tfidx); dfree(e->d_tbounds);
@@ -2470,7 +2512,7 @@
         HIPCHK(launch_grp_first(dev_ev, n, R, e->gbase, ring_mask, e->d_bsmall + 0, d_t0, e->d_prio, e->d_keyring,
                                 e->d_comp, dev_ext, dev_args, n_args, SG_MAX_CONTEXTS, dev_auth(e), dev_auth_ids(e),
                                 e->d_hot_tab, nhot, nblocks,
-                                words, hot_off, e->d_k1, e->d_v1, ccnt, e->d_hist, gs));
+                                words, hot_off, e->d_k1, e->d_v1, ccnt, e->d_hist, e->d_tile_ts, gs));
         if (int drc = decide_prev()) return drc;
         HIPCHK(launch_hot_scan(hot_off, nblocks, nhot, e->d_hot_part, e->d_hot_hb, e->d_bsmall + 77, gs));
         HIPCHK(launch_cold_n(n, e->d_bsmall + 77, e->d_bsmall + 78, gs));
@@ -2498,7 +2540,7 @@
             need_hot = e->d_need;
             need_blk = e->d_need + hot_max();
             bmax = e->d_need + e->need_words - hot_max();
-            HIPCHK(launch_hot_bmax(dev_ev, nblocks, hot_off, nhot, e->d_hot_hb, e->d_edges, bmax, gs));
+            HIPCHK(launch_hot_bmax(nblocks, hot_off, nhot, e->d_hot_hb, e->d_tile_ts, bmax, gs));
         }
         if (int brc = bins(need_hot, need_blk, bmax)) return brc;
         HIPCHK(launch_grp_records(dev_ev, n, e->gbase, ring_mask, e->cfg.statistic_max_rt, words, hot_off, nhot, nblocks,
@@ -2612,6 +2654,7 @@
     S.minb = e->d_minb;
     S.info = e->d_info;
     S.prog = e->d_prog;
+    S.lite = e->d_lite;
     S.rules = e->d_rules;
     S.rstate = e->d_rstate;
     S.hot = e->d_hot;
@@ -2949,7 +2992,7 @@
     dc.heads = e->has_head ? 1u : 0u;
     DevState S{};
     std::memset(&S, 0, sizeof(S));
-    S.sec = e->d_sec; S.minb = e->d_minb; S.info = e->d_info; S.prog = e->d_prog; S.rules = e->d_rules;
+    S.sec = e->d_sec; S.minb = e->d_minb; S.info = e->d_info; S.prog = e->d_prog; S.lite = e->d_lite; S.rules = e->d_rules;
     S.rstate = e->d_rstate; S.hot = e->d_hot; S.pmap = e->d_pmap; S.pbkt = e->d_pbkt; S.pdat = e->d_pdat;
     S.pbm = e->d_pbm; S.ppre = e->d_ppre; S.tmid = e->d_tmid; S.ring = e->d_ring; S.sink = e->d_sink;
     S.borrow = e->d_borrow; S.prio = e->d_prio; S.key_ring = e->d_keyring; S.gbase = e->gbase; S.link = e->d_link;
diff --git a/sentinel_amd/csrc/kernels.hip b/sentinel_amd/csrc/kernels.hip
--- a/sentinel_amd/csrc/kernels.hip
+++ b/sentinel_amd/csrc/kernels.hip
@@ -168,7 +168,7 @@
                                                        uint32_t nblocks, uint32_t* __restrict__ words,
                                                        uint32_t* __restrict__ hot_hist, uint32_t* __restrict__ ckeys,
                                                        uint32_t* __restrict__ cvals, uint32_t* __restrict__ ccnt,
-                                                       uint32_t* __restrict__ chist) {
+                                                       uint32_t* __restrict__ chist, int64_t* __restrict__ tile_ts) {
     constexpr int NB = 1 << DB;
     __shared__ uint32_t wcnt[4][HOT_MAX];
     __shared__ uint32_t h[NB];
@@ -180,6 +180,7 @@
     const int64_t t0 = ev[0].ts;
     if (blockIdx.x == 0 && threadIdx.x == 0) *t0_out = t0;
     const uint64_t base = (uint64_t)blockIdx.x * RS_TILE;
+    if (threadIdx.x == 0) tile_ts[blockIdx.x] = ev[base].ts;
     const uint64_t wbase = base + (uint64_t)w * (RS_TILE / 4);
     const uint64_t lt = (l == 0) ? 0ull : (~0ull >> (64 - l));
     uint32_t fl = 0;
@@ -357,57 +358,37 @@
     }
 }
 
-#define BE_THREADS 1024
-#define BE_ITEMS 8
-__global__ __launch_bounds__(BE_THREADS) void k_bkt_edges(const sg_event* __restrict__ ev, uint32_t nblocks,
-                                                          uint32_t* __restrict__ edges) {
-    __shared__ uint32_t ws[BE_THREADS / 64];
-    const uint32_t t = threadIdx.x, l = t & 63, wv = t >> 6;
-    uint32_t run = 0;
-    for (uint32_t c0 = 0; c0 < nblocks; c0 += BE_THREADS * BE_ITEMS) {
-        const uint32_t t0 = c0 + t * BE_ITEMS;
-        int64_t ts[BE_ITEMS + 1];
-#pragma unroll
-        for (int k = 0; k <= BE_ITEMS; ++k) {
-            uint32_t tl = (t0 + k) ? t0 + k - 1 : 0u;
-            if (tl >= nblocks) tl = nblocks - 1;
-            ts[k] = ev[(uint64_t)tl * RS_TILE].ts;
-        }
-        uint32_t f = 0;
-#pragma unroll
-        for (int k = 0; k < BE_ITEMS; ++k)
-            if (t0 + k < nblocks && (t0 + k == 0 || ts[k + 1] / 500 != ts[k] / 500)) f |= 1u << k;
-        const uint32_t c = (uint32_t)__popc(f);
-        uint32_t x = c;
-#pragma unroll
-        for (int o = 1; o < 64; o <<= 1) {
-            const uint32_t y = __shfl_up(x, o, 64);
-            if ((int)l >= o) x += y;
-        }
-        if (l == 63) ws[wv] = x;
+#define BM_TILES 32u
+__global__ __launch_bounds__(256) void k_hot_bmax(const uint32_t* __restrict__ P, uint32_t nblocks, uint32_t nhot,
+                                                  const uint32_t* __restrict__ hb, const int64_t* __restrict__ tile_ts,
+                                                  uint32_t* __restrict__ bmax) {
+    __shared__ uint32_t emask, nxt;
+    const uint32_t j0 = blockIdx.y * BM_TILES;
+    if (threadIdx.x < 64) {
+        const uint32_t t = j0 + threadIdx.x;
+        const bool e = threadIdx.x < BM_TILES && t < nblocks && (t == 0 || tile_ts[t] / 500 != tile_ts[t - 1] / 500);
+        const uint64_t m = __ballot(e);
+        if (threadIdx.x == 0) { emask = (uint32_t)m; nxt = nblocks; }
+    }
+    __syncthreads();
+    uint32_t rem = emask;
+    if (!rem) return;
+    for (uint32_t b = j0 + BM_TILES; b < nblocks; b += 256) {
+        const uint32_t t = b + threadIdx.x;
+        if (t < nblocks && tile_ts[t] / 500 != tile_ts[t - 1] / 500) atomicMin(&nxt, t);
         __syncthreads();
-        uint32_t pre = 0, all = 0;
-        for (uint32_t k = 0; k < BE_THREADS / 64; ++k) { if (k < wv) pre += ws[k]; all += ws[k]; }
-        uint32_t o = 1 + run + pre + x - c;
-#pragma unroll
-        for (int k = 0; k < BE_ITEMS; ++k)
-            if ((f >> k) & 1u) edges[o++] = t0 + k;
-        run += all;
+        const uint32_t v = nxt;
         __syncthreads();
-    }
-    if (t == 0) edges[0] = run;
-}
-#define BM_EDGES 32u
-__global__ __launch_bounds__(256) void k_hot_bmax(const uint32_t* __restrict__ P, uint32_t nblocks, uint32_t nhot,
-                                                  const uint32_t* __restrict__ hb, const uint32_t* __restrict__ edges,
-                                                  uint32_t* __restrict__ bmax) {
-    const uint32_t ne = edges[0], j0 = blockIdx.y * BM_EDGES, j1 = min(ne, j0 + BM_EDGES);
+        if (v < nblocks) break;
+    }
     const uint32_t h = blockIdx.x * 256 + threadIdx.x;
-    if (j0 >= ne || h >= nhot) return;
-    const uint32_t end = hb[h] + hb[HOT_MAX + h];
+    if (h >= nhot) return;
+    const uint32_t past = nxt, end = hb[h] + hb[HOT_MAX + h];
     uint32_t m = 0;
-    for (uint32_t j = j0; j < j1; ++j) {
-        const uint32_t a = edges[1 + j], b = j + 1 < ne ? edges[2 + j] : nblocks;
+    while (rem) {
+        const uint32_t a = j0 + (uint32_t)__ffs(rem) - 1;
+        rem &= rem - 1;
+        const uint32_t b = rem ? j0 + (uint32_t)__ffs(rem) - 1 : past;
         const uint32_t lo = P[(uint64_t)(a ? a - 1 : 0u) * nhot + h];
         const uint32_t hi = b < nblocks ? P[(uint64_t)b * nhot + h] : end;
         m = max(m, hi - lo);
@@ -1078,10 +1059,10 @@
                             const AuthDesc* auth, const uint32_t* auth_ids,
                             const uint16_t* hot_tab, uint32_t nhot, uint32_t nblocks, uint32_t* words,
                             uint32_t* hot_hist, uint32_t* ckeys, uint32_t* cvals, uint32_t* ccnt, uint32_t* chist,
-                            hipStream_t st) {
+                            int64_t* tile_ts, hipStream_t st) {
     hipLaunchKernelGGL(k_grp_first<8>, dim3(nblocks), dim3(RS_THREADS), 0, st, ev, n, max_res, gbase, ring_mask, bflags,
                        t0_out, prio, key_ring, comp, ext, args, n_args, max_ctx, auth, auth_ids, hot_tab, nhot, nblocks, words,
-                       hot_hist, ckeys, cvals, ccnt, chist);
+                       hot_hist, ckeys, cvals, ccnt, chist, tile_ts);
     return hipGetLastError();
 }
 hipError_t launch_hot_scan(uint32_t* C, uint32_t nblocks, uint32_t nhot, uint32_t* part, uint32_t* hb, uint32_t* total,
@@ -1093,12 +1074,11 @@
     hipLaunchKernelGGL(k_hot_scan_c, dim3(nch), dim3(256), 0, st, C, nblocks, nhot, part, hb);
     return hipGetLastError();
 }
-hipError_t launch_hot_bmax(const sg_event* ev, uint32_t nblocks, const uint32_t* P, uint32_t nhot, const uint32_t* hb,
-                           uint32_t* edges, uint32_t* bmax, hipStream_t st) {
+hipError_t launch_hot_bmax(uint32_t nblocks, const uint32_t* P, uint32_t nhot, const uint32_t* hb,
+                           const int64_t* tile_ts, uint32_t* bmax, hipStream_t st) {
     if (!nhot || !nblocks) return hipSuccess;
-    hipLaunchKernelGGL(k_bkt_edges, dim3(1), dim3(BE_THREADS), 0, st, ev, nblocks, edges);
-    hipLaunchKernelGGL(k_hot_bmax, dim3((nhot + 255) / 256, (nblocks + BM_EDGES - 1) / BM_EDGES), dim3(256), 0, st, P,
-                       nblocks, nhot, hb, edges, bmax);
+    hipLaunchKernelGGL(k_hot_bmax, dim3((nhot + 255) / 256, (nblocks + BM_TILES - 1) / BM_TILES), dim3(256), 0, st, P,
+                       nblocks, nhot, hb, tile_ts, bmax);
     return hipGetLastError();
 }
 hipError_t launch_grp_records(const sg_event* ev, uint64_t n, uint64_t gbase, uint64_t ring_mask, int32_t max_rt,
```

Result: no change. 4.709 billion (-0.1%).
